# Mattdl/CLsurvey

Measured on AMD Instinct MI355X. Metric: images/sec (train+importance pass), EWC small_VGG9 Tiny-ImageNet task batch, higher is better.
Workload: dtype f32 (bf16x6 split operands on the conv fwd/bwd-data matrix products, fp32 accumulate); 1 GPU; EWC small_VGG9_cl_128_128, Tiny-ImageNet shapes (3x64x64, 20 classes), batch 200: train step + Fisher step (BASELINE configs[1]); batch=200, parallelism=1 GPU

## Files before the change

clsurvey_amd/_lib.py:

```python
import ctypes as C
import os

_HERE = os.path.dirname(os.path.abspath(__file__))
LIB_PATH = os.path.join(_HERE, "libclhip.so")

_p = C.c_void_p
_i = C.c_int
_f = C.c_float
_z = C.c_size_t
_l = C.c_long


class HatParam(C.Structure):
    _fields_ = [("theta", _p), ("grad", _p), ("buf", _p), ("mask_back", _p), ("n", _z), ("is_emb", _i), ("reserved", _i)]


class HatGateJob(C.Structure):
    _fields_ = [("emb_row", _p), ("gate", _p), ("mask_pre", _p), ("n", _i), ("reserved", _i)]


class HatLayer(C.Structure):
    _fields_ = [("w", _p), ("gate_in", _p), ("out", _p), ("K", _z), ("C", _z), ("R", _z)]


class HatWgradJob(C.Structure):
    _fields_ = [("g", _p), ("w", _p), ("gate_in", _p), ("dgate_in", _p), ("K", _i), ("C", _i), ("R", _i), ("reserved", _i)]


class HatEmbJob(C.Structure):
    _fields_ = [("dgate", _p), ("gate", _p), ("mask_pre", _p), ("demb", _p), ("n", _i), ("rows", _i), ("t", _i), ("reserved", _i)]


class IcarlClass(C.Structure):
    _fields_ = [("row_begin", _i), ("row_end", _i), ("k", _i), ("out_off", _i)]


class LayerDesc(C.Structure):
    _fields_ = [("type", _i), ("cin", _i), ("cout", _i), ("relu", _i), ("pool", _i),
                ("w_off", _l), ("b_off", _l), ("ksize", _i), ("stride", _i), ("pad", _i), ("pool_k", _i), ("pool_s", _i),
                ("bn", _i), ("bn_w_off", _l), ("bn_b_off", _l), ("has_drop", _i)]


SIGNATURES = {
    "clhip_version": (_i, []),
    "clhip_arch": (C.c_char_p, []),
    "clhip_conv3x3_fwd": (_i, [_p, _p, _p, _p, _i, _i, _i, _i, _i, _i, _p]),
    "clhip_conv3x3_relu_pool_fwd": (_i, [_p, _p, _p, _p, _p, _i, _i, _i, _i, _i, _p]),
    "clhip_conv3x3_bwd_weight_unpool": (_i, [_p, _p, _p, _p, _p, _i, _i, _i, _i, _i, _p, _z, _p]),
    "clhip_conv3x3_bwd_data": (_i, [_p, _p, _p, _p, _i, _i, _i, _i, _i, _p]),
    "clhip_conv3x3_bwd_data_unpool": (_i, [_p, _p, _p, _p, _p, _i, _i, _i, _i, _i, _p]),
    "clhip_conv3x3_bwd_weight_ws": (_z, [_i, _i, _i, _i, _i]),
    "clhip_conv3x3_bwd_weight": (_i, [_p, _p, _p, _p, _i, _i, _i, _i, _i, _p, _z, _p]),
    "clhip_conv3x3_bwd_weight_slabs": (_i, [_p, _p, _p, _i, _i, _i, _i, _i, _p, _z, C.POINTER(_i), _p]),
    "clhip_conv3x3_bwd_weight_reduce": (_i, [_p, _p, _p, _i, _i, _i, _p]),
    "clhip_conv3x3_wino_ws": (_z, [_i, _i]),
    "clhip_conv3x3_wino_fwd": (_i, [_p, _p, _p, _p, _p, _i, _i, _i, _i, _i, _i, _p, _z, _p]),
    "clhip_conv3x3_wino_bwd_data": (_i, [_p, _p, _p, _p, _p, _i, _i, _i, _i, _i, _p, _z, _p]),
    "clhip_conv5x5_bs_ws": (_z, [_i, _i]),
    "clhip_conv5x5_bs_fwd": (_i, [_p, _p, _p, _p, _i, _i, _i, _i, _i, _i, _p, _z, _p]),
    "clhip_conv5x5_bs_bwd_data": (_i, [_p, _p, _p, _p, _i, _i, _i, _i, _i, _p, _z, _p]),
    "clhip_conv3x3_bs_ws": (_z, [_i, _i]),
    "clhip_conv3x3_bs_fwd": (_i, [_p, _p, _p, _p, _p, _i, _i, _i, _i, _i, _i, _p, _z, _p]),
    "clhip_conv3x3_bs_bwd_data": (_i, [_p, _p, _p, _p, _p, _i, _i, _i, _i, _i, _p, _z, _p]),
    "clhip_conv3x3_wino_bwd_weight_ws": (_z, [_i, _i, _i, _i, _i]),
    "clhip_conv3x3_wino_bwd_weight": (_i, [_p, _p, _p, _p, _p, _i, _i, _i, _i, _i, _p, _z, _p]),
    "clhip_conv3x3_wino_bwd_ws": (_z, [_i, _i, _i, _i, _i]),
    "clhip_conv3x3_wino_bwd": (_i, [_p, _p, _p, _p, _p, _p, _p, _p, _i, _i, _i, _i, _i, _p, _z, _p]),
    "clhip_maxpool2_fwd": (_i, [_p, _p, _p, _i, _i, _i, _p]),
    "clhip_maxpool2_bwd": (_i, [_p, _p, _p, _i, _i, _i, _p]),
    "clhip_fc_ws": (_z, [_i, _i, _i]),
    "clhip_fc_fwd": (_i, [_p, _p, _p, _p, _i, _i, _i, _i, _p, _z, _p]),
    "clhip_fc_bwd_data": (_i, [_p, _p, _p, _p, _i, _i, _i, _p, _z, _p]),
    "clhip_fc_bwd_weight": (_i, [_p, _p, _p, _p, _i, _i, _i, _p, _z, _p]),
    "clhip_relu_bwd": (_i, [_p, _p, _p, _z, _p]),
    "clhip_softmax_ce": (_i, [_p, _p, _i, _i, _i, _p, _p, _p, _p]),
    "clhip_mse_zero_sum": (_i, [_p, _z, _p, _p, _p]),
    "clhip_reg_sgd_step": (_i, [_p, _p, _p, _p, _p, _z, _f, _f, _f, _f, _i, _p]),
    "clhip_fisher_accum": (_i, [_p, _p, _z, _f, _p]),
    "clhip_mas_accum": (_i, [_p, _p, _z, _f, _f, _p]),
    "clhip_si_step": (_i, [_p, _p, _p, _p, _p, _p, _z, _f, _f, _f, _f, _i, _p]),
    "clhip_si_consolidate": (_i, [_p, _p, _p, _p, _z, _f, _p]),
    "clhip_maxpool_fwd": (_i, [_p, _p, _p, _i, _i, _i, _i, _i, _p]),
    "clhip_maxpool_bwd": (_i, [_p, _p, _p, _i, _i, _i, _i, _i, _p]),
    "clhip_conv2d_bwd_weight_ws": (_z, [_i] * 9),
    "clhip_conv2d_fwd": (_i, [_p, _p, _p, _p] + [_i] * 10 + [_p]),
    "clhip_conv2d_bwd_data": (_i, [_p, _p, _p, _p] + [_i] * 9 + [_p]),
    "clhip_conv2d_bwd_weight": (_i, [_p, _p, _p, _p] + [_i] * 9 + [_p, _z, _p]),
    "clhip_conv3x3_bs_bwd_weight_ws": (_z, [_i] * 5),
    "clhip_conv3x3_bs_bwd_weight": (_i, [_p] * 5 + [_i] * 5 + [_p, _z, _p]),
    "clhip_conv5x5_bs_bwd_weight_ws": (_z, [_i] * 5),
    "clhip_conv5x5_bs_bwd_weight": (_i, [_p] * 4 + [_i] * 5 + [_p, _z, _p]),
    "clhip_conv2d_s2d_ws": (_z, [_i] * 8),
    "clhip_conv2d_s2d_fwd": (_i, [_p, _p, _p, _p] + [_i] * 9 + [_p, _z, _p]),
    "clhip_conv2d_s2d_bwd_weight": (_i, [_p, _p, _p, _p] + [_i] * 8 + [_p, _z, _p]),
    "clhip_imm_merge": (_i, [_p, _p, _p, _i, _z, _p, _p]),
    "clhip_lwf_loss": (_i, [_p, _p, _p, _p, _i, _i, _i, _i, _f, _f, _i, _p, _p, _p, _p]),
    "clhip_packnet_finetune_mask": (_i, [_p, _z, _i, _p]),
    "clhip_packnet_kth_ws": (_z, []),
    "clhip_packnet_kth_abs": (_i, [_p, _p, _z, _i, _z, _p, _p, _z, _p]),
    "clhip_packnet_prune": (_i, [_p, _p, _z, _i, _p, _p]),
    "clhip_mask_grad_zero": (_i, [_p, _p, _z, _i, _p]),
    "clhip_mask_weight_zero": (_i, [_p, _p, _z, _i, _i, _p]),
    "clhip_packnet_sgd_step": (_i, [_p, _p, _p, _p, _z, _i, _f, _f, _f, _i, _p]),
    "clhip_hat_gate": (_i, [_p, _i, _f, _p, _p]),
    "clhip_hat_scale_weight": (_i, [_p, _p, _p, _z, _z, _z, _p]),
    "clhip_hat_weight_grad": (_i, [_p, _p, _p, _p, _p, _i, _i, _i, _p]),
    "clhip_hat_emb_grad": (_i, [_p, _p, _p, _i, _f, _f, _p, _p]),
    "clhip_hat_reg_sums": (_i, [_p, _p, _i, _p, _p]),
    "clhip_hat_backmask": (_i, [_p, _p, _p, _z, _z, _z, _p]),
    "clhip_hat_sgd_ws": (_z, []),
    "clhip_hat_sgd_step": (_i, [_p, _p, _p, _p, _z, _f, _f, _f, _i, _i, _f, _f, _f, _f, _i, _p, _z, _p]),
    "clhip_clamp": (_i, [_p, _z, _f, _f, _p]),
    "clhip_hat_sgd_multi_ws": (_z, [_i]),
    "clhip_hat_sgd_step_multi": (_i, [_p, _i, _f, _f, _f, _i, _f, _f, _f, _f, _f, _i, _p, _z, _p]),
    "clhip_hat_gates_multi": (_i, [_p, _i, _f, _p, _p]),
    "clhip_hat_scale_weights_multi": (_i, [_p, _i, _p]),
    "clhip_hat_weight_grads_multi": (_i, [_p, _i, _p]),
    "clhip_hat_emb_grads_multi": (_i, [_p, _i, _f, _f, _f, _p, _p]),
    "clhip_softmax_ce_slice": (_i, [_p, _p, _i, _i, _i, _i, _i, _p, _p, _p, _p]),
    "clhip_net_loss_step_slice": (_i, [_p, _p, _p, _p, _p, _i, _i, _i, _i, _p, _p, _p, _p, _p]),
    "clhip_axpy": (_i, [_p, _p, _z, _f, _i, _p]),
    "clhip_gem_gram_ws": (_z, [_i]),
    "clhip_gem_gram": (_i, [_p, _z, C.POINTER(_i), _i, _z, _p, _p, _z, _p]),
    "clhip_gem_project": (_i, [_p, _z, C.POINTER(_i), C.POINTER(_f), _i, _p, _p, _z, _p]),
    "clhip_gem_qp": (_i, [_p, _i, C.c_double, C.c_double, _p, _p, _p]),
    "clhip_gem_project_dev": (_i, [_p, _z, C.POINTER(_i), _p, _p, _i, _p, _p, _z, _p]),
    "clhip_net_create": (_i, [C.POINTER(LayerDesc), _i, _i, _i, _i, _i, C.POINTER(_p)]),
    "clhip_net_set_dropout": (_i, [_p, _i, _p, _l]),
    "clhip_net_set_bn": (_i, [_p, _i, _p, _p, _f, _f]),
    "clhip_net_set_training": (_i, [_p, _i]),
    "clhip_net_probe": (_i, [_p, _i]),
    "clhip_net_probe_read": (_i, [_p, C.POINTER(_f), C.POINTER(_i)]),
    "clhip_net_layer_input": (_i, [_p, _i, _p, _p]),
    "clhip_net_layer_pool_idx": (_i, [_p, _i, _p, _p]),
    "clhip_net_layer_paths": (_i, [_p, _i]),
    "clhip_net_probe_kind": (_i, [_p, _i, _i]),
    "clhip_net_set_input_grad": (_i, [_p, _i, _p]),
    "clhip_sigmoid_fwd": (_i, [_p, _p, _z, _p]),
    "clhip_sigmoid_bwd": (_i, [_p, _p, _p, _z, _p]),
    "clhip_mse_mean": (_i, [_p, _p, _z, _f, _p, _p, _p]),
    "clhip_adadelta_step": (_i, [_p, _p, _p, _p, _z, _f, _f, _f, _f, _p]),
    "clhip_bn_ws": (_z, [_i]),
    "clhip_bn_fwd": (_i, [_p, _p, _p, _p, _p, _p, _p, _p, _i, _i, _i, _i, _f, _f, _i, _p, _z, _p]),
    "clhip_bn_bwd": (_i, [_p, _p, _p, _p, _p, _p, _p, _p, _p, _i, _i, _i, _i, _i, _p, _z, _p]),
    "clhip_net_destroy": (None, [_p]),
    "clhip_net_workspace_bytes": (_z, [_p]),
    "clhip_net_num_classes": (_i, [_p]),
    "clhip_net_forward": (_i, [_p, _p, _p, _i, _p, _p, _p]),
    "clhip_net_backward": (_i, [_p, _p, _p, _p, _i, _p, _p, _p]),
    "clhip_net_loss_step": (_i, [_p, _p, _p, _p, _p, _i, _i, _p, _p, _p, _p, _p]),
    "clhip_rehearsal_assemble": (_i, [_p, _p, _i, _z, _p, _p, _l, _l, _i, _p, _i, _p, _p, _p]),
    "clhip_rehearsal_assemble_crop_flip": (_i, [_p, _p, _i, _i, _i, _i, _i, _i, _p, _l, _p, _p, _p, _l, _l, _i, _p, _p, _i, _p, _p, _p]),
    "clhip_loss_segments": (_i, [_p, _p, _p, _i, _i, _i, _p, _i, _f, _p, _p, _p, _p]),
    "clhip_net_loss_step_loss_segments": (_i, [_p, _p, _p, _p, _p, _p, _i, _i, _p, _i, _f, _p, _p, _p, _p, _p]),
    "clhip_gather_tasks": (_i, [_p, _i, _z, _p, _i, _p, _p, _p]),
    "clhip_slice_argmax_count": (_i, [_p, _i, _i, _p, _i, _p, _p, _p, _p, _p]),
    "clhip_gather_tasks_crop_flip": (_i, [_p, _i, _i, _i, _i, _i, _i, _p, _p, _i, _p, _p, _p]),
    "clhip_icarl_herd": (_i, [_p, _l, _i, _p, C.POINTER(IcarlClass), _i, _p, _l, _p]),
    "clhip_icarl_nme": (_i, [_p, _p, _i, _i, _i, _i, _i, _p, _p]),
}

_lib = None


def lib():
    global _lib
    if _lib is None:
        path = os.environ.get("CLHIP_LIB", LIB_PATH)
        if not os.path.exists(path):
            raise RuntimeError(
                "clsurvey_amd: %s not found. Build it with `python clsurvey_amd/build.py` "
                "(hipcc --offload-arch=gfx950). There is no CPU fallback." % path)
        import torch
        bundled = os.path.join(os.path.dirname(torch.__file__), "lib", "libamdhip64.so")
        if os.path.exists(bundled):
            C.CDLL(bundled, mode=C.RTLD_GLOBAL)
        h = C.CDLL(path)
        for name, (res, args) in SIGNATURES.items():
            fn = getattr(h, name)
            fn.restype = res
            fn.argtypes = args
        _lib = h
    return _lib


class ClhipError(RuntimeError):
    pass


def check(rc, what):
    if rc != 0:
        if rc > 0:
            raise ClhipError("%s: HIP error %d" % (what, rc))
        names = {-1: "CLHIP_EINVAL", -2: "CLHIP_ENOSPC", -3: "CLHIP_ENOTSUP"}
        raise ClhipError("%s: %s" % (what, names.get(rc, rc)))
```

clsurvey_amd/csrc/common.hpp:

```cpp
#pragma once
#include <hip/hip_runtime.h>
#include <stdint.h>
#include <stddef.h>
#include "../../include/clhip.h"

#define CLHIP_LAUNCH_CHECK()                          \
    do {                                              \
        hipError_t e__ = hipGetLastError();           \
        if (e__ != hipSuccess) return (int)e__;       \
    } while (0)

static inline hipStream_t as_stream(void* s) { return reinterpret_cast<hipStream_t>(s); }

static inline bool aligned16(const void* p) { return (reinterpret_cast<uintptr_t>(p) & 15u) == 0; }

static inline int ew_grid(size_t work_items, int block) {
    size_t g = (work_items + block - 1) / block;
    if (g < 1) g = 1;
    if (g > 2048) g = 2048;
    return (int)g;
}

static __device__ __attribute__((aligned(16))) float clhip_zero16[4] = {0.f, 0.f, 0.f, 0.f};

constexpr int CLHIP_OOB = (int)0x80000000;

constexpr int CLHIP_POOL_DEAD = 4;
typedef unsigned int clhip_u32x4 __attribute__((ext_vector_type(4)));
__device__ __forceinline__ __amdgpu_buffer_rsrc_t clhip_rsrc(const void* p, size_t bytes) {
    return __builtin_amdgcn_make_buffer_rsrc(const_cast<void*>(p), 0, bytes > 0x7fffffffull ? 0x7fffffff : (int)bytes, 0x00020000);
}
__device__ __forceinline__ float clhip_buf_load(__amdgpu_buffer_rsrc_t r, int voff, int soff) {
    return __uint_as_float(__builtin_amdgcn_raw_buffer_load_b32(r, voff, soff, 0));
}
__device__ __forceinline__ float4 clhip_buf_load4(__amdgpu_buffer_rsrc_t r, int voff, int soff) {
    const clhip_u32x4 v = __builtin_amdgcn_raw_buffer_load_b128(r, voff, soff, 0);
    return make_float4(__uint_as_float(v.x), __uint_as_float(v.y), __uint_as_float(v.z), __uint_as_float(v.w));
}
__device__ __forceinline__ float2 clhip_buf_load2(__amdgpu_buffer_rsrc_t r, int voff, int soff) {
    typedef unsigned int u32x2 __attribute__((ext_vector_type(2)));
    const u32x2 v = __builtin_amdgcn_raw_buffer_load_b64(r, voff, soff, 0);
    return make_float2(__uint_as_float(v.x), __uint_as_float(v.y));
}
__device__ __forceinline__ unsigned clhip_buf_load_u16(__amdgpu_buffer_rsrc_t r, int voff, int soff) {
    return (unsigned)__builtin_amdgcn_raw_buffer_load_b16(r, voff, soff, 0);
}
__device__ __forceinline__ unsigned clhip_buf_load_u8(__amdgpu_buffer_rsrc_t r, int voff, int soff) {
    return (unsigned)__builtin_amdgcn_raw_buffer_load_b8(r, voff, soff, 0);
}
#ifndef CLHIP_ST_AUX
#define CLHIP_ST_AUX 16
#endif
__device__ __forceinline__ void clhip_buf_store(float v, __amdgpu_buffer_rsrc_t r, int voff, int soff) {
    __builtin_amdgcn_raw_buffer_store_b32(__float_as_uint(v), r, voff, soff, CLHIP_ST_AUX);
}
__device__ __forceinline__ void clhip_buf_store_u8(uint8_t v, __amdgpu_buffer_rsrc_t r, int voff, int soff) {
    __builtin_amdgcn_raw_buffer_store_b8(v, r, voff, soff, 0);
}
__device__ __forceinline__ void clhip_buf_store4(float4 v, __amdgpu_buffer_rsrc_t r, int voff, int soff) {
    const clhip_u32x4 q = {__float_as_uint(v.x), __float_as_uint(v.y), __float_as_uint(v.z), __float_as_uint(v.w)};
    __builtin_amdgcn_raw_buffer_store_b128(q, r, voff, soff, CLHIP_ST_AUX);
}
__device__ __forceinline__ void clhip_buf_store2(float2 v, __amdgpu_buffer_rsrc_t r, int voff, int soff) {
    typedef unsigned int u32x2 __attribute__((ext_vector_type(2)));
    const u32x2 q = {__float_as_uint(v.x), __float_as_uint(v.y)};
    __builtin_amdgcn_raw_buffer_store_b64(q, r, voff, soff, CLHIP_ST_AUX);
}
__device__ __forceinline__ __amdgpu_buffer_rsrc_t clhip_out_rsrc(void* base) {
    return __builtin_amdgcn_make_buffer_rsrc(base, 0, 0x7fffffff, 0x00020000);
}
__device__ __forceinline__ size_t out_img_of(int C, int hw) { return (size_t)C * hw; }

__device__ __forceinline__ float wave_max(float v) {
#pragma unroll
    for (int o = 32; o > 0; o >>= 1) v = fmaxf(v, __shfl_xor(v, o, 64));
    return v;
}
__device__ __forceinline__ float wave_sum(float v) {
#pragma unroll
    for (int o = 32; o > 0; o >>= 1) v += __shfl_xor(v, o, 64);
    return v;
}
__device__ __forceinline__ double wave_sum(double v) {
#pragma unroll
    for (int o = 32; o > 0; o >>= 1) v += __shfl_xor(v, o, 64);
    return v;
}
__device__ __forceinline__ int wave_min(int v) {
#pragma unroll
    for (int o = 32; o > 0; o >>= 1) v = min(v, __shfl_xor(v, o, 64));
    return v;
}

typedef float floatx16 __attribute__((ext_vector_type(16)));
typedef float floatx4 __attribute__((ext_vector_type(4)));

__device__ __forceinline__ int mfma32_row(int r, int lane) { return (r & 3) + 8 * (r >> 2) + 4 * (lane >> 5); }


#define CLHIP_FC_MAX 4
struct clhip_fc_chain {
    int n;
    long w_off[CLHIP_FC_MAX], b_off[CLHIP_FC_MAX];
    int din[CLHIP_FC_MAX], dout[CLHIP_FC_MAX], relu[CLHIP_FC_MAX];
    size_t act_off[CLHIP_FC_MAX], dz_off[CLHIP_FC_MAX];
};
int clhip_internal_fc_chain_ok(const clhip_fc_chain* d);
int clhip_internal_fc_chain_wgrad(const clhip_fc_chain* d, float* grads, const float* x, int N, const float* acts,
                                  const float* dlogits, const float* dz, hipStream_t s);
struct clhip_gemm_args {
    const float* a; const float* b; float* out;
    int M, N, K; long sam, sak, sbk, sbn; int n_tiles, splits, k_per_split;
    const float* bias; const float* mask_src; int relu;
};
int clhip_internal_fc_bwd_data_args(const float* dy, const float* w, const float* relu_src, float* dx, int M, int I, int O,
                                    clhip_gemm_args* args_out);
int clhip_internal_fc_bwd_combo(const clhip_gemm_args* g, int gemm_blocks, const clhip_fc_chain* d, float* grads, const float* x,
                                int N, const float* acts, const float* dlogits, const float* dz, hipStream_t s);

int clhip_internal_fc_tail_ok(const clhip_fc_chain* d);
int clhip_internal_fc_tail(const clhip_fc_chain* d, const float* params, float* acts, int N, const int64_t* labels,
                           int reduction, int col_off, int ncols, float* dlogits, float* fcdz, float* loss_out, double* stats,
                           void* row_scratch, unsigned* counter, int do_loss, int do_bwd, const float* h1_slabs, int live,
                           hipStream_t s);
int clhip_internal_fc_fwd_partial(const float* x, const float* w, int M, int I, int O, void* ws, size_t ws_bytes, int* live,
                                  hipStream_t s);

#define CLHIP_WGRAD_JOBS_MAX 32
struct clhip_wgrad_job { const float* part; float* dw; float* db; int K, C, splits; int taps; };
int clhip_internal_conv3x3_wgrad_partial(const float* x, const float* dy, const uint8_t* unpool_idx, float* dw, float* db, int N,
                                         int C, int K, int H, int W, void* ws, size_t ws_bytes, void* stream, clhip_wgrad_job* job);
int clhip_internal_wgrad_reduce_multi(const clhip_wgrad_job* jobs, int n, hipStream_t s);

bool clhip_internal_convkk_ok(int N, int Cin, int Cout, int H, int W, int R, int S, int stride, int pad);
int clhip_internal_convkk(int mode, const float* in, const float* w, const float* bias, const float* mask_src, float* out, int N,
                          int Cin, int Cout, int H, int W, int relu, hipStream_t s);

struct clhip_wino_wt { const float* w; float* U; int Ko, Ci, mode, pad; };
int clhip_internal_wino_weights(const clhip_wino_wt* jobs, int n, hipStream_t s);
int clhip_internal_weight_images(const clhip_wino_wt* wino_jobs, int n_wino, const clhip_wino_wt* bs_jobs, int n_bs, hipStream_t s);
int clhip_internal_wino_conv_u(int mode, const float* in, const float* U, const float* bias, const float* mask_src, float* out,
                               uint8_t* pool_idx, int unpool, int N, int Cin, int Cout, int H, int W, int relu, hipStream_t s);
bool clhip_internal_wino_ok(int Cin, int Cout, int H, int W);
size_t clhip_internal_wino_ws(int Cin, int Cout);
bool clhip_internal_bs_ok(int Cin, int Cout, int H, int W);
bool clhip_internal_bs_preferred(int Cin, int Cout, int H, int W);
bool clhip_internal_bs5_preferred(int Cin, int Cout, int H, int W);
size_t clhip_internal_bs5_ws(int Cin, int Cout);
int clhip_internal_bs5_conv_u(int mode, const float* in, const void* wimg, const float* bias, const float* mask_src, float* out, int N,
                              int Cin, int Cout, int H, int W, int relu, hipStream_t s);
size_t clhip_internal_bs_ws(int Cin, int Cout);
int clhip_internal_bs_weights(const clhip_wino_wt* jobs, int n, hipStream_t s);
int clhip_internal_bs_conv_u(int mode, const float* in, const void* wimg, const float* bias, const float* mask_src, float* out,
                             uint8_t* pool_idx, int unpool, int N, int Cin, int Cout, int H, int W, int relu, hipStream_t s);
bool clhip_internal_bs5_wgrad_ok(int N, int C, int K, int H, int W);
size_t clhip_internal_bs5_wgrad_ws(int N, int C, int K, int H, int W);
int clhip_internal_bs5_wgrad(const float* x, const float* dy, float* dw, float* db, int N, int C, int K, int H, int W, void* ws,
                             size_t ws_bytes, hipStream_t s);
size_t clhip_internal_bs3k_wgrad_ws(int N, int C, int K, int H, int W);
int clhip_internal_bs3k_wgrad(const float* x, const float* dy, float* dw, float* db, int N, int C, int K, int H, int W, void* ws,
                              size_t ws_bytes, hipStream_t s);
bool clhip_internal_bs_wgrad_ok(int C, int K, int H, int W);
bool clhip_internal_bs_wgrad_preferred(int C, int K, int H, int W, int pooled);
size_t clhip_internal_bs_wgrad_ws(int N, int C, int K, int H, int W);
int clhip_internal_bs_wgrad_partial(const float* x, const float* dy, const uint8_t* unpool_idx, float* dw, float* db, int N, int C, int K,
                                    int H, int W, void* ws, size_t ws_bytes, hipStream_t s, clhip_wgrad_job* job);
bool clhip_internal_wino_wgrad_ok(int C, int K, int H, int W);
size_t clhip_internal_wino_wgrad_ws(int N, int C, int K, int H, int W);
int clhip_internal_wino_wgrad_partial(const float* x, const float* dy, const uint8_t* unpool_idx, float* dw, float* db, int N, int C,
                                      int K, int H, int W, void* ws, size_t ws_bytes, hipStream_t s, clhip_wgrad_job* job);
int clhip_internal_wino_pair(const float* dy, const uint8_t* unpool_idx, const float* U, const float* mask_src, float* dx,
                             const float* x, float* dw, float* db, int N, int C, int K, int H, int W, void* ws, size_t ws_bytes,
                             hipStream_t s, clhip_wgrad_job* job);
bool clhip_internal_wino_pair_shape(int N, int C, int K, int H, int W, int pooled);
int clhip_internal_wino_conv(int mode, const float* in, const float* w, const float* bias, const float* mask_src, float* out,
                             uint8_t* pool_idx, int unpool, int N, int Cin, int Cout, int H, int W, int relu, void* ws,
                             size_t ws_bytes, hipStream_t s);
```

clsurvey_amd/csrc/conv3x3.hip:

```cpp
#include "common.hpp"

namespace {

#ifdef CLHIP_TRACE
__device__ unsigned long long* g_trace = nullptr;
#define TR_NOW() __builtin_amdgcn_s_memtime()
#endif

constexpr int KT = 64;
constexpr int LDW = 65;

template <int TW, int TH, int NB>
struct Geo {
    static constexpr int BP = TW * TH * NB;
    static constexpr int TWP = TW + 2;
    static constexpr int PLANE = NB * (TH + 2) * TWP;
    static constexpr int NT = (BP + 63) / 64;
    static constexpr bool DENSE = (32 % TW != 0 && TW != 32);
    static_assert(DENSE || BP == 64 || BP == 128, "block tile must hold 64 or 128 pixels");
    static_assert(!DENSE || (NB == 1 && BP <= 192), "dense tiles: one plane of at most 192 pixels");
};

template <int TW, int TH>
__device__ __forceinline__ void tile_pixel(int s, int li, bool pool, int& nb, int& th, int& tw) {
    if (pool && TW == 32) {
        nb = 0; th = 2 * (s >> 1) + (li >> 4); tw = 16 * (s & 1) + (li & 15);
    } else {
        const int q = 32 * s + li;
        tw = q % TW; th = (q / TW) % TH; nb = q / (TW * TH);
        if ((32 % TW != 0 && TW != 32) && q >= TW * TH) { nb = 0; th = TH; tw = 0; }
    }
}

#ifndef CLHIP_CONV_MIN_WAVES
#define CLHIP_CONV_MIN_WAVES 1
#endif
template <int TW, int TH, int NB, int CK>
struct ConvLds {
    static constexpr int BUF_FLOATS = CK * 9 * LDW + CK * Geo<TW, TH, NB>::PLANE;
    static constexpr int FLOATS = 2 * BUF_FLOATS;
};

template <int TW, int TH, int NB, int CK, int MODE, bool VEC, bool UNPOOL = false>
__device__ __forceinline__ void conv3x3_mfma_body(
    const float* __restrict__ in, const float* __restrict__ wt, const float* __restrict__ bias,
    const float* __restrict__ mask_src, float* __restrict__ out,
    int N, int Cin, int Cout, int H, int W, int Kw, int Cw, int relu,
    int tiles_w, int tiles_h, int n_pix_tiles, uint8_t* __restrict__ pool_idx,
    const int bid, const int img0, float* __restrict__ lds, float* __restrict__ bias_s) {
    using G = Geo<TW, TH, NB>;
    static_assert(!UNPOOL || (MODE == 1 && VEC), "the fused un-pool lives in the 16-byte staging of backward-data");
    const bool pool = !UNPOOL && pool_idx != nullptr;
    constexpr int WS_FLOATS = CK * 9 * LDW;
    constexpr int XS_FLOATS = CK * G::PLANE;
    constexpr int BUF_FLOATS = WS_FLOATS + XS_FLOATS;
    static_assert(BUF_FLOATS == ConvLds<TW, TH, NB, CK>::BUF_FLOATS, "shared-array size of the launching kernel");

    const int tid = threadIdx.x;
    const int lane = tid & 63;
    const int wave = tid >> 6;
#ifdef CLHIP_TRACE
    const unsigned long long tr_start = TR_NOW();
#endif
    const int wk = wave & 1;
    const int wp = wave >> 1;
    const int li = lane & 31;
    const int kk = lane >> 5;

    const int kt = bid / n_pix_tiles;
    const int pt = bid - kt * n_pix_tiles;
    const int tw_i = pt % tiles_w;
    const int th_i = (pt / tiles_w) % tiles_h;
    const int ng = pt / (tiles_w * tiles_h);
    const int n0 = img0 + ng * NB, h0 = th_i * TH, w0 = tw_i * TW;
    const int ko0 = kt * KT;
    if (MODE == 0 && threadIdx.x < KT) bias_s[threadIdx.x] = (bias && ko0 + (int)threadIdx.x < Cout) ? bias[ko0 + threadIdx.x] : 0.f;

    constexpr int W_ELEMS = KT * CK * 9;
    const size_t plane_hw = (size_t)H * W;
    const int n_chunks = (Cin + CK - 1) / CK;
    const int Wp = W >> 1;
    const size_t plane_in = UNPOOL ? (size_t)(H >> 1) * Wp : plane_hw;
    const float* in_blk = in + (size_t)n0 * Cin * plane_in;

    constexpr int W_IT = VEC ? (W_ELEMS / 4 + 255) / 256 : (W_ELEMS + 255) / 256;
    constexpr int XROWS = CK * NB * (TH + 2);
    constexpr int XV_ELEMS = XROWS * (TW / 4);
    constexpr int X_IT = VEC ? (XV_ELEMS + 255) / 256 : (XS_FLOATS + 255) / 256;
    constexpr int H_IT = VEC ? (XROWS * 2 + 255) / 256 : 0;
    constexpr int NUNITS = W_IT + X_IT + H_IT;
    float4 wv[VEC ? W_IT : 1];
    float4 xv[VEC ? X_IT : 1];
    float hv[VEC ? (H_IT > 0 ? H_IT : 1) : 1];
    float wreg[VEC ? 1 : W_IT];
    float xreg[VEC ? 1 : X_IT];
    int woff[W_IT], wdst[VEC ? W_IT * (MODE == 0 ? 1 : 4) : W_IT];
    int xoff[X_IT], xdst[VEC ? X_IT : 1];
    int hoff[H_IT > 0 ? H_IT : 1], hdst[H_IT > 0 ? H_IT : 1];
    int wch[VEC ? 1 : W_IT], xch[VEC ? 1 : X_IT];
    float2 xp[UNPOOL ? X_IT : 1];
    unsigned xi[UNPOOL ? X_IT : 1], hi[UNPOOL && H_IT > 0 ? H_IT : 1];
    int xioff[UNPOOL ? X_IT : 1], xcode[UNPOOL ? X_IT : 1], hioff[UNPOOL && H_IT > 0 ? H_IT : 1], hcode[UNPOOL && H_IT > 0 ? H_IT : 1];

    if constexpr (VEC) {
#pragma unroll
        for (int j = 0; j < W_IT; ++j) {
            const int e = tid + 256 * j;
            woff[j] = CLHIP_OOB;
            if (MODE == 0) {
                const int kl = e / (CK * 9 / 4), f = e - kl * (CK * 9 / 4);
                if (e < W_ELEMS / 4 && ko0 + kl < Kw) woff[j] = ((ko0 + kl) * Cw * 9 + 4 * f) * 4;
            } else {
                const int kl = e / (KT * 9 / 4), f = e - kl * (KT * 9 / 4);
                if (e < W_ELEMS / 4 && 4 * f < (Cw - ko0) * 9) woff[j] = ((kl * Cw + ko0) * 9 + 4 * f) * 4;
            }
        }
#pragma unroll
        for (int j = 0; j < X_IT; ++j) {
            const int e = tid + 256 * j;
            const int rowid = e / (TW / 4), f = e - rowid * (TW / 4);
            const int cl = rowid / (NB * (TH + 2)), rr = rowid - cl * (NB * (TH + 2));
            const int nb = rr / (TH + 2), row = rr - nb * (TH + 2);
            const int n = n0 + nb, h = h0 - 1 + row;
            xoff[j] = CLHIP_OOB;
            if constexpr (UNPOOL) {
                xioff[j] = CLHIP_OOB;
                xcode[j] = (h & 1) << 1;
                if (e < XV_ELEMS && n < N && h >= 0 && h < H) {
                    xioff[j] = (int)(((size_t)nb * Cin + cl) * plane_in) + (h >> 1) * Wp + ((w0 + 4 * f) >> 1);
                    xoff[j] = xioff[j] * 4;
                }
            } else if (e < XV_ELEMS && n < N && h >= 0 && h < H) {
                xoff[j] = ((int)(((size_t)nb * Cin + cl) * plane_hw) + h * W + w0 + 4 * f) * 4;
            }
        }
#pragma unroll
        for (int j = 0; j < H_IT; ++j) {
            const int e = tid + 256 * j;
            const int rowid = e >> 1, side = e & 1;
            const int cl = rowid / (NB * (TH + 2)), rr = rowid - cl * (NB * (TH + 2));
            const int nb = rr / (TH + 2), row = rr - nb * (TH + 2);
            const int n = n0 + nb, h = h0 - 1 + row, w = side ? w0 + TW : w0 - 1;
            hoff[j] = CLHIP_OOB;
            if constexpr (UNPOOL) {
                hioff[j] = CLHIP_OOB;
                hcode[j] = ((h & 1) << 1) | (w & 1);
                if (e < XROWS * 2 && n < N && h >= 0 && h < H && w >= 0 && w < W) {
                    hioff[j] = (int)(((size_t)nb * Cin + cl) * plane_in) + (h >> 1) * Wp + (w >> 1);
                    hoff[j] = hioff[j] * 4;
                }
            } else if (e < XROWS * 2 && n < N && h >= 0 && h < H && w >= 0 && w < W) {
                hoff[j] = ((int)(((size_t)nb * Cin + cl) * plane_hw) + h * W + w) * 4;
            }
// ... 510 lines not shown
        const bool real = tap(j, c, r, s2);
#pragma unroll
        for (int half = 0; half < 2; ++half) {
            const int ch = ko0 + 32 * half + li;
            a[half][j] = (real && ch < Cout) ? wt[(size_t)ch * 27 + c * 9 + r * 3 + s2] : 0.f;
        }
    }
    const int b_row = li + kk * C3_TWP, b_col = li + kk, b_pln = li + kk * C3_PLANE;
    auto b_addr = [&](int j) -> int {
        if (j < 9) return b_row + (j / 3) * C3_PLANE + (j % 3);
        if (j < 12) return b_col + (j - 9) * C3_PLANE + 2 * C3_TWP;
        if (j == 12) return b_pln + 2 * C3_TWP + 2;
        return li + 2 * C3_PLANE + 2 * C3_TWP + 2;
    };

    float sv[7];
    const size_t plane_hw = (size_t)H * W;
    const int st_src = kk * W + li;
    const int st_dst = kk * C3_TWP + li + 1;
    const int e_line = lane >> 1, e_side = lane & 1;
    const int e_c = e_line >> 2, e_rr = e_line & 3;
    const int st_esrc = e_c * (int)plane_hw + (e_rr - 1) * W + (e_side ? C3_TW : -1);
    const int st_edst = e_c * C3_PLANE + e_rr * C3_TWP + (e_side ? C3_TW + 1 : 0);
    auto tile_coords = [&](int t, int& n, int& h, int& w0) {
        const int tw = t % tiles_w, q = t / tiles_w;
        const int th = q % tiles_h;
        n = q / tiles_h; h = th * C3_TH + 2 * wave; w0 = tw * C3_TW;
    };
    auto load_tile = [&](int t) {
        int n, h, w0;
        tile_coords(t, n, h, w0);
        const float* xb = x + (size_t)n * 3 * plane_hw + (size_t)h * W + w0;
        bool rok[2];
        rok[0] = (unsigned)(h - 1 + kk) < (unsigned)H;
        rok[1] = (unsigned)(h + 1 + kk) < (unsigned)H;
#pragma unroll
        for (int i = 0; i < 6; ++i) {
            const float* p = xb + (i >> 1) * (ptrdiff_t)plane_hw + (2 * (i & 1) - 1) * W + st_src;
            sv[i] = *(rok[i & 1] ? p : clhip_zero16);
        }
        const bool eok = lane < 24 && (unsigned)(h - 1 + e_rr) < (unsigned)H &&
                         (unsigned)(w0 + (e_side ? C3_TW : -1)) < (unsigned)W;
        const float* pe = xb + st_esrc;
        sv[6] = *(eok ? pe : clhip_zero16);
    };
    float* hw_s = halo_s + wave * (2 * C3_HALO);
    auto store_tile = [&](int buf) {
        float* d = hw_s + buf * C3_HALO;
#pragma unroll
        for (int i = 0; i < 6; ++i) d[(i >> 1) * C3_PLANE + 2 * (i & 1) * C3_TWP + st_dst] = sv[i];
        if (lane < 24) d[st_edst] = sv[6];
    };

    const int OH = H >> 1, OW = W >> 1;
    int tile = blockIdx.x, buf = 0;
    if (tile < ntiles) { load_tile(tile); store_tile(0); }
    __builtin_amdgcn_s_waitcnt(0x0F70);
    __syncthreads();
    float* pw = pool_s + wave * (KT * C3_PLD);
    uint8_t* iw = idx_s + wave * (KT * 16);
    float* pw_l = pw + 4 * kk * C3_PLD + (li >> 1);
    uint8_t* iw_l = iw + 4 * kk * 16 + (li >> 1);
    const float* bias_k = bias_s + 4 * kk;
    for (; tile < ntiles; tile += gridDim.x, buf ^= 1) {
        const int next = tile + gridDim.x;
        if (next < ntiles) load_tile(next);

        floatx16 acc[2][2];
#pragma unroll
        for (int half = 0; half < 2; ++half)
#pragma unroll
            for (int row = 0; row < 2; ++row)
#pragma unroll
                for (int r = 0; r < 16; ++r) acc[half][row][r] = 0.f;
        const float* xs = hw_s + buf * C3_HALO;
        float b0[14], b1[14];
#pragma unroll
        for (int j = 0; j < 14; ++j) { b0[j] = xs[b_addr(j)]; b1[j] = xs[b_addr(j) + C3_TWP]; }
        __builtin_amdgcn_sched_barrier(0);
#pragma unroll
        for (int j = 0; j < 14; ++j) {
            acc[0][0] = __builtin_amdgcn_mfma_f32_32x32x2f32(a[0][j], b0[j], acc[0][0], 0, 0, 0);
            acc[1][0] = __builtin_amdgcn_mfma_f32_32x32x2f32(a[1][j], b0[j], acc[1][0], 0, 0, 0);
            acc[0][1] = __builtin_amdgcn_mfma_f32_32x32x2f32(a[0][j], b1[j], acc[0][1], 0, 0, 0);
            acc[1][1] = __builtin_amdgcn_mfma_f32_32x32x2f32(a[1][j], b1[j], acc[1][1], 0, 0, 0);
        }

        if (next < ntiles) store_tile(buf ^ 1);

        int n, h, w0;
        tile_coords(tile, n, h, w0);
        asm volatile("" ::: "memory");
#pragma unroll
        for (int half = 0; half < 2; ++half)
#pragma unroll
            for (int r = 0; r < 16; ++r) {
                const float bv = bias_k[32 * half + (r & 3) + 8 * (r >> 2)];
                const float tl = fmaxf(acc[half][0][r] + bv, 0.f), bl = fmaxf(acc[half][1][r] + bv, 0.f);
                const float tr = dpp_xor1(tl), br = dpp_xor1(bl);
                float m = tl; int am = 0;
                if (tr > m) { m = tr; am = 1; }
                if (bl > m) { m = bl; am = 2; }
                if (br > m) { m = br; am = 3; }
                if (!(m > 0.f)) am = CLHIP_POOL_DEAD;
                acc[half][0][r] = m;
                acc[half][1][r] = __int_as_float(am);
            }
        if (!(li & 1)) {
#pragma unroll
            for (int half = 0; half < 2; ++half)
#pragma unroll
                for (int r = 0; r < 16; ++r) {
                    const int c0 = 32 * half + (r & 3) + 8 * (r >> 2);
                    pw_l[c0 * C3_PLD] = acc[half][0][r];
                    iw_l[c0 * 16] = (uint8_t)__float_as_int(acc[half][1][r]);
                }
        }
        __builtin_amdgcn_wave_barrier();
        if (h < H) {
            const size_t chw = (size_t)OH * OW;
            const size_t obase = (size_t)n * Cout * chw + (size_t)(h >> 1) * OW + (w0 >> 1);
#pragma unroll
            for (int i = 0; i < 4; ++i) {
                const int q = lane + 64 * i, cl = q >> 2, part = q & 3;
                const float4 v = *reinterpret_cast<const float4*>(pw + cl * C3_PLD + 4 * part);
                if (ko0 + cl < Cout) *reinterpret_cast<float4*>(out + obase + (size_t)(ko0 + cl) * chw + 4 * part) = v;
            }
            const uint4 iv = *reinterpret_cast<const uint4*>(iw + lane * 16);
            if (ko0 + lane < Cout) *reinterpret_cast<uint4*>(pool_idx + obase + (size_t)(ko0 + lane) * chw) = iv;
        }
        __builtin_amdgcn_wave_barrier();
    }
}

#ifndef CLHIP_C3W64
#define CLHIP_C3W64 1
#endif
constexpr int W6_TWP = 67;
constexpr int W6_PLANE = 4 * W6_TWP;
constexpr int W6_HALO = 3 * W6_PLANE;

#ifndef C3W64_ABL
#define C3W64_ABL 0
#endif
#ifndef CLHIP_C3W64_BIAS_IN_K
#define CLHIP_C3W64_BIAS_IN_K 0
#endif
#if C3W64_ABL & 8
__device__ __forceinline__ floatx16 c3w64_fake_mfma(float a, float b, floatx16 c) { c[0] += a * b; return c; }
#define C3W64_MFMA(a, b, c, x, y, z) c3w64_fake_mfma(a, b, c)
#else
#define C3W64_MFMA(a, b, c, x, y, z) __builtin_amdgcn_mfma_f32_32x32x2f32(a, b, c, x, y, z)
#endif
template <bool FULL>
__global__ __launch_bounds__(512) void conv3x3_c3w64_relu_pool_kernel(
    const float* __restrict__ x, const float* __restrict__ wt, const float* __restrict__ bias,
    float* __restrict__ out, uint8_t* __restrict__ pool_idx, int N, int Cout, int H, int W,
    int tiles_w, int row_pairs, int ntiles) {
    __shared__ __attribute__((aligned(16))) float halo_s[8 * 2 * W6_HALO];
#if CLHIP_C3W64_BIAS_IN_K
    __shared__ float ones_s[W6_TWP + 5];
#else
    __shared__ float bias_s[KT];
#endif
    const int tid = threadIdx.x, lane = tid & 63, wave = tid >> 6, li = lane & 31, kk = lane >> 5;
    const int ko0 = blockIdx.y * KT;
#if CLHIP_C3W64_BIAS_IN_K
    if (tid < W6_TWP + 5) ones_s[tid] = 1.f;
#else
    if (tid < KT) bias_s[tid] = (bias && ko0 + tid < Cout) ? bias[ko0 + tid] : 0.f;
#endif

    float a[2][14];
    auto tap = [&](int j, int& c, int& r, int& s) -> bool {
        if (j < 9) { c = j / 3; s = j - 3 * c; r = kk; return true; }
        if (j < 12) { c = j - 9; r = 2; s = kk; return true; }
        if (j == 12) { c = kk; r = 2; s = 2; return true; }
        c = 2; r = 2; s = 2; return kk == 0;
    };
#pragma unroll
    for (int j = 0; j < 14; ++j) {
        int c, r, s2;
        const bool real = tap(j, c, r, s2);
#pragma unroll
        for (int half = 0; half < 2; ++half) {
            const int ch = ko0 + 32 * half + li;
            a[half][j] = (real && ch < Cout) ? wt[(size_t)ch * 27 + c * 9 + r * 3 + s2] : 0.f;
#if CLHIP_C3W64_BIAS_IN_K
            if (j == 13 && kk == 1) a[half][j] = (bias && ch < Cout) ? bias[ch] : 0.f;
#endif
        }
    }
    const int b_row = 2 * li + kk * W6_TWP, b_col = 2 * li + kk, b_pln = 2 * li + kk * W6_PLANE;
    auto b_addr = [&](int j) -> int {
        if (j < 9) return b_row + (j / 3) * W6_PLANE + (j % 3);
        if (j < 12) return b_col + (j - 9) * W6_PLANE + 2 * W6_TWP;
        if (j == 12) return b_pln + 2 * W6_TWP + 2;
        return 2 * li + 2 * W6_PLANE + 2 * W6_TWP + 2;
    };

    const int simd = blockIdx.x * 4 + (wave & 3), nsimd = gridDim.x * 4;
    const int units = 2 * ntiles;
    const int per = units / nsimd, rem = units - per * nsimd;
    const int s_start = simd * per + min(simd, rem), s_cnt = per + (simd < rem ? 1 : 0);
    const int first = (s_cnt + 1) >> 1;
    const int u0 = __builtin_amdgcn_readfirstlane((wave >> 2) ? s_start + first : s_start);
    const int u1 = __builtin_amdgcn_readfirstlane((wave >> 2) ? s_start + s_cnt : s_start + first);

    const size_t plane_hw = (size_t)H * W;
    const __amdgpu_buffer_rsrc_t r_x = clhip_rsrc(x, (size_t)N * 3 * plane_hw * 4);
    float sv[13];
    const int e_line = lane >> 1, e_side = lane & 1, e_c = e_line >> 2, e_rr = e_line & 3;
    auto tile_coords = [&](int t, int& n, int& h, int& w0) {
        const int tw = t % tiles_w, q = t / tiles_w;
        const int rp = q % row_pairs;
        n = q / row_pairs; h = 2 * rp; w0 = tw * 64;
    };
    auto load_tile = [&](int t) {
        int n, h, w0;
        tile_coords(t, n, h, w0);
        const int base = (n * 3 * H + h - 1) * W + w0;
#pragma unroll
        for (int i = 0; i < 12; ++i) {
            const int c = i >> 2, rr = i & 3;
            const bool ok = (unsigned)(h - 1 + rr) < (unsigned)H;
            sv[i] = clhip_buf_load(r_x, ok ? (base + (c * H + rr) * W + lane) * 4 : CLHIP_OOB, 0);
        }
        const int ecol = w0 + (e_side ? 64 : -1);
        const bool eok = (lane < 24) & ((unsigned)(h - 1 + e_rr) < (unsigned)H) & ((unsigned)ecol < (unsigned)W);
        sv[12] = clhip_buf_load(r_x, eok ? ((n * 3 * H + h - 1) * W + (e_c * H + e_rr) * W + ecol) * 4 : CLHIP_OOB, 0);
    };
    float* hw_s = halo_s + wave * (2 * W6_HALO);
    auto store_tile = [&](int buf) {
        float* d = hw_s + buf * W6_HALO;
#pragma unroll
        for (int i = 0; i < 12; ++i) d[(i >> 2) * W6_PLANE + (i & 3) * W6_TWP + 1 + lane] = sv[i];
        if (lane < 24) d[e_c * W6_PLANE + e_rr * W6_TWP + (e_side ? 65 : 0)] = sv[12];
    };

    const int OH = H >> 1, OW = W >> 1;
    const int chw = OH * OW;
    const __amdgpu_buffer_rsrc_t r_o = clhip_rsrc(out, (size_t)N * Cout * chw * 4);
    const __amdgpu_buffer_rsrc_t r_i = clhip_rsrc(pool_idx, (size_t)N * Cout * chw);
    __syncthreads();
    if (u0 >= u1) return;
    int t_cur = u0 >> 1;
    const int t_last = (u1 - 1) >> 1;
    int buf = 0;
    load_tile(t_cur);
    store_tile(0);
    if (t_cur < t_last) load_tile(t_cur + 1);
    for (int u = u0; u < u1; ++u) {
        const int t = u >> 1, half = u & 1;
        float ac[14];
#pragma unroll
        for (int j = 0; j < 14; ++j) ac[j] = half ? a[1][j] : a[0][j];
        floatx16 acc[2][2];
        const float* xs = hw_s + buf * W6_HALO;
        float b[2][2][14];
#pragma unroll
        for (int j = 0; j < 14; ++j)
#pragma unroll
            for (int row = 0; row < 2; ++row)
#pragma unroll
                for (int par = 0; par < 2; ++par)
#if C3W64_ABL & 4
                    b[row][par][j] = __int_as_float(0x3f800000 + j + row + par + lane);
#else
#if CLHIP_C3W64_BIAS_IN_K
                    b[row][par][j] = (j == 13 && kk == 1) ? ones_s[row * W6_TWP + par] : xs[b_addr(j) + row * W6_TWP + par];
#else
                    b[row][par][j] = xs[b_addr(j) + row * W6_TWP + par];
#endif
#endif
        __builtin_amdgcn_sched_barrier(0);
        {
            const floatx16 zero = {0.f, 0.f, 0.f, 0.f, 0.f, 0.f, 0.f, 0.f, 0.f, 0.f, 0.f, 0.f, 0.f, 0.f, 0.f, 0.f};
            acc[0][0] = C3W64_MFMA(ac[0], b[0][0][0], zero, 0, 0, 0);
            acc[0][1] = C3W64_MFMA(ac[0], b[0][1][0], zero, 0, 0, 0);
            acc[1][0] = C3W64_MFMA(ac[0], b[1][0][0], zero, 0, 0, 0);
            acc[1][1] = C3W64_MFMA(ac[0], b[1][1][0], zero, 0, 0, 0);
        }
#pragma unroll
        for (int j = 1; j < 14; ++j) {
            acc[0][0] = C3W64_MFMA(ac[j], b[0][0][j], acc[0][0], 0, 0, 0);
            acc[0][1] = C3W64_MFMA(ac[j], b[0][1][j], acc[0][1], 0, 0, 0);
            acc[1][0] = C3W64_MFMA(ac[j], b[1][0][j], acc[1][0], 0, 0, 0);
            acc[1][1] = C3W64_MFMA(ac[j], b[1][1][j], acc[1][1], 0, 0, 0);
        }
        const bool last_of_tile = u + 1 < u1 && ((u + 1) >> 1) != t;
        if (last_of_tile) {
            store_tile(buf ^ 1);
            t_cur = t + 1;
            if (t_cur < t_last) load_tile(t_cur + 1);
        }
        int n, h, w0;
        tile_coords(t, n, h, w0);
        const int cbase = ko0 + 32 * half;
        const int obase = ((n * Cout + cbase) * OH + (h >> 1)) * OW + (w0 >> 1);
        const int ovoff = (4 * kk * chw + li);
#pragma unroll
        for (int r = 0; r < 16; ++r) {
            const int c0 = (r & 3) + 8 * (r >> 2);
#if CLHIP_C3W64_BIAS_IN_K
            const float bv = 0.f;
#else
            const float bv = bias_s[32 * half + 4 * kk + c0];
#endif
#if C3W64_ABL & 2
            const float m2 = acc[0][0][r] + acc[0][1][r] + acc[1][0][r] + acc[1][1][r];
            const bool cok2 = FULL || cbase + c0 + 4 * kk < Cout;
            clhip_buf_store(m2, r_o, cok2 ? ovoff * 4 : CLHIP_OOB, (obase + c0 * chw) * 4);
            clhip_buf_store_u8((uint8_t)r, r_i, cok2 ? ovoff : CLHIP_OOB, obase + c0 * chw);
            continue;
#endif
            const float tl = acc[0][0][r] + bv, tr = acc[0][1][r] + bv, bl = acc[1][0][r] + bv, br = acc[1][1][r] + bv;
            float mx, m;
            asm("v_max3_f32 %0, %1, %2, %3" : "=v"(mx) : "v"(tl), "v"(tr), "v"(bl));
            asm("v_max_f32 %0, %1, %2" : "=v"(mx) : "v"(mx), "v"(br));
            int am = 3;
            am = bl == mx ? 2 : am;
            am = tr == mx ? 1 : am;
            am = tl == mx ? 0 : am;
            if (!(mx > 0.f)) am = CLHIP_POOL_DEAD;
            asm("v_max_f32 %0, 0, %1" : "=v"(m) : "v"(mx));
            const bool cok = FULL || cbase + c0 + 4 * kk < Cout;
#if C3W64_ABL & 1
            if (m == 12345.678f) {
#endif
            clhip_buf_store(m, r_o, cok ? ovoff * 4 : CLHIP_OOB, (obase + c0 * chw) * 4);
            clhip_buf_store_u8((uint8_t)am, r_i, cok ? ovoff : CLHIP_OOB, obase + c0 * chw);
#if C3W64_ABL & 1
            }
#endif
        }
        if (last_of_tile) buf ^= 1;
    }
}

int launch_c3w64_pool(const float* x, const float* wt, const float* bias, float* out, uint8_t* idx,
                      int N, int Cout, int H, int W, hipStream_t s) {
    const int tiles_w = W / 64, row_pairs = H / 2;
    const long long ntiles = (long long)tiles_w * row_pairs * N;
    const int kts = (Cout + KT - 1) / KT;
    long long gx = 256;
    if (gx * 8 > 2 * ntiles) gx = (2 * ntiles + 7) / 8;
    if (Cout % KT == 0)
        hipLaunchKernelGGL(conv3x3_c3w64_relu_pool_kernel<true>, dim3((unsigned)gx, (unsigned)kts), dim3(512), 0, s,
                           x, wt, bias, out, idx, N, Cout, H, W, tiles_w, row_pairs, (int)ntiles);
    else
        hipLaunchKernelGGL(conv3x3_c3w64_relu_pool_kernel<false>, dim3((unsigned)gx, (unsigned)kts), dim3(512), 0, s,
                           x, wt, bias, out, idx, N, Cout, H, W, tiles_w, row_pairs, (int)ntiles);
    CLHIP_LAUNCH_CHECK();
    return 0;
}

int launch_c3_pool(const float* x, const float* wt, const float* bias, float* out, uint8_t* idx,
                   int N, int Cout, int H, int W, hipStream_t s) {
    const int tiles_w = W / C3_TW, tiles_h = (H + C3_TH - 1) / C3_TH;
    const long long ntiles = (long long)tiles_w * tiles_h * N;
    const int kts = (Cout + KT - 1) / KT;
    if (ntiles <= 0 || ntiles > 0x7fffffffLL) return CLHIP_EINVAL;
    long long gx = 512 / kts;
    if (gx < 1) gx = 1;
    if (gx > ntiles) gx = ntiles;
    hipLaunchKernelGGL(conv3x3_c3_relu_pool_kernel, dim3((unsigned)gx, (unsigned)kts), dim3(256), 0, s,
                       x, wt, bias, out, idx, N, Cout, H, W, tiles_w, tiles_h, (int)ntiles);
    CLHIP_LAUNCH_CHECK();
    return 0;
}

bool vec_ok(const float* in, const float* wt, int Cin, int H, int W, int Cw) {
    const int TW = W > 16 ? 32 : (W > 8 ? 16 : 8);
    return (Cin % 8 == 0) && (Cw % 4 == 0) && (W % 4 == 0) && (W % TW == 0) && aligned16(in) && aligned16(wt);
}

}

extern "C" {

#ifdef CLHIP_TRACE
int clhip_debug_set_conv_trace(void* p) {
    unsigned long long* q = static_cast<unsigned long long*>(p);
    return (int)hipMemcpyToSymbol(HIP_SYMBOL(g_trace), &q, sizeof(q));
}
#endif

int clhip_conv3x3_fwd(const float* x, const float* w, const float* b, float* y,
                      int N, int C, int K, int H, int W, int relu, void* stream) {
    if (!x || !w || !y || N <= 0 || C <= 0 || K <= 0 || H <= 0 || W <= 0) return CLHIP_EINVAL;
    hipStream_t s = as_stream(stream);
    if (C <= 4) return launch_conv<4, 0, false>(x, w, b, nullptr, y, N, C, K, H, W, K, C, relu, s);
    if (vec_ok(x, w, C, H, W, C)) return launch_conv<8, 0, true>(x, w, b, nullptr, y, N, C, K, H, W, K, C, relu, s);
    return launch_conv<8, 0, false>(x, w, b, nullptr, y, N, C, K, H, W, K, C, relu, s);
}

int clhip_conv3x3_relu_pool_fwd(const float* x, const float* w, const float* b, float* y_pool, uint8_t* idx_u8,
                                int N, int C, int K, int H, int W, void* stream) {
    if (!x || !w || !y_pool || !idx_u8 || N <= 0 || C <= 0 || K <= 0 || H <= 0 || W <= 0 || (H & 1) || (W & 1))
        return CLHIP_EINVAL;
    hipStream_t s = as_stream(stream);
    if (CLHIP_C3W64 && C == 3 && W % 64 == 0 && H % 2 == 0 && (size_t)N * 3 * H * W < ((size_t)1 << 29) &&
        (size_t)N * K * (H / 2) * (W / 2) < ((size_t)1 << 29))
        return launch_c3w64_pool(x, w, b, y_pool, idx_u8, N, K, H, W, s);
    if (C == 3 && W % C3_TW == 0) return launch_c3_pool(x, w, b, y_pool, idx_u8, N, K, H, W, s);

    if (C <= 4) return launch_conv<4, 0, false>(x, w, b, nullptr, y_pool, N, C, K, H, W, K, C, 1, s, idx_u8);
    if (vec_ok(x, w, C, H, W, C)) return launch_conv<8, 0, true>(x, w, b, nullptr, y_pool, N, C, K, H, W, K, C, 1, s, idx_u8);
    return launch_conv<8, 0, false>(x, w, b, nullptr, y_pool, N, C, K, H, W, K, C, 1, s, idx_u8);
}

int clhip_conv3x3_bwd_data(const float* dy, const float* w, const float* relu_src, float* dx,
                           int N, int C, int K, int H, int W, void* stream) {
    if (!dy || !w || !dx || N <= 0 || C <= 0 || K <= 0 || H <= 0 || W <= 0) return CLHIP_EINVAL;
    if (vec_ok(dy, w, K, H, W, C))
        return launch_conv<8, 1, true>(dy, w, nullptr, relu_src, dx, N, K, C, H, W, K, C, 0, as_stream(stream));
    return launch_conv<8, 1, false>(dy, w, nullptr, relu_src, dx, N, K, C, H, W, K, C, 0, as_stream(stream));
}

int clhip_conv3x3_bwd_data_unpool(const float* dy_pool, const uint8_t* idx_u8, const float* w, const float* relu_src, float* dx,
                                  int N, int C, int K, int H, int W, void* stream) {
    if (!dy_pool || !idx_u8 || !w || !dx || N <= 0 || C <= 0 || K <= 0 || H <= 0 || W <= 0) return CLHIP_EINVAL;
    if ((H & 1) || (W & 1) || !vec_ok(dy_pool, w, K, H, W, C) || (reinterpret_cast<uintptr_t>(idx_u8) & 1u)) return CLHIP_ENOTSUP;
    return launch_conv<8, 1, true, true>(dy_pool, w, nullptr, relu_src, dx, N, K, C, H, W, K, C, 0, as_stream(stream),
                                         const_cast<uint8_t*>(idx_u8));
}

}
```

clsurvey_amd/csrc/engine.hip:

```cpp
#include <vector>
#include <cstdlib>
#include <new>
#include "common.hpp"

namespace {

struct LayerPlan {
    int type;
    int cin, cout, relu, pool;
    long w_off, b_off;
    int h, w;
    int ks, st, pd;
    int oh, ow;
    int pk, ps;
    int ph, pw;
    size_t in_elems, out_elems, pool_elems;
    size_t act_off;
    size_t pool_off;
    size_t idx_off;
    int bn;
    long bn_w_off, bn_b_off;
    size_t z_off;
    size_t stat_off;
    float* rmean; float* rvar; float bn_momentum, bn_eps;
    size_t wino_uf, wino_ud;
    int wino_f, wino_d, wino_w;
    int bs5_f, bs5_d;
    int bs5_w;
    int bs_f, bs_d;
    int bs_w;
    int s2d;
    size_t s2d_off, s2d_bytes;
    int wg3;
    size_t wg_off, wg_bytes;
    const float* extra_grad;
    const float* drop;
    long drop_stride;
    int has_drop_buf;
    size_t drop_off;
};

constexpr long long WINO_MIN_UNITS = 640;
constexpr long long WINO16_MIN_UNITS = 384;
static bool wino_small_wgrad() { return true; }

static bool wino_enabled() {
    const char* e = std::getenv("CLHIP_WINO");
    return !(e && e[0] == '0');
}

constexpr unsigned PROBE_RING = 64;
#ifndef CLHIP_OVERLAP_DEFAULT
#define CLHIP_OVERLAP_DEFAULT 0
#endif

struct NetPlan {
    std::vector<LayerPlan> layers;
    int max_batch, in_c, in_h, in_w, n_classes;
    size_t in_elems;
    size_t acts_floats;
    size_t idx_bytes;
    size_t grad_floats;
    size_t scratch_bytes;
    size_t wino_bytes;
    size_t off_wino;
    size_t off_s2d;
    int s2d_fresh_n;
    size_t total_bytes;
    size_t off_acts, off_idx, off_g0, off_g1, off_scratch, off_dlogits, off_loss, off_fcdz, off_wg;
    int training;
    int n_wg;
    int fc_first;
    bool fc_fused;
    clhip_fc_chain chain;
    int probe_layer;
    int probe_kind;
    unsigned probe_count;
    std::vector<hipEvent_t> probe_ev;
    bool fc_tail, no_combo;
    unsigned* tail_counter;
    size_t off_rows;
    bool overlap;
    int overlap_mode;
    hipStream_t side;
    std::vector<hipEvent_t> ev_dy, ev_wg;
    ~NetPlan() {
        for (hipEvent_t e : ev_dy) (void)hipEventDestroy(e);
        for (hipEvent_t e : ev_wg) (void)hipEventDestroy(e);
        if (side) (void)hipStreamDestroy(side);
        if (tail_counter) (void)hipFree(tail_counter);
        for (hipEvent_t e : probe_ev) (void)hipEventDestroy(e);
    }
};

inline size_t align_up(size_t v, size_t a) { return (v + a - 1) / a * a; }

__global__ void drop_scale_kernel(float* __restrict__ h, const float* __restrict__ mask, long stride, int feat, size_t total) {
    for (size_t i = blockIdx.x * (size_t)blockDim.x + threadIdx.x; i < total; i += (size_t)gridDim.x * blockDim.x) {
        const size_t n = i / feat, f = i - n * feat;
        h[i] *= mask[n * stride + f];
    }
}

__global__ void add_inplace_kernel(float* __restrict__ a, const float* __restrict__ b, size_t n) {
    for (size_t i = blockIdx.x * (size_t)blockDim.x + threadIdx.x; i < n; i += (size_t)gridDim.x * blockDim.x) a[i] += b[i];
}

int add_inplace(float* a, const float* b, size_t n, hipStream_t s) {
    hipLaunchKernelGGL(add_inplace_kernel, dim3(ew_grid(n, 256)), dim3(256), 0, s, a, b, n);
    CLHIP_LAUNCH_CHECK();
    return 0;
}

__global__ void drop_copy_kernel(const float* __restrict__ h, float* __restrict__ out, const float* __restrict__ mask, long stride,
                                 int feat, size_t total) {
    for (size_t i = blockIdx.x * (size_t)blockDim.x + threadIdx.x; i < total; i += (size_t)gridDim.x * blockDim.x) {
        const size_t n = i / feat, f = i - n * feat;
        out[i] = h[i] * mask[n * stride + f];
    }
}

int drop_copy(const float* h, float* out, const float* mask, long stride, size_t feat, int N, hipStream_t s) {
    const size_t total = feat * N;
    hipLaunchKernelGGL(drop_copy_kernel, dim3(ew_grid(total, 256)), dim3(256), 0, s, h, out, mask, stride, (int)feat, total);
    CLHIP_LAUNCH_CHECK();
    return 0;
}

int drop_scale(float* h, const float* mask, long stride, size_t feat, int N, hipStream_t s) {
    const size_t total = feat * N;
    hipLaunchKernelGGL(drop_scale_kernel, dim3(ew_grid(total, 256)), dim3(256), 0, s, h, mask, stride, (int)feat, total);
    CLHIP_LAUNCH_CHECK();
    return 0;
}

}

extern "C" {

int clhip_net_create(const clhip_layer_desc* descs, int n_layers, int max_batch, int in_c, int in_h, int in_w,
                     void** out_handle) {
    if (!descs || n_layers <= 0 || max_batch <= 0 || !out_handle) return CLHIP_EINVAL;
    NetPlan* p = new (std::nothrow) NetPlan();
    if (!p) return CLHIP_ENOSPC;
    p->max_batch = max_batch; p->in_c = in_c; p->in_h = in_h; p->in_w = in_w;
    p->in_elems = (size_t)in_c * in_h * in_w;
    int c = in_c, h = in_h, w = in_w;
    size_t feat = p->in_elems;
    size_t acts = 0, idxb = 0, gmax = 0, scratch = 0, wg_total = 0, wino_ws = 0, s2d_total = 0;
    int n_wg = 0;
    bool seen_fc = false;
    for (int i = 0; i < n_layers; ++i) {
        LayerPlan L{};
        L.type = descs[i].type; L.cin = descs[i].cin; L.cout = descs[i].cout;
        L.relu = descs[i].relu; L.pool = descs[i].pool; L.w_off = descs[i].w_off; L.b_off = descs[i].b_off;
        if (L.type == 0) {
            if (seen_fc || L.cin != c) { delete p; return CLHIP_EINVAL; }
            L.h = h; L.w = w;
            L.ks = descs[i].ksize > 0 ? descs[i].ksize : 3;
            L.st = descs[i].ksize > 0 ? descs[i].stride : 1;
            L.pd = descs[i].ksize > 0 ? descs[i].pad : 1;
            if (L.st < 1 || L.pd < 0) { delete p; return CLHIP_EINVAL; }
            L.oh = (h + 2 * L.pd - L.ks) / L.st + 1; L.ow = (w + 2 * L.pd - L.ks) / L.st + 1;
            if (L.oh <= 0 || L.ow <= 0) { delete p; return CLHIP_EINVAL; }
            const bool vgg = L.ks == 3 && L.st == 1 && L.pd == 1;
            L.in_elems = (size_t)c * h * w;
            L.out_elems = (size_t)L.cout * L.oh * L.ow;
            L.bn = descs[i].bn ? 1 : 0; L.bn_w_off = descs[i].bn_w_off; L.bn_b_off = descs[i].bn_b_off;
            L.bn_momentum = 0.1f; L.bn_eps = 1e-5f;
            if (L.bn) {
                L.z_off = acts; acts += L.out_elems * max_batch;
                L.stat_off = acts; acts += align_up(2 * (size_t)L.cout, 4);
                const size_t bs = clhip_bn_ws(L.cout);
                if (bs > scratch) scratch = bs;
            }
            L.act_off = acts; acts += L.out_elems * max_batch;
            int oh = L.oh, ow = L.ow;
            if (L.pool) {
                L.pk = descs[i].pool_k > 0 ? descs[i].pool_k : 2;
                L.ps = descs[i].pool_k > 0 ? descs[i].pool_s : 2;
                if (L.ps < 1 || oh < L.pk || ow < L.pk) { delete p; return CLHIP_EINVAL; }
                if (L.pk == 2 && L.ps == 2 && ((oh & 1) || (ow & 1))) { delete p; return CLHIP_EINVAL; }
                L.ph = (oh - L.pk) / L.ps + 1; L.pw = (ow - L.pk) / L.ps + 1;
                L.pool_elems = (size_t)L.cout * L.ph * L.pw;
                L.pool_off = acts; acts += L.pool_elems * max_batch;
                L.idx_off = idxb; idxb += align_up(L.pool_elems * max_batch, 256);
                oh = L.ph; ow = L.pw;
            }
            L.wg3 = (vgg && (L.w % 4 == 0 || L.cin * 9 <= 32)) ? 1 : 0;
            size_t s = L.wg3 ? clhip_conv3x3_bwd_weight_ws(max_batch, L.cin, L.cout, L.h, L.w)
                             : clhip_conv2d_bwd_weight_ws(max_batch, L.cin, L.h, L.w, L.cout, L.ks, L.ks, L.st, L.pd);
            if (s > scratch) scratch = s;
            if (L.wg3) { L.wg_off = wg_total; L.wg_bytes = align_up(s, 256); wg_total += L.wg_bytes; ++n_wg; }
            if (vgg && !L.bn) {
                const long long tiles = (long long)max_batch * ((L.h + 1) / 2) * ((L.w + 1) / 2);
                auto units = [&](int kout) { return ((tiles + 31) / 32) * ((kout + 31) / 32); };
                auto enough = [&](int kout) {
                    if (units(kout) >= WINO_MIN_UNITS) return true;
                    return L.h == 8 && L.w == 8 && (long long)max_batch * ((kout + 31) / 32) >= WINO16_MIN_UNITS;
                };
                const bool wino = wino_enabled();
                L.wino_f = wino && clhip_internal_wino_ok(L.cin, L.cout, L.h, L.w) && enough(L.cout);
                L.wino_d = wino && i > 0 && clhip_internal_wino_ok(L.cout, L.cin, L.h, L.w) && enough(L.cin);
                const bool even = ((L.h | L.w) & 1) == 0;
                L.bs_f = clhip_internal_bs_preferred(L.cin, L.cout, L.h, L.w) && (even || !L.pool);
                L.bs_d = i > 0 && clhip_internal_bs_preferred(L.cout, L.cin, L.h, L.w) && (even || !L.pool);
                if (L.bs_f) L.wino_f = 1;
                if (L.bs_d) L.wino_d = 1;
                if (wino && clhip_internal_wino_wgrad_ok(L.cin, L.cout, L.h, L.w)) {
                    const int kc = (L.cin / 64) * (L.cout / 64), splits = (256 + kc - 1) / kc;
                    const long long stages = (long long)max_batch * (((L.w + 1) / 2 + (L.w >= 16 ? 7 : 3)) / (L.w >= 16 ? 8 : 4)) *
                                             (((L.h + 1) / 2 + (L.w >= 16 ? 1 : 3)) / (L.w >= 16 ? 2 : 4));
                    L.wino_w = stages >= 8LL * splits || wino_small_wgrad();
                    if (L.wino_w) {
                        const size_t ww = clhip_internal_wino_wgrad_ws(max_batch, L.cin, L.cout, L.h, L.w);
                        if (L.wg3) {
                            if (ww > L.wg_bytes) { wg_total += align_up(ww, 256) - L.wg_bytes; L.wg_bytes = align_up(ww, 256); }
                        } else {
                            L.wg_off = wg_total; L.wg_bytes = align_up(ww, 256); wg_total += L.wg_bytes; ++n_wg;
                        }
                    }
                }
                {
                    const bool pooled22 = L.pool && L.pk == 2 && L.ps == 2;
                    const bool merged = i > 0 && L.wino_w && L.wino_d && !L.bs_d && L.wg_bytes &&
                                        clhip_internal_wino_pair_shape(max_batch, L.cin, L.cout, L.h, L.w, pooled22 ? 1 : 0);
                    if (!merged && clhip_internal_bs_wgrad_preferred(L.cin, L.cout, L.h, L.w, pooled22 ? 1 : 0)) {
                        const size_t bw = clhip_internal_bs_wgrad_ws(max_batch, L.cin, L.cout, L.h, L.w);
                        if (bw && L.wg3) {
                            L.bs_w = 1;
                            if (bw > L.wg_bytes) { wg_total += align_up(bw, 256) - L.wg_bytes; L.wg_bytes = align_up(bw, 256); }
                        }
                    }
                }
                if (L.wino_f) { L.wino_uf = wino_ws; wino_ws += align_up(L.bs_f ? clhip_internal_bs_ws(L.cin, L.cout) : clhip_internal_wino_ws(L.cin, L.cout), 256); }
                if (L.wino_d) { L.wino_ud = wino_ws; wino_ws += align_up(L.bs_d ? clhip_internal_bs_ws(L.cout, L.cin) : clhip_internal_wino_ws(L.cout, L.cin), 256); }
            }
            if (!vgg && !L.bn && L.ks == 5 && L.st == 1 && L.pd == 2) {
                L.bs5_f = clhip_internal_bs5_preferred(L.cin, L.cout, L.h, L.w);
                L.bs5_d = i > 0 && clhip_internal_bs5_preferred(L.cout, L.cin, L.h, L.w);
                {
                    const char* e = std::getenv("CLHIP_BS_WGRAD");
                    const size_t w5 = (e && e[0] == '0') ? 0 : clhip_internal_bs5_wgrad_ws(max_batch, L.cin, L.cout, L.h, L.w);
                    if (w5) { L.bs5_w = 1; if (w5 > scratch) scratch = w5; }
                }
                if (L.bs5_f) { L.wino_uf = wino_ws; wino_ws += align_up(clhip_internal_bs5_ws(L.cin, L.cout), 256); }
                if (L.bs5_d) { L.wino_ud = wino_ws; wino_ws += align_up(clhip_internal_bs5_ws(L.cout, L.cin), 256); }
            }
            if (!vgg && !L.bn && i == 0 && !descs[i].has_drop) {
                const char* e = std::getenv("CLHIP_S2D");
                const size_t sb = !(e && e[0] == '1') ? 0 : clhip_conv2d_s2d_ws(max_batch, L.cin, L.h, L.w, L.cout, L.ks, L.st, L.pd);
                if (sb) { L.s2d = 1; L.s2d_off = s2d_total; L.s2d_bytes = align_up(sb, 256); s2d_total += L.s2d_bytes; }
            }
            if (L.out_elems > gmax) gmax = L.out_elems;
            if (L.in_elems > gmax) gmax = L.in_elems;
            h = oh; w = ow;
            c = L.cout;
            feat = (size_t)c * h * w;
        } else if (L.type == 1) {
            seen_fc = true;
            if ((size_t)L.cin != feat) { delete p; return CLHIP_EINVAL; }
            L.in_elems = feat; L.out_elems = (size_t)L.cout;
            L.act_off = acts; acts += L.out_elems * max_batch;
            size_t s = clhip_fc_ws(max_batch, L.cin, L.cout);
            if (s > scratch) scratch = s;
            if (L.in_elems > gmax) gmax = L.in_elems;
            if (L.out_elems > gmax) gmax = L.out_elems;
            feat = L.out_elems;
        } else { delete p; return CLHIP_EINVAL; }
        L.has_drop_buf = (descs[i].has_drop && i > 0) ? 1 : 0;
        if (L.has_drop_buf) { L.drop_off = acts; acts += L.in_elems * max_batch; }
        p->layers.push_back(L);
    }
    p->n_classes = (int)feat;
    p->acts_floats = acts; p->idx_bytes = idxb; p->grad_floats = gmax * max_batch; p->scratch_bytes = scratch;
    size_t off = 0;
    p->off_acts = off; off += align_up(acts * 4, 256);
    p->off_idx = off; off += align_up(idxb, 256);
    p->off_g0 = off; off += align_up(p->grad_floats * 4, 256);
    p->off_g1 = off; off += align_up(p->grad_floats * 4, 256);
    p->off_scratch = off; off += align_up(scratch, 256);
    p->wino_bytes = wino_ws;
    p->off_wino = off; off += align_up(wino_ws, 256);
    p->off_dlogits = off; off += align_up((size_t)max_batch * p->n_classes * 4, 256);
    p->off_loss = off; off += 256;
    p->fc_first = n_layers;
    for (int i = 0; i < n_layers; ++i) if (p->layers[i].type == 1) { p->fc_first = i; break; }
    p->fc_fused = false;
    p->off_fcdz = off;
    const int nfc = n_layers - p->fc_first;
    if (nfc >= 1 && nfc <= CLHIP_FC_MAX) {
        clhip_fc_chain& ch = p->chain;
        ch.n = nfc;
        size_t dzf = 0;
        for (int l = 0; l < nfc; ++l) {
            const LayerPlan& L = p->layers[p->fc_first + l];
            ch.w_off[l] = L.w_off; ch.b_off[l] = L.b_off; ch.din[l] = L.cin; ch.dout[l] = L.cout; ch.relu[l] = L.relu;
            ch.act_off[l] = L.act_off;
            ch.dz_off[l] = dzf;
            if (l < nfc - 1) dzf += (size_t)L.cout * max_batch;
        }
        if (clhip_internal_fc_chain_ok(&ch)) {
            p->fc_fused = true;
            off += align_up(dzf * 4 + 256, 256);
            p->off_rows = off;
            off += align_up((size_t)max_batch * 8, 256);
        }
    }
    p->off_wg = off;
    p->n_wg = (n_wg >= 2 && n_wg <= CLHIP_WGRAD_JOBS_MAX) ? n_wg : 0;
    if (p->n_wg) off += align_up(wg_total, 256);
    p->off_s2d = off; off += s2d_total;
    p->s2d_fresh_n = 0;
    p->total_bytes = off;
    p->training = 1;
    p->overlap = false;
    p->side = nullptr;
    const char* ov = getenv("CLHIP_WGRAD_OVERLAP");
    bool any_bn = false;
    for (const LayerPlan& L : p->layers) any_bn = any_bn || L.bn;
    p->overlap_mode = (ov && ov[0] == '1') ? 1 : (ov && ov[0] == '2') ? 2 : CLHIP_OVERLAP_DEFAULT;
    if (p->overlap_mode && !any_bn) {
        if (hipStreamCreateWithFlags(&p->side, hipStreamNonBlocking) == hipSuccess) {
            p->overlap = true;
            p->ev_dy.resize(n_layers); p->ev_wg.resize(n_layers);
            for (int i = 0; i < n_layers && p->overlap; ++i)
                if (hipEventCreateWithFlags(&p->ev_dy[i], hipEventDisableTiming) != hipSuccess ||
                    hipEventCreateWithFlags(&p->ev_wg[i], hipEventDisableTiming) != hipSuccess) p->overlap = false;
        } else {
            (void)hipGetLastError();
            p->side = nullptr;
        }
    }
    p->probe_layer = -1;
    p->probe_kind = 0;
    p->probe_count = 0;
    p->fc_tail = false;
    p->no_combo = false;
    p->tail_counter = nullptr;
    const char* tl = getenv("CLHIP_FC_TAIL");
    if (tl && tl[0] == '0') p->no_combo = true;
    if (p->fc_fused && !(tl && tl[0] == '0') && clhip_internal_fc_tail_ok(&p->chain) &&
        max_batch <= 1024) {
        if (hipMalloc(reinterpret_cast<void**>(&p->tail_counter), 256) == hipSuccess &&
            hipMemset(p->tail_counter, 0, 256) == hipSuccess) {
            p->fc_tail = true;
        } else {
            (void)hipGetLastError();
            if (p->tail_counter) { (void)hipFree(p->tail_counter); p->tail_counter = nullptr; }
        }
    }
    *out_handle = p;
    return 0;
}

int clhip_net_set_dropout(void* handle, int layer, const float* mask, long row_stride) {
    NetPlan* p = static_cast<NetPlan*>(handle);
    if (!p || layer <= 0 || layer >= (int)p->layers.size() || row_stride < 0) return CLHIP_EINVAL;
    p->layers[layer].drop = mask;
    p->layers[layer].drop_stride = row_stride;
    return 0;
}

int clhip_net_set_bn(void* handle, int layer, float* running_mean, float* running_var, float momentum, float eps) {
    NetPlan* p = static_cast<NetPlan*>(handle);
    if (!p || layer < 0 || layer >= (int)p->layers.size() || !p->layers[layer].bn || !(eps > 0.f)) return CLHIP_EINVAL;
    LayerPlan& L = p->layers[layer];
    L.rmean = running_mean; L.rvar = running_var; L.bn_momentum = momentum; L.bn_eps = eps;
    return 0;
}

int clhip_net_layer_input(void* handle, int layer, size_t* ws_float_off, size_t* in_elems) {
    NetPlan* p = static_cast<NetPlan*>(handle);
    if (!p || layer <= 0 || layer >= (int)p->layers.size() || !ws_float_off || !in_elems) return CLHIP_EINVAL;
    const LayerPlan& P = p->layers[layer - 1];
    *ws_float_off = p->off_acts / sizeof(float) + ((P.type == 0 && P.pool) ? P.pool_off : P.act_off);
    *in_elems = p->layers[layer].in_elems;
    return 0;
}

int clhip_net_layer_pool_idx(void* handle, int layer, size_t* ws_byte_off, size_t* elems) {
    NetPlan* p = static_cast<NetPlan*>(handle);
    if (!p || layer < 0 || layer >= (int)p->layers.size() || !ws_byte_off || !elems) return CLHIP_EINVAL;
    const LayerPlan& L = p->layers[layer];
    if (L.type != 0 || !L.pool) return CLHIP_EINVAL;
    *ws_byte_off = p->off_idx + L.idx_off;
    *elems = L.pool_elems;
    return 0;
}

int clhip_net_layer_paths(void* handle, int layer) {
    NetPlan* p = static_cast<NetPlan*>(handle);
    if (!p || layer < 0 || layer >= (int)p->layers.size()) return CLHIP_EINVAL;
    const LayerPlan& L = p->layers[layer];
    const bool defer_capable = p->n_wg > 0 && !(p->overlap && p->overlap_mode == 1);
    return (L.wino_f ? 1 : 0) | (L.wino_d ? 2 : 0) | ((L.wino_w && defer_capable) ? 4 : 0) | ((L.bs_f || L.bs5_f) ? 8 : 0) |
           ((L.bs_d || L.bs5_d) ? 16 : 0) | ((L.bs_w && defer_capable) ? 32 : 0);
}

int clhip_net_set_input_grad(void* handle, int layer, const float* extra) {
    NetPlan* p = static_cast<NetPlan*>(handle);
    if (!p || layer <= 0 || layer >= (int)p->layers.size()) return CLHIP_EINVAL;
    p->layers[layer].extra_grad = extra;
    return 0;
}

int clhip_net_probe(void* handle, int layer) {
    NetPlan* p = static_cast<NetPlan*>(handle);
    if (!p || layer >= (int)p->layers.size()) return CLHIP_EINVAL;
    if (layer >= 0 && p->probe_ev.empty()) {
        std::vector<hipEvent_t> made;
        made.reserve(2 * PROBE_RING);
        for (unsigned i = 0; i < 2 * PROBE_RING; ++i) {
            hipEvent_t e;
            if (hipEventCreate(&e) != hipSuccess) {
                for (hipEvent_t m : made) (void)hipEventDestroy(m);
                return CLHIP_ENOTSUP;
            }
            made.push_back(e);
        }
        p->probe_ev.swap(made);
    }
    p->probe_layer = layer;
    p->probe_kind = 0;
    p->probe_count = 0;
    return 0;
}

int clhip_net_probe_kind(void* handle, int layer, int kind) {
    if (kind < 0 || kind > 2) return CLHIP_EINVAL;
    const int rc = clhip_net_probe(handle, layer);
    if (rc == 0) static_cast<NetPlan*>(handle)->probe_kind = kind;
    return rc;
}

int clhip_net_probe_read(void* handle, float* avg_us, int* count) {
    NetPlan* p = static_cast<NetPlan*>(handle);
    if (!p || !avg_us || !count) return CLHIP_EINVAL;
    const unsigned n = p->probe_count < PROBE_RING ? p->probe_count : PROBE_RING;
    double sum = 0.0;
    for (unsigned i = 0; i < n; ++i) {
        const unsigned slot = (p->probe_count - 1 - i) % PROBE_RING;
        float ms = 0.f;
        hipError_t e = hipEventSynchronize(p->probe_ev[2 * slot + 1]);
        if (e == hipSuccess) e = hipEventElapsedTime(&ms, p->probe_ev[2 * slot], p->probe_ev[2 * slot + 1]);
        if (e != hipSuccess) return (int)e;
        sum += ms;
    }
    *avg_us = n ? (float)(sum / n * 1e3) : 0.f;
    *count = (int)n;
    p->probe_count = 0;
    return 0;
}

int clhip_net_set_training(void* handle, int training) {
    NetPlan* p = static_cast<NetPlan*>(handle);
    if (!p) return CLHIP_EINVAL;
    p->training = training ? 1 : 0;
    return 0;
}

void clhip_net_destroy(void* handle) { delete static_cast<NetPlan*>(handle); }

size_t clhip_net_workspace_bytes(void* handle) { return handle ? static_cast<NetPlan*>(handle)->total_bytes : 0; }
int clhip_net_num_classes(void* handle) { return handle ? static_cast<NetPlan*>(handle)->n_classes : 0; }

static bool tail_usable(const NetPlan* p, const float* params, const void* ws, int N) {
    if (!p->fc_tail) return false;
    for (size_t i = p->fc_first + 1; i < p->layers.size(); ++i)
        if (p->layers[i].drop || p->layers[i].extra_grad) return false;
    const float* acts = reinterpret_cast<const float*>(static_cast<const char*>(ws) + p->off_acts);
    return aligned16(params + p->chain.w_off[1]) && aligned16(params + p->chain.w_off[2]) && aligned16(acts + p->chain.act_off[0]) &&
           aligned16(params + p->chain.b_off[0]) &&
           (size_t)N * (p->n_classes | 1) <= 12288;
}

static int plan_conv_u(int bs, int mode, const float* in, const float* U, const float* bias, const float* mask_src, float* out,
                       uint8_t* pool_idx, int unpool, int N, int Cin, int Cout, int H, int W, int relu, hipStream_t s) {
    return bs ? clhip_internal_bs_conv_u(mode, in, U, bias, mask_src, out, pool_idx, unpool, N, Cin, Cout, H, W, relu, s)
              : clhip_internal_wino_conv_u(mode, in, U, bias, mask_src, out, pool_idx, unpool, N, Cin, Cout, H, W, relu, s);
}

static int wino_prepare(NetPlan* p, const float* params, char* base, bool fwd, bool bwd, hipStream_t s) {
    std::vector<clhip_wino_wt> jobs, bsjobs;
    jobs.reserve(2 * p->layers.size());
    bsjobs.reserve(2 * p->layers.size());
    for (const LayerPlan& L : p->layers) {
        if (L.type != 0) continue;
        if (fwd && L.wino_f)
            (L.bs_f ? bsjobs : jobs).push_back(clhip_wino_wt{params + L.w_off, reinterpret_cast<float*>(base + p->off_wino + L.wino_uf), L.cout, L.cin, 0, 0});
        if (bwd && L.wino_d)
            (L.bs_d ? bsjobs : jobs).push_back(clhip_wino_wt{params + L.w_off, reinterpret_cast<float*>(base + p->off_wino + L.wino_ud), L.cin, L.cout, 1, 0});
        if (fwd && L.bs5_f)
            bsjobs.push_back(clhip_wino_wt{params + L.w_off, reinterpret_cast<float*>(base + p->off_wino + L.wino_uf), L.cout, L.cin, 0, 5});
        if (bwd && L.bs5_d)
            bsjobs.push_back(clhip_wino_wt{params + L.w_off, reinterpret_cast<float*>(base + p->off_wino + L.wino_ud), L.cin, L.cout, 1, 5});
    }
    return clhip_internal_weight_images(jobs.data(), (int)jobs.size(), bsjobs.data(), (int)bsjobs.size(), s);
}

static int net_forward_impl(void* handle, const float* params, const float* x, int N, void* ws, float* logits_out,
                            void* stream, int tail, int* slabs_live = nullptr, bool prep_bwd = false) {
    NetPlan* p = static_cast<NetPlan*>(handle);
    if (!p || !params || !x || !ws || N <= 0 || N > p->max_batch) return CLHIP_EINVAL;
    char* base = static_cast<char*>(ws);
    float* acts = reinterpret_cast<float*>(base + p->off_acts);
    uint8_t* idx = reinterpret_cast<uint8_t*>(base + p->off_idx);
    void* scratch = base + p->off_scratch;
    if (p->wino_bytes) {
        int rcw = wino_prepare(p, params, base, true, prep_bwd, as_stream(stream));
        if (rcw) return rcw;
    }
    const float* cur = x;
    int rc;
    const size_t n_run = tail ? (size_t)p->fc_first + 1 : p->layers.size();
    int live = 0;
    for (size_t li = 0; li < n_run; ++li) {
        const LayerPlan& L = p->layers[li];
        float* y = acts + L.act_off;
        const bool probed = (int)li == p->probe_layer && p->probe_kind == 0 && !p->probe_ev.empty();
        if (probed) (void)hipEventRecord(p->probe_ev[2 * (p->probe_count % PROBE_RING)], as_stream(stream));
        struct ProbeEnd {
            NetPlan* p; bool on; hipStream_t s;
            ~ProbeEnd() { if (on) { (void)hipEventRecord(p->probe_ev[2 * (p->probe_count % PROBE_RING) + 1], s); ++p->probe_count; } }
        } probe_end{p, probed, as_stream(stream)};
        if (L.drop && L.has_drop_buf) {
            float* dropped = acts + L.drop_off;
            rc = drop_copy(cur, dropped, L.drop, L.drop_stride, L.in_elems, N, as_stream(stream));
            if (rc) return rc;
            cur = dropped;
        } else if (L.drop) {
            rc = drop_scale(const_cast<float*>(cur), L.drop, L.drop_stride, L.in_elems, N, as_stream(stream));
            if (rc) return rc;
        }
        const bool vgg = L.type == 0 && L.ks == 3 && L.st == 1 && L.pd == 1;
        const bool pool22 = L.pool && L.pk == 2 && L.ps == 2;
        if (L.type == 0 && (L.bn || !(vgg && (!L.pool || pool22)))) {
            float* zc = L.bn ? acts + L.z_off : y;
            const int crelu = L.bn ? 0 : L.relu;
            rc = (vgg && L.wino_f)
                     ? plan_conv_u(L.bs_f, 0, cur, reinterpret_cast<const float*>(base + p->off_wino + L.wino_uf), params + L.b_off,
                                                  nullptr, zc, nullptr, 0, N, L.cin, L.cout, L.h, L.w, crelu, as_stream(stream))
                 : vgg ? clhip_conv3x3_fwd(cur, params + L.w_off, params + L.b_off, zc, N, L.cin, L.cout, L.h, L.w, crelu, stream)
                 : L.bs5_f ? clhip_internal_bs5_conv_u(0, cur, base + p->off_wino + L.wino_uf, params + L.b_off, nullptr, zc, N, L.cin, L.cout,
                                                       L.h, L.w, crelu, as_stream(stream))
                 : L.s2d ? clhip_conv2d_s2d_fwd(cur, params + L.w_off, params + L.b_off, zc, N, L.cin, L.h, L.w, L.cout, L.ks, L.st, L.pd,
                                                crelu, base + p->off_s2d + L.s2d_off, L.s2d_bytes, stream)
                     : clhip_conv2d_fwd(cur, params + L.w_off, params + L.b_off, zc, N, L.cin, L.h, L.w, L.cout, L.ks, L.ks, L.st,
                                        L.pd, crelu, stream);
            if (rc) return rc;
            if (L.s2d) p->s2d_fresh_n = N;
            if (L.bn) {
                float* st = acts + L.stat_off;
                rc = clhip_bn_fwd(zc, params + L.bn_w_off, params + L.bn_b_off, L.rmean, L.rvar, y, st, st + L.cout, N, L.cout,
                                  L.oh * L.ow, p->training, L.bn_momentum, L.bn_eps, L.relu, scratch, p->scratch_bytes, stream);
                if (rc) return rc;
            }
            cur = y;
            if (L.pool) {
                float* pl = acts + L.pool_off;
                rc = pool22 ? clhip_maxpool2_fwd(y, pl, idx + L.idx_off, N * L.cout, L.oh, L.ow, stream)
                            : clhip_maxpool_fwd(y, pl, idx + L.idx_off, N * L.cout, L.oh, L.ow, L.pk, L.ps, stream);
                if (rc) return rc;
                cur = pl;
            }
        } else if (L.type == 0) {
            if (L.pool && L.relu) {
                float* pl = acts + L.pool_off;
                rc = L.wino_f ? plan_conv_u(L.bs_f, 0, cur, reinterpret_cast<const float*>(base + p->off_wino + L.wino_uf),
                                                           params + L.b_off, nullptr, pl, idx + L.idx_off, 0, N, L.cin, L.cout, L.h, L.w, 1,
                                                           as_stream(stream))
                              : clhip_conv3x3_relu_pool_fwd(cur, params + L.w_off, params + L.b_off, pl, idx + L.idx_off, N, L.cin,
                                                            L.cout, L.h, L.w, stream);
                if (rc) return rc;
                cur = pl;
            } else {
                rc = L.wino_f ? plan_conv_u(L.bs_f, 0, cur, reinterpret_cast<const float*>(base + p->off_wino + L.wino_uf),
                                                           params + L.b_off, nullptr, y, nullptr, 0, N, L.cin, L.cout, L.h, L.w, L.relu,
                                                           as_stream(stream))
                              : clhip_conv3x3_fwd(cur, params + L.w_off, params + L.b_off, y, N, L.cin, L.cout, L.h, L.w, L.relu, stream);
                if (rc) return rc;
                cur = y;
                if (L.pool) {
                    float* pl = acts + L.pool_off;
                    rc = clhip_maxpool2_fwd(y, pl, idx + L.idx_off, N * L.cout, L.h, L.w, stream);
                    if (rc) return rc;
                    cur = pl;
                }
            }
        } else {
            if (tail && (int)li == p->fc_first) {
                rc = clhip_internal_fc_fwd_partial(cur, params + L.w_off, N, L.cin, L.cout, scratch, p->scratch_bytes, &live,
                                                   as_stream(stream));
                if (rc) return rc;
            }
            if (!live) {
                rc = clhip_fc_fwd(cur, params + L.w_off, params + L.b_off, y, N, L.cin, L.cout, L.relu, scratch,
                                  p->scratch_bytes, stream);
                if (rc) return rc;
            }
            cur = y;
        }
    }
    if (slabs_live) *slabs_live = live;
    if (tail == 1) return 0;
    if (tail == 2) {
        rc = clhip_internal_fc_tail(&p->chain, params, acts, N, nullptr, 0, 0, 0, nullptr, nullptr, nullptr, nullptr,
                                    base + p->off_rows, p->tail_counter, 0, 0, static_cast<const float*>(scratch), live,
                                    as_stream(stream));
        if (rc) return rc;
        cur = acts + p->layers.back().act_off;
    }
    if (logits_out) {
        hipError_t e = hipMemcpyAsync(logits_out, cur, (size_t)N * p->n_classes * sizeof(float),
                                      hipMemcpyDeviceToDevice, as_stream(stream));
        if (e != hipSuccess) return (int)e;
    }
    return 0;
}

int clhip_net_forward(void* handle, const float* params, const float* x, int N, void* ws, float* logits_out,
                      void* stream) {
    NetPlan* p = static_cast<NetPlan*>(handle);
    if (!p || !params || !x || !ws || N <= 0 || N > p->max_batch) return CLHIP_EINVAL;
    return net_forward_impl(handle, params, x, N, ws, logits_out, stream, tail_usable(p, params, ws, N) ? 2 : 0);
}

static int net_backward_impl(void* handle, const float* params, float* grads, const float* x, int N, void* ws,
                             const float* dlogits, void* stream, bool tail_done, bool wino_ready = false) {
    NetPlan* p = static_cast<NetPlan*>(handle);
    if (!p || !params || !grads || !x || !ws || !dlogits || N <= 0 || N > p->max_batch) return CLHIP_EINVAL;
    char* base = static_cast<char*>(ws);
    float* acts = reinterpret_cast<float*>(base + p->off_acts);
    uint8_t* idx = reinterpret_cast<uint8_t*>(base + p->off_idx);
    float* g[2] = {reinterpret_cast<float*>(base + p->off_g0), reinterpret_cast<float*>(base + p->off_g1)};
    void* scratch = base + p->off_scratch;
    const float* gin = dlogits;
    int gin_buf = -1;
    int flip = 0;
    int rc;
    const int top = (int)p->layers.size() - 1;
    float* fcdz = reinterpret_cast<float*>(base + p->off_fcdz);
    hipStream_t main_s = as_stream(stream);
    if (p->wino_bytes && !wino_ready) {
        rc = wino_prepare(p, params, base, false, true, main_s);
        if (rc) return rc;
    }
    const bool ov = p->overlap && p->overlap_mode == 1;
    const bool ov_small = p->overlap && p->overlap_mode == 2;
    auto side_ok = [&](int layer) {
        if (ov) return true;
        const LayerPlan& Ls = p->layers[layer];
        return ov_small && Ls.type == 0 && Ls.wg3 && Ls.h * Ls.w <= 256;
    };
    hipEvent_t pending[2] = {nullptr, nullptr};
    hipEvent_t last_side = nullptr;
    int taken = -1;
    const bool defer = p->n_wg > 0 && !ov;
    auto pair_ok = [&](const LayerPlan& Lp, int layer) {
        return defer && layer > 0 && Lp.type == 0 && Lp.ks == 3 && Lp.st == 1 && Lp.pd == 1 && !Lp.bn && Lp.wino_w && Lp.wino_d &&
               !Lp.bs_d && !Lp.bs_w && Lp.wg_bytes && !Lp.drop && !Lp.extra_grad && !side_ok(layer);
    };
    clhip_wgrad_job jobs[CLHIP_WGRAD_JOBS_MAX];
    int n_jobs = 0;
    auto take = [&]() -> float* {
        const int bi = flip;
        flip ^= 1;
        if (pending[bi]) { (void)hipStreamWaitEvent(main_s, pending[bi], 0); pending[bi] = nullptr; }
        taken = bi;
        return g[bi];
    };
    auto on_side = [&](int layer, int dy_buf, auto&& launch) -> int {
        if (!side_ok(layer)) return launch(stream);
        hipError_t e = hipEventRecord(p->ev_dy[layer], main_s);
        if (e == hipSuccess) e = hipStreamWaitEvent(p->side, p->ev_dy[layer], 0);
        if (e != hipSuccess) return (int)e;
        const int r = launch((void*)p->side);
        if (r) return r;
        e = hipEventRecord(p->ev_wg[layer], p->side);
        if (e != hipSuccess) return (int)e;
        last_side = p->ev_wg[layer];
        if (dy_buf >= 0) pending[dy_buf] = p->ev_wg[layer];
        return 0;
    };
    for (int i = top; i >= 0; --i) {
        const LayerPlan& L = p->layers[i];
        const float* xin = x;
        if (i > 0) {
            const LayerPlan& P = p->layers[i - 1];
            xin = acts + ((P.type == 0 && P.pool) ? P.pool_off : P.act_off);
            if (L.drop && L.has_drop_buf) xin = acts + L.drop_off;
        }
        const float* xmask = xin;
        if (i > 0 && L.type == 0 && !L.drop) {
            const LayerPlan& P = p->layers[i - 1];
            if (P.type == 0 && !P.bn && P.ks == 3 && P.st == 1 && P.pd == 1 && P.pool && P.pk == 2 && P.ps == 2 && P.relu) xmask = nullptr;
        }
        if (L.type == 1 && tail_done && i > p->fc_first) {
            gin = fcdz + p->chain.dz_off[i - p->fc_first - 1];
            gin_buf = -1;
            continue;
        }
        if (L.type == 1) {
            if (!p->fc_fused) {
                rc = clhip_fc_bwd_weight(xin, gin, grads + L.w_off, grads + L.b_off, N, L.cin, L.cout, scratch, p->scratch_bytes, stream);
                if (rc) return rc;
            }
            bool combo = false;
            clhip_fc_chain ch;
            if (p->fc_fused && i == p->fc_first) {
                ch = p->chain;
                for (int l = 1; l < ch.n; ++l) {
                    const LayerPlan& Ll = p->layers[p->fc_first + l];
                    if (Ll.drop && Ll.has_drop_buf) ch.act_off[l - 1] = Ll.drop_off;
                }
            }
            if (i > 0) {
                float* gout;
                if (p->fc_fused && i > p->fc_first) { gout = fcdz + p->chain.dz_off[i - p->fc_first - 1]; gin_buf = -1; }
                else { gout = take(); gin_buf = taken; }
                clhip_gemm_args ga;
// ... 265 lines not shown
```

clsurvey_amd/csrc/wino.hip:

```cpp
#include "common.hpp"
#include "bs_weight.hpp"
#include <cstdlib>

namespace {

#ifndef CLHIP_W16G_ABL
#define CLHIP_W16G_ABL 0
#endif
#ifndef CLHIP_W16G_PRIO
#define CLHIP_W16G_PRIO 2
#endif
#ifndef CLHIP_W16_ADIRECT
#define CLHIP_W16_ADIRECT 1
#endif
#ifndef CLHIP_W16G_PRIO_UNPOOL
#define CLHIP_W16G_PRIO_UNPOOL 0
#endif
#ifndef CLHIP_WGPS_FENCE
#ifndef CLHIP_WGPS_PITCH
#define CLHIP_WGPS_PITCH 0
#endif
#define CLHIP_WGPS_FENCE 1
#endif
#ifndef CLHIP_W16G_BURST
#define CLHIP_W16G_BURST 0
#endif
#ifndef CLHIP_W16G_PF
#define CLHIP_W16G_PF 2
#endif
#ifndef CLHIP_W16G_ADIRECT
#define CLHIP_W16G_ADIRECT 1
#endif

constexpr int WKT = 64;
constexpr int WCK = 8;
constexpr int WFP = 20;
constexpr int W_FLOATS = WCK * WKT * WFP;
constexpr int WD_FLOATS = 4 * WKT * 16;
#if CLHIP_W16G_ADIRECT
constexpr int WU_FLOATS = W_FLOATS + 2 * WD_FLOATS;
#else
constexpr int WU_FLOATS = W_FLOATS;
#endif

__device__ __forceinline__ void wino_u_store(float* __restrict__ U, int kts, int n_chunks, int kt, int chunk, int c_l, int k_l,
                                             const float4 (&u)[4]) {
    float4* dst = reinterpret_cast<float4*>(U + (((size_t)(kt * n_chunks + chunk) * WCK + c_l) * WKT + k_l) * WFP);
#pragma unroll
    for (int a = 0; a < 4; ++a) dst[a] = u[a];
    dst[4] = make_float4(0.f, 0.f, 0.f, 0.f);
#if CLHIP_W16G_ADIRECT
    float* Ud = U + (size_t)kts * n_chunks * W_FLOATS;
    const int chunk4 = 2 * chunk + (c_l >> 2), q = c_l & 3, wk = k_l >> 5, r = (k_l >> 4) & 1, ti = k_l & 15;
    float4* dd = reinterpret_cast<float4*>(Ud + ((((size_t)(kt * 2 * n_chunks + chunk4) * 2 + wk) * 2 + r) * 4) * 256 + (q * 16 + ti) * 4);
#pragma unroll
    for (int a = 0; a < 4; ++a) dd[a * 64] = u[a];
#else
    (void)kts;
#endif
}

template <int TCB, int TRB, int NIMG>
struct WGeoW {
    static_assert(TCB * TRB * NIMG == 64, "64 tiles per block");
    static constexpr int PW = 2 * TCB + 2;
    static constexpr int PR = 2 * TRB + 2;
    static constexpr int PLANE = NIMG * PR * PW;
    static constexpr int X_FLOATS = WCK * PLANE;
    static constexpr int BUF = W_FLOATS + X_FLOATS;
};

__global__ __launch_bounds__(256) void wino_weight_kernel(const float* __restrict__ w, float* __restrict__ U, int Ko, int Ci,
                                                          int mode, int n_chunks) {
    const int total = ((Ko + WKT - 1) / WKT) * n_chunks * WCK * WKT;
    for (int i = blockIdx.x * 256 + threadIdx.x; i < total; i += gridDim.x * 256) {
        const int k_l = i % WKT, c_l = (i / WKT) % WCK, chunk = (i / (WKT * WCK)) % n_chunks, kt = i / (WKT * WCK * n_chunks);
        const int k = kt * WKT + k_l, c = chunk * WCK + c_l;
        float g[3][3];
#pragma unroll
        for (int r = 0; r < 3; ++r)
#pragma unroll
            for (int s = 0; s < 3; ++s) {
                float v = 0.f;
                if (k < Ko && c < Ci)
                    v = mode == 0 ? w[((size_t)k * Ci + c) * 9 + r * 3 + s]
                                  : w[((size_t)c * Ko + k) * 9 + (2 - r) * 3 + (2 - s)];
                g[r][s] = v;
            }
        float t[4][3];
#pragma unroll
        for (int s = 0; s < 3; ++s) {
            t[0][s] = g[0][s];
            t[1][s] = 0.5f * (g[0][s] + g[1][s] + g[2][s]);
            t[2][s] = 0.5f * (g[0][s] - g[1][s] + g[2][s]);
            t[3][s] = g[2][s];
        }
        float4 u[4];
#pragma unroll
        for (int a = 0; a < 4; ++a)
            u[a] = make_float4(t[a][0], 0.5f * (t[a][0] + t[a][1] + t[a][2]), 0.5f * (t[a][0] - t[a][1] + t[a][2]), t[a][2]);
        wino_u_store(U, (Ko + WKT - 1) / WKT, n_chunks, kt, chunk, c_l, k_l, u);
    }
}

constexpr int WT_JOBS = 24;
struct WtJobs { int n; int pad; clhip_wino_wt j[WT_JOBS]; int first[WT_JOBS + 1]; };

__device__ __forceinline__ void wino_weight_one(const float* __restrict__ w, float* __restrict__ U, int Ko, int Ci, int mode,
                                                int n_chunks, int i) {
    const int k_l = i % WKT, c_l = (i / WKT) % WCK, chunk = (i / (WKT * WCK)) % n_chunks, kt = i / (WKT * WCK * n_chunks);
    const int k = kt * WKT + k_l, c = chunk * WCK + c_l;
    float g[3][3];
#pragma unroll
    for (int r = 0; r < 3; ++r)
#pragma unroll
        for (int s = 0; s < 3; ++s) {
            float v = 0.f;
            if (k < Ko && c < Ci)
                v = mode == 0 ? w[((size_t)k * Ci + c) * 9 + r * 3 + s] : w[((size_t)c * Ko + k) * 9 + (2 - r) * 3 + (2 - s)];
            g[r][s] = v;
        }
    float t[4][3];
#pragma unroll
    for (int s = 0; s < 3; ++s) {
        t[0][s] = g[0][s];
        t[1][s] = 0.5f * (g[0][s] + g[1][s] + g[2][s]);
        t[2][s] = 0.5f * (g[0][s] - g[1][s] + g[2][s]);
        t[3][s] = g[2][s];
    }
    float4 u[4];
#pragma unroll
    for (int a = 0; a < 4; ++a)
        u[a] = make_float4(t[a][0], 0.5f * (t[a][0] + t[a][1] + t[a][2]), 0.5f * (t[a][0] - t[a][1] + t[a][2]), t[a][2]);
    wino_u_store(U, (Ko + WKT - 1) / WKT, n_chunks, kt, chunk, c_l, k_l, u);
}

__global__ __launch_bounds__(256) void wino_weight_multi_kernel(WtJobs J) {
    int jb = 0;
    for (int i = 1; i < J.n; ++i) jb = ((int)blockIdx.x >= J.first[i]) ? i : jb;
    const clhip_wino_wt& q = J.j[jb];
    if ((J.pad >> jb) & 1) {
        bs_weight_block(q, (int)blockIdx.x - J.first[jb], (int)threadIdx.x);
        return;
    }
    const int n_chunks = (q.Ci + WCK - 1) / WCK;
    const int total = ((q.Ko + WKT - 1) / WKT) * n_chunks * WCK * WKT;
    const int i = ((int)blockIdx.x - J.first[jb]) * 256 + threadIdx.x;
    if (i < total) wino_weight_one(q.w, q.U, q.Ko, q.Ci, q.mode, n_chunks, i);
}

template <int TCB, int TRB, int NIMG, int MODE, bool UNPOOL, bool ROWPACK = false>
__global__ __launch_bounds__(256, 1) void wino_conv_kernel(
    const float* __restrict__ in, const float* __restrict__ U, const float* __restrict__ bias,
    const float* __restrict__ mask_src, float* __restrict__ out, uint8_t* __restrict__ pool_idx,
    int N, int Cin, int Cout, int H, int W, int relu, int tiles_w, int tiles_h, int n_pix_blocks) {
    using G = WGeoW<TCB, TRB, NIMG>;
    static_assert(!ROWPACK || (TRB == 1 && !UNPOOL), "row packing: one tile row per entity, no fused un-pooling");
    __shared__ __attribute__((aligned(16))) float lds[2 * G::BUF];
    __shared__ float bias_s[WKT];
    const int tid = threadIdx.x, lane = tid & 63, wave = tid >> 6;
    const int wk = wave & 1, wp = wave >> 1;
    const int li = lane & 31, kk = lane >> 5;

    const int kt = blockIdx.x / n_pix_blocks, pb = blockIdx.x - kt * n_pix_blocks;
    const int bw = pb % tiles_w, bh = (pb / tiles_w) % tiles_h, ng = pb / (tiles_w * tiles_h);
    const int v0 = ROWPACK ? pb * NIMG : 0;
    const int n0 = ROWPACK ? v0 / tiles_h : ng * NIMG, h0 = ROWPACK ? 0 : bh * 2 * TRB, w0 = ROWPACK ? 0 : bw * 2 * TCB;
    const int ko0 = kt * WKT;
    const int n_chunks = (Cin + WCK - 1) / WCK;
    if (MODE == 0 && tid < WKT) bias_s[tid] = (bias && ko0 + tid < Cout) ? bias[ko0 + tid] : 0.f;

    const int Hi = UNPOOL ? H >> 1 : H, Wi = UNPOOL ? W >> 1 : W;
    const size_t plane_in = (size_t)Hi * Wi;
    const float* in_blk = in + (size_t)n0 * Cin * plane_in;
    const __amdgpu_buffer_rsrc_t rs_x = clhip_rsrc(in_blk, (size_t)(N - n0) * Cin * plane_in * sizeof(float));
    const __amdgpu_buffer_rsrc_t rs_i = clhip_rsrc(UNPOOL ? pool_idx + (size_t)n0 * Cin * plane_in : pool_idx,
                                                   UNPOOL ? (size_t)(N - n0) * Cin * plane_in : 0);
    const __amdgpu_buffer_rsrc_t rs_u = clhip_rsrc(U + (size_t)kt * n_chunks * W_FLOATS, (size_t)n_chunks * W_FLOATS * sizeof(float));

    constexpr int W_IT = W_FLOATS / 4 / 256;
    constexpr int X_IT = (G::X_FLOATS + 255) / 256;
    constexpr int NU = W_IT + X_IT;
    float4 wv[W_IT];
    float xr[X_IT];
    unsigned xi[UNPOOL ? X_IT : 1];
    int xoff[X_IT], xcode[UNPOOL ? X_IT : 1];
#pragma unroll
    for (int j = 0; j < X_IT; ++j) {
        const int e = tid + 256 * j;
        xoff[j] = CLHIP_OOB;
        if (e < G::X_FLOATS) {
            const int cl = e / G::PLANE, rem = e - cl * G::PLANE;
            const int col = rem % G::PW, rr = rem / G::PW;
            const int row = rr % G::PR, nb = rr / G::PR;
            int n = n0 + nb, h = h0 - 1 + row;
            const int w = w0 - 1 + col;
            if constexpr (ROWPACK) { const int v = v0 + nb; n = v / tiles_h; h = 2 * (v - n * tiles_h) - 1 + row; }
            const int nr = n - n0;
            if (n < N && h >= 0 && h < H && w >= 0 && w < W) {
                if constexpr (UNPOOL) {
                    xoff[j] = (int)(((size_t)nr * Cin + cl) * plane_in) + (h >> 1) * Wi + (w >> 1);
                    xcode[j] = ((h & 1) << 1) | (w & 1);
                } else {
                    xoff[j] = ((int)(((size_t)nr * Cin + cl) * plane_in) + h * W + w) * 4;
                }
            }
        }
    }
    auto load_unit = [&](int u, int chunk) {
        const int cw = chunk < n_chunks ? chunk : n_chunks - 1;
        if (u < W_IT) {
            wv[u] = clhip_buf_load4(rs_u, (tid + 256 * u) * 16, cw * W_FLOATS * 4);
        } else {
            const int j = u - W_IT;
            const int xb = cw * WCK * (int)plane_in;
            if constexpr (UNPOOL) {
                xr[j] = clhip_buf_load(rs_x, xoff[j] != CLHIP_OOB ? xoff[j] * 4 : CLHIP_OOB, xb * 4);
                xi[j] = clhip_buf_load_u8(rs_i, xoff[j], xb);
            } else {
                xr[j] = clhip_buf_load(rs_x, xoff[j], xb * 4);
            }
        }
    };
    auto store_unit = [&](int u, int bo) {
        if (u < W_IT) {
            float* wd = lds + bo + 4 * (tid + 256 * u);
            *reinterpret_cast<floatx4*>(wd) = floatx4{wv[u].x, wv[u].y, wv[u].z, wv[u].w};
        } else {
            const int j = u - W_IT;
            float* xs = lds + bo + W_FLOATS;
            if (256 * (j + 1) <= G::X_FLOATS || tid + 256 * j < G::X_FLOATS) {
                if constexpr (UNPOOL) xs[tid + 256 * j] = ((int)xi[j] == xcode[j]) ? xr[j] : 0.f;
                else xs[tid + 256 * j] = xr[j];
            }
        }
    };

    const int t_idx = 32 * wp + li;
    const int t_img = t_idx / (TRB * TCB), t_row = (t_idx / TCB) % TRB, t_col = t_idx % TCB;
    const int d_off = W_FLOATS + kk * G::PLANE + (t_img * G::PR + 2 * t_row) * G::PW + 2 * t_col;
    const int a_off = (kk * WKT + wk * 32 + li) * WFP;

    floatx16 acc[16];
#pragma unroll
    for (int f = 0; f < 16; ++f)
#pragma unroll
        for (int r = 0; r < 16; ++r) acc[f][r] = 0.f;

    typedef float f2 __attribute__((ext_vector_type(2)));
    constexpr int NP = WCK / 2;
    floatx4 av[2][4];
    float vv[2][16];
    f2 dlo[4], dhi[4], tlo[4], thi[4];
    auto rd_a = [&](const float* abase, int pair, int q, int slot) {
        av[slot][q] = *reinterpret_cast<const floatx4*>(abase + 2 * pair * WKT * WFP + 4 * q);
    };
    auto rd_d = [&](const float* dbase, int pair, int r) {
        dlo[r] = *reinterpret_cast<const f2*>(dbase + 2 * pair * G::PLANE + r * G::PW);
        dhi[r] = *reinterpret_cast<const f2*>(dbase + 2 * pair * G::PLANE + r * G::PW + 2);
    };
    auto row_tf = [&](int i) {
        if (i == 0) { tlo[0] = dlo[0] - dlo[2]; thi[0] = dhi[0] - dhi[2]; }
        if (i == 1) { tlo[1] = dlo[1] + dlo[2]; thi[1] = dhi[1] + dhi[2]; }
        if (i == 2) { tlo[2] = dlo[2] - dlo[1]; thi[2] = dhi[2] - dhi[1]; }
        if (i == 3) { tlo[3] = dlo[1] - dlo[3]; thi[3] = dhi[1] - dhi[3]; }
    };
    auto col_tf = [&](int i, int slot) {
        const f2 o = tlo[i] - thi[i];
        vv[slot][4 * i + 0] = o.x;
        vv[slot][4 * i + 3] = o.y;
        vv[slot][4 * i + 1] = tlo[i].y + thi[i].x;
        vv[slot][4 * i + 2] = thi[i].x - tlo[i].y;
    };

#pragma unroll
    for (int u = 0; u < NU; ++u) load_unit(u, 0);
#pragma unroll
    for (int u = 0; u < NU; ++u) store_unit(u, 0);
#pragma unroll
    for (int u = 0; u < NU; ++u) load_unit(u, 1);
    __syncthreads();
#pragma unroll
    for (int q = 0; q < 4; ++q) rd_a(lds + a_off, 0, q, 0);
#pragma unroll
    for (int r = 0; r < 4; ++r) rd_d(lds + d_off, 0, r);
#pragma unroll
    for (int i = 0; i < 4; ++i) row_tf(i);
#pragma unroll
    for (int i = 0; i < 4; ++i) col_tf(i, 0);

    static_assert(NU <= 32, "two store units per slot of pair 0, one load unit per slot of pairs 1-2");
    for (int chunk = 0; chunk < n_chunks; ++chunk) {
        const int bo = (chunk & 1) * G::BUF, bn = G::BUF - bo;
        const float* a_cur = lds + bo + a_off;
        const float* d_cur = lds + bo + d_off;
        const float* a_nxt = lds + bn + a_off;
        const float* d_nxt = lds + bn + d_off;
#pragma unroll
        for (int p = 0; p < NP; ++p) {
            const float* ab = (p + 1 < NP) ? a_cur : a_nxt;
            const float* db = (p + 1 < NP) ? d_cur : d_nxt;
// ... 1310 lines not shown
            t[0][j] = m[0][j] + s12;
            t[1][j] = 0.5f * (m[1][j] - m[2][j]);
            t[2][j] = s12 + m[3][j];
        }
        const int k = k0 + wp * 16 + 4 * q + r;
        if (k < K && cidx < C) {
#pragma unroll
            for (int a = 0; a < 3; ++a) {
                const float s12 = 0.5f * (t[a][1] + t[a][2]);
                clhip_buf_store(t[a][0] + s12, rs_slab, (int)(((3 * a + 0) * K + k) * C + cidx) * 4, 0);
                clhip_buf_store(0.5f * (t[a][1] - t[a][2]), rs_slab, (int)(((3 * a + 1) * K + k) * C + cidx) * 4, 0);
                clhip_buf_store(s12 + t[a][3], rs_slab, (int)(((3 * a + 2) * K + k) * C + cidx) * 4, 0);
            }
        }
    }
    if (ct == 0 && wc == 0) {
        bfin += __shfl_xor(bfin, 16, 64);
        bfin += __shfl_xor(bfin, 32, 64);
        const int k = k0 + wp * 16 + li;
        if (q == 0 && k < K) clhip_buf_store(bfin, rs_slab, (int)(9 * K * C + k) * 4, 0);
    }
}

template <int TCS, int TRS, bool UNPOOL, bool VEC>
__global__ __launch_bounds__(256, 2) void wino_wgrad_ps_kernel(
    const float* __restrict__ x, const float* __restrict__ dy, float* __restrict__ part, const uint8_t* __restrict__ unpool_idx,
    int N, int C, int K, int H, int W, int tiles_w, int tiles_h, int total_stages, int splits, int c_tiles, size_t slab_stride) {
    __shared__ __attribute__((aligned(16))) float lds[WGeoP<TCS, TRS>::LDS_FLOATS];
    wino_wgrad_ps_body<TCS, TRS, UNPOOL, VEC>(lds, (int)blockIdx.x, x, dy, part, unpool_idx, N, C, K, H, W, tiles_w, tiles_h,
                                              total_stages, splits, c_tiles, slab_stride);
}

static bool wgrad_ps_on() { return true; }

template <int DK, int TC, int TR, int EROWS, bool UNPOOL, int TCS, int TRS>
__global__ __launch_bounds__(256, 2) void wino_pair_kernel(
    const float* __restrict__ d_in, const float* __restrict__ d_U, const float* __restrict__ d_mask, float* __restrict__ d_out,
    uint8_t* __restrict__ d_idx, int N, int d_Cin, int d_Cout, int H, int W, int d_tiles_w, int d_tiles_h, int d_npb,
    const float* __restrict__ w_x, float* __restrict__ w_part, int w_tiles_w, int w_tiles_h, int w_total, int w_splits, int w_ctiles,
    size_t w_slab, int nb_w) {
    constexpr int LD = DK ? wino16_lds_floats<UNPOOL, 1>() : wino16g_lds_floats<TC, TR, EROWS>(), LW = WGeoP<TCS, TRS>::LDS_FLOATS;
    __shared__ __attribute__((aligned(16))) float lds[LD > LW ? LD : LW];
    const int b = (int)blockIdx.x;
    const int kind = b < nb_w ? 1 : 0, idx = kind ? b : b - nb_w;
    if (kind == 0) {
        if constexpr (DK)
            wino_conv16_body<1, UNPOOL, 1>(lds, idx, d_in, d_U, nullptr, d_mask, d_out, d_idx, N, d_Cin, d_Cout, 0);
        else
            wino_conv16g_body<TC, TR, EROWS, 1, UNPOOL>(lds, idx, d_in, d_U, nullptr, d_mask, d_out, d_idx, N, d_Cin, d_Cout, H, W, 0,
                                                        d_tiles_w, d_tiles_h, d_npb);
    } else
        wino_wgrad_ps_body<TCS, TRS, UNPOOL, true>(lds, idx, w_x, d_in, w_part, d_idx, N, d_Cout, d_Cin, H, W, w_tiles_w, w_tiles_h,
                                                   w_total, w_splits, w_ctiles, w_slab);
}

template <int MODE, bool UNPOOL>
int launch_wino(const float* in, const float* U, const float* bias, const float* mask_src, float* out, uint8_t* pool_idx,
                int N, int Cin, int Cout, int H, int W, int relu, hipStream_t s) {
    const int kts = (Cout + WKT - 1) / WKT;
    if (H == 8 && W == 8 && ((long long)N * 16 + 31) / 32 * ((Cout + 31) / 32) < WINO16_BELOW_UNITS) {
        const bool narrow = (long long)N * ((Cout + 31) / 32) <= 512;
        const long long blocks = (long long)(narrow ? N : (N + 1) / 2) * kts;
        if (blocks <= 0 || blocks > 0x7fffffffLL) return CLHIP_EINVAL;
        if (narrow)
            hipLaunchKernelGGL((wino_conv16_kernel<MODE, UNPOOL, 1>), dim3((unsigned)blocks), dim3(256), 0, s, in, U, bias, mask_src, out,
                               pool_idx, N, Cin, Cout, relu);
        else
            hipLaunchKernelGGL((wino_conv16_kernel<MODE, UNPOOL, 2>), dim3((unsigned)blocks), dim3(256), 0, s, in, U, bias, mask_src, out,
                               pool_idx, N, Cin, Cout, relu);
        CLHIP_LAUNCH_CHECK();
        return 0;
    }
    if (wino16g_on()) {
#define WINO_16G(TC_, TR_, ER_, UNP_)                                                                                          \
        do {                                                                                                                   \
            const int tiles_w = ((W + 1) / 2 + TC_ - 1) / TC_, groups = ((H + 1) / 2 + ER_ - 1) / ER_;                          \
            constexpr int NE_ = 2 * TR_ / ER_;                                                                                  \
            const long long npb = (((long long)N * groups + NE_ - 1) / NE_) * tiles_w, blocks = npb * kts;                      \
            if (blocks <= 0 || blocks > 0x7fffffffLL) return CLHIP_EINVAL;                                                      \
            hipLaunchKernelGGL((wino_conv16g_kernel<TC_, TR_, ER_, MODE, UNP_>), dim3((unsigned)blocks), dim3(256), 0, s, in, U, \
                               bias, mask_src, out, pool_idx, N, Cin, Cout, H, W, relu, tiles_w, groups, (int)npb);             \
            CLHIP_LAUNCH_CHECK();                                                                                               \
            return 0;                                                                                                           \
        } while (0)
        if ((H | W) & 1) { if (W <= 16) WINO_16G(8, 2, 1, false); }
        else if (W >= 16) WINO_16G(8, 2, 4, UNPOOL);
        else if (H == 8 && W == 8) WINO_16G(4, 4, 4, UNPOOL);
#undef WINO_16G
    }
#define WINO_GEO(TCB_, TRB_, NIMG_)                                                                                          \
    do {                                                                                                                      \
        const int tiles_w = ((W + 1) / 2 + TCB_ - 1) / TCB_, tiles_h = ((H + 1) / 2 + TRB_ - 1) / TRB_, ngrp = (N + NIMG_ - 1) / NIMG_; \
        const long long npb = (long long)tiles_w * tiles_h * ngrp, blocks = npb * kts;                                        \
        if (blocks <= 0 || blocks > 0x7fffffffLL) return CLHIP_EINVAL;                                                        \
        hipLaunchKernelGGL((wino_conv_kernel<TCB_, TRB_, NIMG_, MODE, UNPOOL>), dim3((unsigned)blocks), dim3(256), 0, s, in, U, \
                           bias, mask_src, out, pool_idx, N, Cin, Cout, H, W, relu, tiles_w, tiles_h, (int)npb);              \
    } while (0)
    WINO_GEO(4, 4, 4);
#undef WINO_GEO
    CLHIP_LAUNCH_CHECK();
    return 0;
}

}

bool clhip_internal_wino_ok(int Cin, int Cout, int H, int W) {
    if (Cin % WCK || Cin < 16 || Cout % 32 || H < 4 || W < 8) return false;
    if (((H | W) & 1) == 0) return true;
    return W > 8 && W <= 16;
}

size_t clhip_internal_wino_ws(int Cin, int Cout) {
    return (size_t)((Cout + WKT - 1) / WKT) * ((Cin + WCK - 1) / WCK) * WU_FLOATS * sizeof(float);
}

int clhip_internal_wino_conv_u(int mode, const float* in, const float* U, const float* bias, const float* mask_src, float* out,
                               uint8_t* pool_idx, int unpool, int N, int Cin, int Cout, int H, int W, int relu, hipStream_t s) {
    if (!in || !U || !out || !clhip_internal_wino_ok(Cin, Cout, H, W)) return CLHIP_EINVAL;
    if (((H | W) & 1) && (pool_idx || unpool)) return CLHIP_ENOTSUP;
    if (mode == 0) return launch_wino<0, false>(in, U, bias, nullptr, out, pool_idx, N, Cin, Cout, H, W, relu, s);
    if (unpool) return launch_wino<1, true>(in, U, nullptr, mask_src, out, pool_idx, N, Cin, Cout, H, W, 0, s);
    return launch_wino<1, false>(in, U, nullptr, mask_src, out, nullptr, N, Cin, Cout, H, W, 0, s);
}

int clhip_internal_wino_weights(const clhip_wino_wt* jobs, int n, hipStream_t s) {
    if (n <= 0) return 0;
    if (!jobs) return CLHIP_EINVAL;
    for (int base = 0; base < n; base += WT_JOBS) {
        WtJobs J;
        J.n = n - base < WT_JOBS ? n - base : WT_JOBS;
        J.pad = 0;
        int blocks = 0;
        for (int i = 0; i < J.n; ++i) {
            const clhip_wino_wt& q = jobs[base + i];
            if (!q.w || !q.U || q.Ko <= 0 || q.Ci <= 0) return CLHIP_EINVAL;
            J.j[i] = q;
            J.first[i] = blocks;
            const int total = ((q.Ko + WKT - 1) / WKT) * ((q.Ci + WCK - 1) / WCK) * WCK * WKT;
            blocks += (total + 255) / 256;
        }
        J.first[J.n] = blocks;
        hipLaunchKernelGGL(wino_weight_multi_kernel, dim3(blocks), dim3(256), 0, s, J);
        CLHIP_LAUNCH_CHECK();
    }
    return 0;
}

int clhip_internal_weight_images(const clhip_wino_wt* wj, int nw, const clhip_wino_wt* bj, int nb, hipStream_t s) {
    if (nw <= 0 || nb <= 0 || nw + nb > WT_JOBS) {
        const int rc = clhip_internal_wino_weights(wj, nw, s);
        if (rc) return rc;
        return clhip_internal_bs_weights(bj, nb, s);
    }
    if (!wj || !bj) return CLHIP_EINVAL;
    WtJobs J;
    J.n = nw + nb;
    J.pad = 0;
    int blocks = 0;
    for (int i = 0; i < J.n; ++i) {
        const bool is_bs = i >= nw;
        const clhip_wino_wt& q = is_bs ? bj[i - nw] : wj[i];
        if (!q.w || !q.U || q.Ko <= 0 || q.Ci <= 0) return CLHIP_EINVAL;
        J.j[i] = q;
        J.first[i] = blocks;
        if (is_bs) {
            J.pad |= 1 << i;
            blocks += bs_weight_blocks(q);
        } else {
            const int total = ((q.Ko + WKT - 1) / WKT) * ((q.Ci + WCK - 1) / WCK) * WCK * WKT;
            blocks += (total + 255) / 256;
        }
    }
    J.first[J.n] = blocks;
    hipLaunchKernelGGL(wino_weight_multi_kernel, dim3(blocks), dim3(256), 0, s, J);
    CLHIP_LAUNCH_CHECK();
    return 0;
}

int clhip_internal_wino_conv(int mode, const float* in, const float* w, const float* bias, const float* mask_src, float* out,
                             uint8_t* pool_idx, int unpool, int N, int Cin, int Cout, int H, int W, int relu, void* ws,
                             size_t ws_bytes, hipStream_t s) {
    if (!in || !w || !out || !ws || !clhip_internal_wino_ok(Cin, Cout, H, W) || ws_bytes < clhip_internal_wino_ws(Cin, Cout))
        return CLHIP_EINVAL;
    float* U = static_cast<float*>(ws);
    const int n_chunks = (Cin + WCK - 1) / WCK;
    const int total = ((Cout + WKT - 1) / WKT) * n_chunks * WCK * WKT;
    hipLaunchKernelGGL(wino_weight_kernel, dim3((total + 255) / 256), dim3(256), 0, s, w, U, Cout, Cin, mode, n_chunks);
    CLHIP_LAUNCH_CHECK();
    return clhip_internal_wino_conv_u(mode, in, U, bias, mask_src, out, pool_idx, unpool, N, Cin, Cout, H, W, relu, s);
}

bool clhip_internal_wino_wgrad_ok(int C, int K, int H, int W) {
    return C % WKT == 0 && K % WKT == 0 && H >= 4 && W >= 8;
}

size_t clhip_internal_wino_wgrad_ws(int N, int C, int K, int H, int W) {
    if (N <= 0 || !clhip_internal_wino_wgrad_ok(C, K, H, W)) return 0;
    const int kc_tiles = (K / WKT) * (C / WKT);
    return ((size_t)9 * K * C + K) * (size_t)((256 + kc_tiles - 1) / kc_tiles) * sizeof(float);
}

struct WgradGeo {
    bool wide, ps, vec;
    int tiles_w, tiles_h, kc_tiles, kc32;
    long long total, splits;
    size_t slab;
};

static int wino_wgrad_geo(const float* x, const float* dy, const uint8_t* unpool_idx, int N, int C, int K, int H, int W,
                          size_t ws_bytes, WgradGeo* g) {
    if (!clhip_internal_wino_wgrad_ok(C, K, H, W)) return CLHIP_ENOTSUP;
    if ((size_t)N * K * H * W >= ((size_t)1 << 29) || (size_t)N * C * H * W >= ((size_t)1 << 29)) return CLHIP_ENOTSUP;
    g->wide = W >= 16;
    const int TCS = g->wide ? 8 : 4, TRS = g->wide ? 2 : 4;
    if (((H | W) & 1) && unpool_idx) return CLHIP_ENOTSUP;
    g->tiles_w = ((W + 1) / 2 + TCS - 1) / TCS;
    g->tiles_h = ((H + 1) / 2 + TRS - 1) / TRS;
    g->total = (long long)g->tiles_w * g->tiles_h * N;
    if (g->total > 0x7fffffffLL) return CLHIP_ENOTSUP;
    g->kc_tiles = (K / WKT) * (C / WKT);
    g->slab = (size_t)9 * K * C + K;
    long long splits = g->kc_tiles >= 256 ? 1 : 256 / g->kc_tiles;
    if (splits > g->total) splits = g->total;
    const long long cap = (long long)(ws_bytes / (g->slab * sizeof(float)));
    if (cap < 1) return CLHIP_ENOSPC;
    if (splits > cap) splits = cap;
    g->splits = splits;
    g->vec = W % (2 * TCS) == 0 && ((reinterpret_cast<uintptr_t>(x) | reinterpret_cast<uintptr_t>(dy)) & 15) == 0;
    g->kc32 = (K / 32) * (C / 32);
    g->ps = wgrad_ps_on() && g->total < 16 * splits;
    if (g->ps) {
        const int target = ((long long)H * W <= 64 && g->kc32 <= 16) ? 256 : 512;
        long long sp = g->kc32 >= target ? 1 : target / g->kc32;
        if (sp > g->total) sp = g->total;
        if (sp > cap) sp = cap;
        g->splits = sp;
    }
    return 0;
}

int clhip_internal_wino_wgrad_partial(const float* x, const float* dy, const uint8_t* unpool_idx, float* dw, float* db, int N, int C,
                                      int K, int H, int W, void* ws, size_t ws_bytes, hipStream_t s, clhip_wgrad_job* job) {
    if (!x || !dy || !dw || !ws || !job || N <= 0) return CLHIP_EINVAL;
    WgradGeo g;
    const int rc = wino_wgrad_geo(x, dy, unpool_idx, N, C, K, H, W, ws_bytes, &g);
    if (rc) return rc;
    const bool wide = g.wide;
    const int tiles_w = g.tiles_w, tiles_h = g.tiles_h, kc_tiles = g.kc_tiles;
    const long long total = g.total, splits = g.splits;
    const size_t slab = g.slab;
    float* part = static_cast<float*>(ws);
    if (g.ps) {
        const long long sp = g.splits;
        const unsigned gridp = (unsigned)(g.kc32 * sp);
        const bool vec = g.vec;
#define WGP(TCS_, TRS_, UNP_)                                                                                                       \
        do {                                                                                                                       \
            if (vec) hipLaunchKernelGGL((wino_wgrad_ps_kernel<TCS_, TRS_, UNP_, true>), dim3(gridp), dim3(256), 0, s, x, dy, part,  \
                                        unpool_idx, N, C, K, H, W, tiles_w, tiles_h, (int)total, (int)sp, C / 32, slab);            \
            else hipLaunchKernelGGL((wino_wgrad_ps_kernel<TCS_, TRS_, UNP_, false>), dim3(gridp), dim3(256), 0, s, x, dy, part,     \
                                    unpool_idx, N, C, K, H, W, tiles_w, tiles_h, (int)total, (int)sp, C / 32, slab);                \
        } while (0)
        if (wide) { if (unpool_idx) WGP(8, 2, true); else WGP(8, 2, false); }
        else { if (unpool_idx) WGP(4, 4, true); else WGP(4, 4, false); }
#undef WGP
        CLHIP_LAUNCH_CHECK();
        *job = clhip_wgrad_job{part, dw, db, K, C, (int)sp};
        return 0;
    }
    const unsigned grid = (unsigned)(kc_tiles * splits);
    const bool vecg = g.vec;
#define WG(TCS_, TRS_, UNP_)                                                                                                         \
    do {                                                                                                                            \
        if (vecg) hipLaunchKernelGGL((wino_wgrad_kernel<TCS_, TRS_, 1, UNP_, true>), dim3(grid), dim3(256), 0, s, x, dy, part,       \
                                     unpool_idx, N, C, K, H, W, tiles_w, tiles_h, (int)total, (int)splits, C / WKT, slab);           \
        else hipLaunchKernelGGL((wino_wgrad_kernel<TCS_, TRS_, 1, UNP_, false>), dim3(grid), dim3(256), 0, s, x, dy, part,           \
                                unpool_idx, N, C, K, H, W, tiles_w, tiles_h, (int)total, (int)splits, C / WKT, slab);                \
    } while (0)
    if (wide) { if (unpool_idx) WG(8, 2, true); else WG(8, 2, false); }
    else { if (unpool_idx) WG(4, 4, true); else WG(4, 4, false); }
#undef WG
    CLHIP_LAUNCH_CHECK();
    *job = clhip_wgrad_job{part, dw, db, K, C, (int)splits};
    return 0;
}

#ifndef CLHIP_PAIR_MAX_PIXELS
#define CLHIP_PAIR_MAX_PIXELS 256
#endif
int clhip_internal_wino_pair(const float* dy, const uint8_t* unpool_idx, const float* U, const float* mask_src, float* dx,
                             const float* x, float* dw, float* db, int N, int C, int K, int H, int W, void* ws, size_t ws_bytes,
                             hipStream_t s, clhip_wgrad_job* job) {
    if (!dy || !U || !dx || !x || !dw || !ws || !job || N <= 0) return CLHIP_EINVAL;
    if (((H | W) & 1) || (long long)H * W > CLHIP_PAIR_MAX_PIXELS || !clhip_internal_wino_ok(K, C, H, W)) return CLHIP_ENOTSUP;
    const bool wide = W >= 16, m88 = H == 8 && W == 8;
    if (!wide && !m88) return CLHIP_ENOTSUP;
    WgradGeo g;
    const int rc = wino_wgrad_geo(x, dy, unpool_idx, N, C, K, H, W, ws_bytes, &g);
    if (rc) return rc == CLHIP_ENOSPC ? CLHIP_ENOTSUP : rc;
    if (!g.ps || !g.vec || g.wide != wide) return CLHIP_ENOTSUP;
    const int TC = wide ? 8 : 4, TR = wide ? 2 : 4, ER = 4, NE = 2 * TR / ER;
    const int d_tiles_w = (W / 2 + TC - 1) / TC, d_groups = (H / 2 + ER - 1) / ER;
    const bool narrow = m88 && ((long long)N * 16 + 31) / 32 * ((C + 31) / 32) < WINO16_BELOW_UNITS && (long long)N * ((C + 31) / 32) <= 512;
    const long long npb = narrow ? N : (((long long)N * d_groups + NE - 1) / NE) * d_tiles_w, nb_d = npb * ((C + WKT - 1) / WKT);
    const long long nb_w = (long long)g.kc32 * g.splits;
    if (nb_d <= 0 || nb_w <= 0 || nb_d + nb_w > 0x7fffffffLL) return CLHIP_ENOTSUP;
    float* part = static_cast<float*>(ws);
    uint8_t* idx = const_cast<uint8_t*>(unpool_idx);
#define PAIR(DK_, TC_, TR_, UNP_)                                                                                                   \
    hipLaunchKernelGGL((wino_pair_kernel<DK_, TC_, TR_, 4, UNP_, TC_, TR_>), dim3((unsigned)(nb_d + nb_w)), dim3(256), 0, s, dy, U,  \
                       mask_src, dx, idx, N, K, C, H, W, d_tiles_w, d_groups, (int)npb, x, part, g.tiles_w, g.tiles_h, (int)g.total, \
                       (int)g.splits, C / 32, g.slab, (int)nb_w)
    if (wide) { if (unpool_idx) PAIR(0, 8, 2, true); else PAIR(0, 8, 2, false); }
    else if (narrow) { if (unpool_idx) PAIR(1, 4, 4, true); else PAIR(1, 4, 4, false); }
    else { if (unpool_idx) PAIR(0, 4, 4, true); else PAIR(0, 4, 4, false); }
#undef PAIR
    CLHIP_LAUNCH_CHECK();
    *job = clhip_wgrad_job{part, dw, db, K, C, (int)g.splits};
    return 0;
}

bool clhip_internal_wino_pair_shape(int N, int C, int K, int H, int W, int pooled) {
    if (N <= 0 || ((H | W) & 1) || (long long)H * W > CLHIP_PAIR_MAX_PIXELS || !clhip_internal_wino_ok(K, C, H, W)) return false;
    const bool wide = W >= 16, m88 = H == 8 && W == 8;
    if (!wide && !m88) return false;
    WgradGeo g;
// ... 71 lines not shown
```

clsurvey_amd/net.py:

```python
import ctypes as C
import weakref

import torch
import torch.nn as nn

from . import _lib
from ._lib import check, LayerDesc


def _pad4(n):
    return (n + 3) // 4 * 4


class ParamArena:
    _registry = weakref.WeakValueDictionary()

    @classmethod
    def find(cls, params):
        params = list(params)
        if not params:
            return None
        a = cls._registry.get(id(params[0]))
        if a is None or len(a.params) != len(params) or any(x is not y for x, y in zip(a.params, params)):
            return None
# ... 70 lines not shown
            if ks[0] != ks[1] or st[0] != st[1] or pd[0] != pd[1] or m.groups != 1 or _pair(m.dilation) != (1, 1):
                raise NotImplementedError("NetEngine: square kernels, symmetric stride / padding, no groups / dilation")
            j = i + 1
            if j < len(feats) and isinstance(feats[j], nn.BatchNorm2d):
                bn = feats[j]
                if not with_bn:
                    raise NotImplementedError("this caller does not handle BatchNorm2d layers")
                if not bn.affine or not bn.track_running_stats or bn.momentum is None or bn.num_features != m.out_channels:
                    raise NotImplementedError("NetEngine: BatchNorm2d must be affine with running statistics and a momentum")
                bns[len(layers)] = bn
                j += 1
            relu = j < len(feats) and isinstance(feats[j], nn.ReLU)
            j += 1 if relu else 0
            pool = False
            if j < len(feats) and isinstance(feats[j], nn.MaxPool2d):
                mp = feats[j]
                pk, ps = _pair(mp.kernel_size), _pair(mp.stride if mp.stride is not None else mp.kernel_size)
                if pk[0] != pk[1] or ps[0] != ps[1] or _pair(mp.padding) != (0, 0) or mp.ceil_mode or _pair(mp.dilation) != (1, 1):
                    raise NotImplementedError("NetEngine: square un-padded floor-mode max-pool only")
                pool = True if (pk[0], ps[0]) == (2, 2) else (pk[0], ps[0])
                j += 1
            if pending is not None:
                drops[len(layers)] = pending
                pending = None
            layers.append(("conv", m, relu, pool))
            i = j
        else:
            raise NotImplementedError("NetEngine: unsupported feature module %r" % (m,))
    cls = list(model.classifier.children())
    i = 0
    while i < len(cls):
        m = cls[i]
        if isinstance(m, nn.Dropout):
            pending = m
            i += 1
        elif isinstance(m, nn.Linear):
            relu = i + 1 < len(cls) and isinstance(cls[i + 1], nn.ReLU)
            if pending is not None:
                drops[len(layers)] = pending
                pending = None
            layers.append(("fc", m, relu, False))
            i += 2 if relu else 1
        else:
            raise NotImplementedError("NetEngine: unsupported classifier module %r" % (m,))
    if pending is not None or 0 in drops:
        raise NotImplementedError("NetEngine: Dropout must sit in front of a layer other than the first")
    return (layers, drops, bns) if with_bn else (layers, drops)


def parse_vgg(model):
    return parse_net(model)[0]


def conv_geometry(m):
    return _pair(m.kernel_size)[0], _pair(m.stride)[0], _pair(m.padding)[0]


class NetEngine:
    LOSS = {"ce_mean": 0, "ce_sum": 1, "mse_sum_zero": 2}

    def __init__(self, model, max_batch, in_shape, device="cuda", layers=None, params=None, drops=None):
        self.model = model
        self.device = torch.device(device)
        self.drops, self.bns = {}, {}
        if layers is None:
            self.layers, self.drops, self.bns = parse_net(model, with_bn=True)
            specs = [(kind, m.weight, m.bias, m.in_channels if kind == "conv" else m.in_features,
                      m.out_channels if kind == "conv" else m.out_features, relu, pool) +
                     ((conv_geometry(m),) if kind == "conv" else ()) for kind, m, relu, pool in self.layers]
        else:
            specs = list(layers)
            self.layers = specs
            self.drops = dict(drops or {})
        if any(sp[2] is None for sp in specs):
            raise NotImplementedError("NetEngine: layers without bias")
        self.arena = ParamArena(list(model.parameters()) if params is None else list(params), self.device)
        descs = (LayerDesc * len(specs))()
        for d, sp in zip(descs, specs):
            kind, w, b, cin, cout, relu, pool = sp[:7]
            d.type = 0 if kind == "conv" else 1
            d.cin, d.cout = int(cin), int(cout)
            d.relu, d.pool = int(relu), int(bool(pool))
            if isinstance(pool, tuple):
                d.pool_k, d.pool_s = int(pool[0]), int(pool[1])
            if kind == "conv":
                d.ksize, d.stride, d.pad = (int(v) for v in (sp[7] if len(sp) > 7 else (w.shape[2], 1, w.shape[2] // 2)))
            d.w_off = self.arena.slot(w)[0]
            d.b_off = self.arena.slot(b)[0]
        for li in self.drops:
            descs[li].has_drop = 1
        for li, bn in self.bns.items():
            descs[li].bn = 1
            descs[li].bn_w_off = self.arena.slot(bn.weight)[0]
            descs[li].bn_b_off = self.arena.slot(bn.bias)[0]
        self.max_batch = int(max_batch)
        self.in_shape = tuple(in_shape)
        h = C.c_void_p()
        L = _lib.lib()
        check(L.clhip_net_create(descs, len(specs), self.max_batch, *self.in_shape, C.byref(h)),
              "clhip_net_create")
        self._h = h
        self.n_classes = L.clhip_net_num_classes(h)
        self.ws = torch.empty(L.clhip_net_workspace_bytes(h), dtype=torch.uint8, device=self.device)
        self.loss = torch.zeros(1, dtype=torch.float32, device=self.device)
        for li, bn in self.bns.items():
            for name in ("running_mean", "running_var", "num_batches_tracked"):
                buf = getattr(bn, name)
                buf.data = buf.data.to(self.device).contiguous()
            check(L.clhip_net_set_bn(h, li, bn.running_mean.data_ptr(), bn.running_var.data_ptr(), float(bn.momentum), float(bn.eps)),
                  "clhip_net_set_bn")
        self._training = None
        self.in_elems = {}
        shp = self.in_shape
        if self.drops:
            with torch.no_grad():
                c, h, w = shp
                for li, sp in enumerate(specs):
                    self.in_elems[li] = c * h * w
                    if sp[0] == "conv":
                        ks, st, pd = sp[7] if len(sp) > 7 else (3, 1, 1)
                        c, h, w = sp[4], (h + 2 * pd - ks) // st + 1, (w + 2 * pd - ks) // st + 1
                        if sp[6]:
                            pk, ps = sp[6] if isinstance(sp[6], tuple) else (2, 2)
                            h, w = (h - pk) // ps + 1, (w - pk) // ps + 1
                    else:
                        c, h, w = sp[4], 1, 1
        self.auto_dropout = True
        self._masks = {}

    def set_dropout(self, layer, mask):
        if mask is None:
            self._masks.pop(layer, None)
            ptr, stride = None, 0
        else:
            if not mask.is_cuda or mask.dtype != torch.float32 or not mask.is_contiguous():
                raise RuntimeError("dropout masks are contiguous fp32 HIP tensors")
            if mask.shape[-1] != self.in_elems[layer] or (mask.dim() == 2 and mask.shape[0] < 1):
                raise RuntimeError("dropout mask shape %s does not fit layer %d" % (tuple(mask.shape), layer))
            self._masks[layer] = mask
            ptr, stride = mask.data_ptr(), (mask.shape[-1] if mask.dim() == 2 else 0)
        check(_lib.lib().clhip_net_set_dropout(self._h, int(layer), ptr, int(stride)), "clhip_net_set_dropout")

    def layer_input(self, layer, n):
        off, elems = C.c_size_t(), C.c_size_t()
        check(_lib.lib().clhip_net_layer_input(self._h, int(layer), C.byref(off), C.byref(elems)), "clhip_net_layer_input")
        lo = off.value * 4
        return self.ws[lo:lo + n * elems.value * 4].view(torch.float32).view(n, elems.value)

    def pool_idx(self, layer, n):
        off, elems = C.c_size_t(), C.c_size_t()
        check(_lib.lib().clhip_net_layer_pool_idx(self._h, int(layer), C.byref(off), C.byref(elems)), "clhip_net_layer_pool_idx")
        return self.ws[off.value:off.value + n * elems.value].view(n, elems.value)

    def layer_paths(self, layer):
        bits = _lib.lib().clhip_net_layer_paths(self._h, int(layer))
        if bits < 0:
            raise RuntimeError("clhip_net_layer_paths(%d)" % layer)
        return {"fwd": bool(bits & 1), "bwd_data": bool(bits & 2), "bwd_weight": bool(bits & 4),
                "bs_fwd": bool(bits & 8), "bs_bwd_data": bool(bits & 16), "bs_bwd_weight": bool(bits & 32)}

    def set_input_grad(self, layer, extra):
        if extra is not None and (not extra.is_cuda or extra.dtype != torch.float32 or not extra.is_contiguous()):
            raise RuntimeError("set_input_grad needs a contiguous fp32 HIP tensor")
        self._extra = extra
        check(_lib.lib().clhip_net_set_input_grad(self._h, int(layer), extra.data_ptr() if extra is not None else None),
              "clhip_net_set_input_grad")

    def _mode(self):
        if not self.bns:
            return
        training = bool(self.model.training)
        if training != self._training:
            check(_lib.lib().clhip_net_set_training(self._h, int(training)), "clhip_net_set_training")
            self._training = training
        if training:
            for bn in self.bns.values():
                bn.num_batches_tracked += 1

    def probe(self, layer, kind="fwd"):
        k = {"fwd": 0, "bwd_data": 1, "bwd_weight": 2}[kind]
        check(_lib.lib().clhip_net_probe_kind(self._h, -1 if layer is None else int(layer), k), "clhip_net_probe_kind")

    def probe_read(self):
        import ctypes as C
        us, n = C.c_float(0.0), C.c_int(0)
        check(_lib.lib().clhip_net_probe_read(self._h, C.byref(us), C.byref(n)), "clhip_net_probe_read")
        return float(us.value), int(n.value)

    def _auto_drop(self, n):
        if not self.drops or not self.auto_dropout:
            return
        for li, m in self.drops.items():
            if self.model.training and m.p > 0:
                keep = 1.0 - m.p
                mask = torch.empty((n, self.in_elems[li]), dtype=torch.float32, device=self.device).bernoulli_(keep).div_(keep)
                self.set_dropout(li, mask)
            elif li in self._masks:
                self.set_dropout(li, None)

    def __del__(self):
        try:
            if getattr(self, "_h", None):
                _lib.lib().clhip_net_destroy(self._h)
                self._h = None
        except Exception:
            pass

    def _check_x(self, x):
        if not x.is_cuda or x.dtype != torch.float32 or not x.is_contiguous():
            raise RuntimeError("NetEngine needs contiguous fp32 HIP tensors")
        if tuple(x.shape[1:]) != self.in_shape or x.shape[0] > self.max_batch:
            raise RuntimeError("NetEngine: bad input shape %s" % (tuple(x.shape),))

    def forward(self, x, params=None):
        self._check_x(x)
        self._mode()
        self._auto_drop(x.shape[0])
        logits = torch.empty((x.shape[0], self.n_classes), dtype=torch.float32, device=self.device)
        check(_lib.lib().clhip_net_forward(self._h, (params if params is not None else self.arena.theta).data_ptr(),
                                           x.data_ptr(), x.shape[0],
                                           self.ws.data_ptr(), logits.data_ptr(),
                                           torch.cuda.current_stream().cuda_stream), "clhip_net_forward")
        return logits

    def backward(self, x, dlogits):
        self._check_x(x)
        check(_lib.lib().clhip_net_backward(self._h, self.arena.theta.data_ptr(), self.arena.grad.data_ptr(), x.data_ptr(),
                                            x.shape[0], self.ws.data_ptr(), dlogits.data_ptr(),
                                            torch.cuda.current_stream().cuda_stream), "clhip_net_backward")

    def loss_step(self, x, y, kind="ce_mean", backward=True, stats=None, want_logits=False, params=None,
                  class_slice=None):
        self._check_x(x)
        self._mode()
        self._auto_drop(x.shape[0])
        logits = torch.empty((x.shape[0], self.n_classes), dtype=torch.float32, device=self.device) if want_logits else None
        o1, nc = (class_slice[0], class_slice[1] - class_slice[0]) if class_slice is not None else (0, 0)
        check(_lib.lib().clhip_net_loss_step_slice(
            self._h, (params if params is not None else self.arena.theta).data_ptr(),
            self.arena.grad.data_ptr() if backward else None, x.data_ptr(),
            y.data_ptr() if y is not None else None, x.shape[0], self.LOSS[kind], int(o1), int(nc), self.ws.data_ptr(),
            self.loss.data_ptr(), stats.data_ptr() if stats is not None else None,
            logits.data_ptr() if logits is not None else None, torch.cuda.current_stream().cuda_stream),
            "clhip_net_loss_step_slice")
        return self.loss, logits

    def loss_step_segments(self, x, y, segs, n_segs, stats=None, backward=True, want_logits=False, targets=None, T=1.0):
        self._check_x(x)
        self._mode()
        self._auto_drop(x.shape[0])
        logits = torch.empty((x.shape[0], self.n_classes), dtype=torch.float32, device=self.device) if want_logits else None
        check(_lib.lib().clhip_net_loss_step_loss_segments(
            self._h, self.arena.theta.data_ptr(), self.arena.grad.data_ptr() if backward else None, x.data_ptr(),
            y.data_ptr(), targets.data_ptr() if targets is not None else None, targets.shape[1] if targets is not None else 0,
            x.shape[0], segs.data_ptr(), int(n_segs), float(T), self.ws.data_ptr(), self.loss.data_ptr(),
            stats.data_ptr() if stats is not None else None, logits.data_ptr() if logits is not None else None,
            torch.cuda.current_stream().cuda_stream), "clhip_net_loss_step_loss_segments")
        return self.loss, logits
```

include/clhip.h:

```cpp
#ifndef CLHIP_H
#define CLHIP_H

#include <stddef.h>
#include <stdint.h>

#ifdef __cplusplus
extern "C" {
#endif

#if defined(__GNUC__) || defined(__clang__)
#pragma GCC visibility push(default)
#define CLHIP_VISIBILITY_PUSHED 1
#endif

#define CLHIP_EINVAL (-1)
#define CLHIP_ENOSPC (-2)
#define CLHIP_ENOTSUP (-3)

int clhip_sigmoid_fwd(const float* x, float* y, size_t n, void* stream);
int clhip_sigmoid_bwd(const float* dy, const float* y, float* dx, size_t n, void* stream);
int clhip_mse_mean(const float* a, const float* b, size_t n, float grad_scale, float* da, float* loss_out, void* stream);
int clhip_adadelta_step(float* theta, const float* grad, float* square_avg, float* acc_delta, size_t n, float lr, float rho,
                        float eps, float weight_decay, void* stream);

// ... 28 lines not shown
int clhip_maxpool2_bwd(const float* dy, const uint8_t* idx_u8, float* dx, int NC, int H, int W,
                       void* stream);

int clhip_maxpool_fwd(const float* x, float* y, uint8_t* idx_u8, int NC, int H, int W, int k, int stride, void* stream);
int clhip_maxpool_bwd(const float* dy, const uint8_t* idx_u8, float* dx, int NC, int H, int W, int k, int stride, void* stream);

size_t clhip_bn_ws(int C);
int clhip_bn_fwd(const float* z, const float* gamma, const float* beta, float* running_mean, float* running_var, float* y,
                 float* save_mean, float* save_invstd, int N, int C, int HW, int training, float momentum, float eps, int relu,
                 void* ws, size_t ws_bytes, void* stream);
int clhip_bn_bwd(const float* dy, const float* y, const float* z, const float* gamma, const float* save_mean,
                 const float* save_invstd, float* dz, float* dgamma, float* dbeta, int N, int C, int HW, int training, int relu,
                 void* ws, size_t ws_bytes, void* stream);

size_t clhip_conv2d_bwd_weight_ws(int N, int C, int H, int W, int K, int R, int S, int stride, int pad);
int clhip_conv2d_fwd(const float* x, const float* w, const float* b, float* y, int N, int C, int H, int W, int K, int R, int S,
                     int stride, int pad, int relu, void* stream);
int clhip_conv2d_bwd_data(const float* dy, const float* w, const float* relu_src, float* dx, int N, int C, int H, int W, int K,
                          int R, int S, int stride, int pad, void* stream);
int clhip_conv2d_bwd_weight(const float* x, const float* dy, float* dw, float* db, int N, int C, int H, int W, int K, int R,
                            int S, int stride, int pad, void* ws, size_t ws_bytes, void* stream);

size_t clhip_conv3x3_bs_bwd_weight_ws(int N, int C, int K, int H, int W);
int clhip_conv3x3_bs_bwd_weight(const float* x, const float* dy, const uint8_t* idx_u8_or_null, float* dw, float* db, int N, int C, int K,
                                int H, int W, void* ws, size_t ws_bytes, void* stream);

size_t clhip_conv5x5_bs_bwd_weight_ws(int N, int C, int K, int H, int W);
int clhip_conv5x5_bs_bwd_weight(const float* x, const float* dy, float* dw, float* db, int N, int C, int K, int H, int W, void* ws,
                                size_t ws_bytes, void* stream);

size_t clhip_conv2d_s2d_ws(int N, int C, int H, int W, int K, int R, int stride, int pad);
int clhip_conv2d_s2d_fwd(const float* x, const float* w, const float* b, float* y, int N, int C, int H, int W, int K, int R, int stride,
                         int pad, int relu, void* ws, size_t ws_bytes, void* stream);
int clhip_conv2d_s2d_bwd_weight(const float* x_or_null, const float* dy, float* dw, float* db, int N, int C, int H, int W, int K, int R,
                                int stride, int pad, void* ws, size_t ws_bytes, void* stream);

size_t clhip_fc_ws(int M, int I, int O);
int clhip_fc_fwd(const float* x, const float* w, const float* b, float* y,
                 int M, int I, int O, int relu, void* ws, size_t ws_bytes, void* stream);
int clhip_fc_bwd_data(const float* dy, const float* w, const float* relu_src, float* dx,
                      int M, int I, int O, void* ws, size_t ws_bytes, void* stream);
int clhip_fc_bwd_weight(const float* x, const float* dy, float* dw, float* db,
                        int M, int I, int O, void* ws, size_t ws_bytes, void* stream);
int clhip_relu_bwd(const float* dy, const float* y, float* dx, size_t n, void* stream);

int clhip_softmax_ce(const float* logits, const int64_t* labels_i64, int N, int C, int reduction,
                     float* dlogits, float* loss_out, double* stats, void* stream);
int clhip_softmax_ce_slice(const float* logits, const int64_t* labels_i64, int N, int ld, int col_off, int ncols,
                           int reduction, float* dlogits, float* loss_out, double* stats, void* stream);
int clhip_mse_zero_sum(const float* logits, size_t n, float* dlogits, float* loss_out, void* stream);

int clhip_lwf_loss(const float* logits, const int64_t* labels_i64, const float* teacher, const int* head_sizes, int n_heads,
                   int N, int ld, int ld_teacher, float T, float reg_lambda, int distill, float* dlogits, float* loss_out2,
                   double* stats, void* stream);

int clhip_reg_sgd_step(float* theta, const float* grad, const float* omega, const float* init_val,
                       float* buf, size_t n, float reg_lambda, float lr, float momentum, float wd,
                       int first, void* stream);
int clhip_fisher_accum(float* omega, const float* grad, size_t n, float data_len, void* stream);
int clhip_mas_accum(float* omega, const float* grad, size_t n, float prev_size, float curr_size,
                    void* stream);
int clhip_si_step(float* theta, const float* grad, const float* omega, const float* init_val,
                  float* w, float* buf, size_t n, float reg_lambda, float lr, float momentum,
                  float wd, int first, void* stream);
int clhip_si_consolidate(float* omega, float* w, const float* theta, float* init_val, size_t n,
                         float slack, void* stream);

int clhip_imm_merge(const float* const* thetas, const float* const* precisions, const float* sum_precision,
                    int n_models, size_t n, float* out, void* stream);

int clhip_packnet_finetune_mask(uint8_t* mask_u8, size_t n, int cur, void* stream);
size_t clhip_packnet_kth_ws(void);
int clhip_packnet_kth_abs(const float* w, const uint8_t* mask_u8, size_t n, int cur, size_t k,
                          float* out_cutoff, void* ws, size_t ws_bytes, void* stream);
int clhip_packnet_prune(float* w, uint8_t* mask_u8, size_t n, int cur, const float* cutoff_dev, void* stream);
int clhip_mask_grad_zero(float* grad, const uint8_t* mask_u8, size_t n, int cur, void* stream);
int clhip_mask_weight_zero(float* w, const uint8_t* mask_u8, size_t n, int mode, int idx, void* stream);
int clhip_packnet_sgd_step(float* theta, float* grad, float* buf, const uint8_t* mask_u8, size_t n, int cur,
                           float lr, float momentum, float wd, int first, void* stream);

size_t clhip_conv3x3_wino_ws(int C, int K);
int clhip_conv3x3_wino_fwd(const float* x, const float* w, const float* b, float* y, uint8_t* idx_u8_or_null, int N, int C, int K,
                           int H, int W, int relu, void* ws, size_t ws_bytes, void* stream);
int clhip_conv3x3_wino_bwd_data(const float* dy, const uint8_t* idx_u8_or_null, const float* w, const float* relu_src, float* dx,
                                int N, int C, int K, int H, int W, void* ws, size_t ws_bytes, void* stream);
size_t clhip_conv3x3_wino_bwd_weight_ws(int N, int C, int K, int H, int W);
int clhip_conv3x3_wino_bwd_weight(const float* x, const float* dy, const uint8_t* idx_u8_or_null, float* dw, float* db, int N, int C,
                                  int K, int H, int W, void* ws, size_t ws_bytes, void* stream);
size_t clhip_conv3x3_wino_bwd_ws(int N, int C, int K, int H, int W);
int clhip_conv3x3_wino_bwd(const float* x, const float* dy, const uint8_t* idx_u8_or_null, const float* w, const float* relu_src,
                           float* dx, float* dw, float* db, int N, int C, int K, int H, int W, void* ws, size_t ws_bytes, void* stream);

size_t clhip_conv3x3_bs_ws(int C, int K);
int clhip_conv3x3_bs_fwd(const float* x, const float* w, const float* b, float* y, uint8_t* idx_u8_or_null, int N, int C, int K,
                         int H, int W, int relu, void* ws, size_t ws_bytes, void* stream);
int clhip_conv3x3_bs_bwd_data(const float* dy, const uint8_t* idx_u8_or_null, const float* w, const float* relu_src, float* dx,
                              int N, int C, int K, int H, int W, void* ws, size_t ws_bytes, void* stream);
size_t clhip_conv5x5_bs_ws(int C, int K);
int clhip_conv5x5_bs_fwd(const float* x, const float* w, const float* b, float* y, int N, int C, int K, int H, int W, int relu,
                         void* ws, size_t ws_bytes, void* stream);
int clhip_conv5x5_bs_bwd_data(const float* dy, const float* w, const float* relu_src, float* dx, int N, int C, int K, int H, int W,
                              void* ws, size_t ws_bytes, void* stream);

int clhip_hat_gate(const float* emb_row, int n, float s, float* gate, void* stream);
int clhip_hat_scale_weight(const float* w, const float* gate_in, float* out, size_t K, size_t C, size_t R, void* stream);
int clhip_hat_weight_grad(const float* g_wprime, const float* w, const float* gate_in, float* dw, float* dgate_in,
                          int K, int C, int R, void* stream);
int clhip_hat_emb_grad(const float* dgate, const float* gate, const float* mask_pre, int n, float s,
                       float lamb_over_count, float* demb, void* stream);
int clhip_hat_reg_sums(const float* gate, const float* mask_pre, int n, double* sums2, void* stream);
int clhip_hat_backmask(const float* a_post, const float* a_pre, float* out, size_t K, size_t C, size_t R, void* stream);
size_t clhip_hat_sgd_ws(void);
int clhip_hat_sgd_step(float* theta, float* grad, float* buf, const float* mask_back, size_t n, float lr,
                       float momentum, float wd, int is_emb, int finetune, float s, float smax, float thres_cosh,
                       float clipgrad, int first, void* ws, size_t ws_bytes, void* stream);
int clhip_clamp(float* x, size_t n, float lo, float hi, void* stream);

typedef struct { float* theta; float* grad; float* buf; const float* mask_back; size_t n; int is_emb; int reserved; } clhip_hat_param;
typedef struct { const float* emb_row; float* gate; const float* mask_pre; int n; int reserved; } clhip_hat_gate_job;
typedef struct { const float* w; const float* gate_in; float* out; size_t K, C, R; } clhip_hat_layer;
typedef struct { float* g; const float* w; const float* gate_in; float* dgate_in; int K, C, R, reserved; } clhip_hat_wgrad_job;
typedef struct { const float* dgate; const float* gate; const float* mask_pre; float* demb; int n, rows, t, reserved; } clhip_hat_emb_job;
size_t clhip_hat_sgd_multi_ws(int n_params);
int clhip_hat_sgd_step_multi(const clhip_hat_param* params, int n_params, float lr, float momentum, float wd, int finetune,
                             float s, float smax, float thres_cosh, float clipgrad, float thres_emb, int first, void* ws,
                             size_t ws_bytes, void* stream);
int clhip_hat_gates_multi(const clhip_hat_gate_job* jobs, int n_jobs, float s, double* sums2, void* stream);
int clhip_hat_scale_weights_multi(const clhip_hat_layer* layers, int n_layers, void* stream);
int clhip_hat_weight_grads_multi(const clhip_hat_wgrad_job* jobs, int n_jobs, void* stream);
int clhip_hat_emb_grads_multi(const clhip_hat_emb_job* jobs, int n_jobs, float s, float lamb, float count, const double* sums2,
                              void* stream);

typedef struct {
    int type;
    int cin, cout;
    int relu, pool;
    long w_off, b_off;
    int ksize, stride, pad;
    int pool_k, pool_s;
    int bn;
    long bn_w_off, bn_b_off;
    int has_drop;
} clhip_layer_desc;

int clhip_net_create(const clhip_layer_desc* layers, int n_layers, int max_batch, int in_c, int in_h,
                     int in_w, void** out_handle);
int clhip_net_set_dropout(void* handle, int layer, const float* mask, long row_stride);
int clhip_net_set_bn(void* handle, int layer, float* running_mean, float* running_var, float momentum, float eps);
int clhip_net_set_training(void* handle, int training);
int clhip_net_probe(void* handle, int layer);
int clhip_net_probe_kind(void* handle, int layer, int kind);
int clhip_net_probe_read(void* handle, float* avg_us, int* count);
int clhip_net_layer_pool_idx(void* handle, int layer, size_t* ws_byte_off, size_t* elems_per_sample);
int clhip_net_layer_paths(void* handle, int layer);

int clhip_net_layer_input(void* handle, int layer, size_t* ws_float_off, size_t* in_elems);
int clhip_net_set_input_grad(void* handle, int layer, const float* extra);
void clhip_net_destroy(void* handle);
size_t clhip_net_workspace_bytes(void* handle);
int clhip_net_num_classes(void* handle);
int clhip_net_forward(void* handle, const float* params, const float* x, int N, void* ws,
                      float* logits_out, void* stream);
int clhip_net_backward(void* handle, const float* params, float* grads, const float* x, int N, void* ws,
                       const float* dlogits, void* stream);
int clhip_net_loss_step(void* handle, const float* params, float* grads, const float* x,
                        const int64_t* labels_i64, int N, int loss_kind, void* ws, float* loss_out,
                        double* stats, float* logits_out, void* stream);

int clhip_net_loss_step_slice(void* handle, const float* params, float* grads, const float* x,
                              const int64_t* labels_i64, int N, int loss_kind, int col_off, int ncols, void* ws,
                              float* loss_out, double* stats, float* logits_out, void* stream);

int clhip_axpy(float* y, const float* x, size_t n, float alpha, int assign, void* stream);
size_t clhip_gem_gram_ws(int m);
int clhip_gem_gram(const float* G, size_t ld, const int* row_idx_host, int m, size_t n, double* out_f64, void* ws,
                   size_t ws_bytes, void* stream);
int clhip_gem_project(const float* G, size_t ld, const int* row_idx_host, const float* v_host, int m, const float* g,
                      float* out, size_t n, void* stream);
int clhip_gem_qp(const double* gram_f64, int m, double margin, double eps, double* v_out_f64, int* info_i32, void* stream);
int clhip_gem_project_dev(const float* G, size_t ld, const int* row_idx_host, const double* v_dev_f64, const int* info_dev,
                          int m, const float* g, float* out, size_t n, void* stream);

#define CLHIP_LOSS_MAX_ROWS 1024
#define CLHIP_LOSS_MAX_SEGS 256
typedef struct clhip_loss_segment { int row_begin; int row_end; int col_off; int ncols; float scale; int kind; } clhip_loss_segment;
int clhip_rehearsal_assemble(const float* x, const int64_t* labels_i64, int B, size_t row_elems, float* store_x,
                             int64_t* store_labels, long store_rows, long ring_row0, int ring_rows, const int* gather_rows,
                             int E, float* x_mix, int64_t* labels_mix, void* stream);
int clhip_rehearsal_assemble_crop_flip(const float* x, const int64_t* labels_i64, int B, int C, int Hs, int Ws, int th, int tw,
                                       const float* src_frames, long src_rows, const int64_t* src_idx, float* store_frames,
                                       int64_t* store_labels, long store_rows, long ring_row0, int ring_rows,
                                       const int* gather_rows, const int* gather_params, int E, float* x_mix, int64_t* labels_mix,
                                       void* stream);
int clhip_loss_segments(const float* logits, const int64_t* labels_i64, const float* targets, int ld_t, int N, int ld,
                        const clhip_loss_segment* segs, int n_segs, float T, float* dlogits, float* loss_out, double* stats,
                        void* stream);
int clhip_net_loss_step_loss_segments(void* handle, const float* params, float* grads, const float* x,
                                      const int64_t* labels_i64, const float* targets, int ld_t, int N,
                                      const clhip_loss_segment* segs, int n_segs, float T, void* ws, float* loss_out,
                                      double* stats, float* logits_out, void* stream);

#define CLHIP_MAX_TASKS 64
typedef struct clhip_task_src { const float* x; const int64_t* labels; int64_t cum_rows; int64_t label_shift; } clhip_task_src;
int clhip_gather_tasks(const clhip_task_src* tasks_dev, int T, size_t row_elems, const int64_t* idx, int B, float* x_out,
                       int64_t* labels_out, void* stream);
int clhip_slice_argmax_count(const float* logits, int N, int ld, const int* cols, int K, const int64_t* labels_i64,
                             int64_t* correct, int64_t* total, int64_t* out_of_range, void* stream);

int clhip_gather_tasks_crop_flip(const clhip_task_src* tasks_dev, int T, int C, int Hs, int Ws, int th, int tw, const int64_t* idx,
                                 const int* params, int B, float* x_out, int64_t* labels_out, void* stream);

#define CLHIP_ICARL_MAX_CLASSES 128
#define CLHIP_ICARL_MAX_FEATS 4096
#define CLHIP_ICARL_MAX_CLASS_ROWS 65536
typedef struct clhip_icarl_class { int row_begin; int row_end; int k; int out_off; } clhip_icarl_class;
int clhip_icarl_herd(const float* feats, long n_rows, int F, const float* w, const clhip_icarl_class* classes_host,
                     int n_classes, int* ranking, long ranking_len, void* stream);
int clhip_icarl_nme(const float* feats, const float* means, int N, int F, int C, int offset1, int n_outputs, float* out,
                    void* stream);

#ifdef CLHIP_VISIBILITY_PUSHED
#pragma GCC visibility pop
#undef CLHIP_VISIBILITY_PUSHED
#endif

#ifdef __cplusplus
}
#endif
#endif
```

Measured before the change: 284,700 images/s.

## Fuse weight-image preparation into first conv+ReLU+pool kernel launch

The Winograd and BS weight-image transforms, which used to run as a separate kernel before the forward pass, are now appended as extra blocks to the first-layer C=3 conv+ReLU+pool grid. This removes one kernel launch and lets the weight transforms run alongside the first conv. Shared weight-image code moves into a header so both kernels can use it, and new debug accessors expose the prepared weights and a count of fused launches. The trade-off is a heterogeneous grid: 512-thread blocks do 256-thread weight work, so half their threads idle, and the bigger kernel may change occupancy.

```diff
diff --git a/clsurvey_amd/_lib.py b/clsurvey_amd/_lib.py
--- a/clsurvey_amd/_lib.py
+++ b/clsurvey_amd/_lib.py
@@ -133,6 +133,8 @@
     "clhip_net_probe_read": (_i, [_p, C.POINTER(_f), C.POINTER(_i)]),
     "clhip_net_layer_input": (_i, [_p, _i, _p, _p]),
     "clhip_net_layer_pool_idx": (_i, [_p, _i, _p, _p]),
+    "clhip_net_prepared_weights": (_i, [_p, _p, _p]),
+    "clhip_net_edge_grid_count": (_i, [_p]),
     "clhip_net_layer_paths": (_i, [_p, _i]),
     "clhip_net_probe_kind": (_i, [_p, _i, _i]),
     "clhip_net_set_input_grad": (_i, [_p, _i, _p]),
diff --git a/clsurvey_amd/csrc/common.hpp b/clsurvey_amd/csrc/common.hpp
--- a/clsurvey_amd/csrc/common.hpp
+++ b/clsurvey_amd/csrc/common.hpp
@@ -139,6 +139,9 @@
 struct clhip_wino_wt { const float* w; float* U; int Ko, Ci, mode, pad; };
 int clhip_internal_wino_weights(const clhip_wino_wt* jobs, int n, hipStream_t s);
 int clhip_internal_weight_images(const clhip_wino_wt* wino_jobs, int n_wino, const clhip_wino_wt* bs_jobs, int n_bs, hipStream_t s);
+int clhip_internal_c3w64_pool_weight_images(const float* x, const float* w, const float* b, float* y_pool, uint8_t* idx_u8, int N, int C,
+                                            int K, int H, int W, const clhip_wino_wt* wino_jobs, int n_wino, const clhip_wino_wt* bs_jobs,
+                                            int n_bs, int wt_first, hipStream_t s);
 int clhip_internal_wino_conv_u(int mode, const float* in, const float* U, const float* bias, const float* mask_src, float* out,
                                uint8_t* pool_idx, int unpool, int N, int Cin, int Cout, int H, int W, int relu, hipStream_t s);
 bool clhip_internal_wino_ok(int Cin, int Cout, int H, int W);
diff --git a/clsurvey_amd/csrc/conv3x3.hip b/clsurvey_amd/csrc/conv3x3.hip
--- a/clsurvey_amd/csrc/conv3x3.hip
+++ b/clsurvey_amd/csrc/conv3x3.hip
@@ -1,4 +1,5 @@
 #include "common.hpp"
+#include "weight_images.hpp"
 
 namespace {
 
@@ -815,19 +816,20 @@
 #else
 #define C3W64_MFMA(a, b, c, x, y, z) __builtin_amdgcn_mfma_f32_32x32x2f32(a, b, c, x, y, z)
 #endif
+constexpr int W6_AUX = CLHIP_C3W64_BIAS_IN_K ? W6_TWP + 5 : KT;
 template <bool FULL>
-__global__ __launch_bounds__(512) void conv3x3_c3w64_relu_pool_kernel(
+__device__ __forceinline__ void c3w64_relu_pool_body(
+    float* __restrict__ halo_s, float* __restrict__ aux_s, const int bx, const int by, const int gx,
     const float* __restrict__ x, const float* __restrict__ wt, const float* __restrict__ bias,
     float* __restrict__ out, uint8_t* __restrict__ pool_idx, int N, int Cout, int H, int W,
     int tiles_w, int row_pairs, int ntiles) {
-    __shared__ __attribute__((aligned(16))) float halo_s[8 * 2 * W6_HALO];
 #if CLHIP_C3W64_BIAS_IN_K
-    __shared__ float ones_s[W6_TWP + 5];
+    float* const ones_s = aux_s;
 #else
-    __shared__ float bias_s[KT];
+    float* const bias_s = aux_s;
 #endif
     const int tid = threadIdx.x, lane = tid & 63, wave = tid >> 6, li = lane & 31, kk = lane >> 5;
-    const int ko0 = blockIdx.y * KT;
+    const int ko0 = by * KT;
 #if CLHIP_C3W64_BIAS_IN_K
     if (tid < W6_TWP + 5) ones_s[tid] = 1.f;
 #else
@@ -862,7 +864,7 @@
         return 2 * li + 2 * W6_PLANE + 2 * W6_TWP + 2;
     };
 
-    const int simd = blockIdx.x * 4 + (wave & 3), nsimd = gridDim.x * 4;
+    const int simd = bx * 4 + (wave & 3), nsimd = gx * 4;
     const int units = 2 * ntiles;
     const int per = units / nsimd, rem = units - per * nsimd;
     const int s_start = simd * per + min(simd, rem), s_cnt = per + (simd < rem ? 1 : 0);
@@ -1001,13 +1003,63 @@
     }
 }
 
+template <bool FULL>
+__global__ __launch_bounds__(512) void conv3x3_c3w64_relu_pool_kernel(
+    const float* __restrict__ x, const float* __restrict__ wt, const float* __restrict__ bias,
+    float* __restrict__ out, uint8_t* __restrict__ pool_idx, int N, int Cout, int H, int W,
+    int tiles_w, int row_pairs, int ntiles) {
+    __shared__ __attribute__((aligned(16))) float halo_s[8 * 2 * W6_HALO];
+    __shared__ float aux_s[W6_AUX];
+    c3w64_relu_pool_body<FULL>(halo_s, aux_s, (int)blockIdx.x, (int)blockIdx.y, (int)gridDim.x, x, wt, bias, out, pool_idx, N, Cout, H, W,
+                               tiles_w, row_pairs, ntiles);
+}
+
+template <bool FULL>
+__global__ __launch_bounds__(512) void c3w64_relu_pool_wt_kernel(
+    const float* __restrict__ x, const float* __restrict__ wt, const float* __restrict__ bias,
+    float* __restrict__ out, uint8_t* __restrict__ pool_idx, int N, int Cout, int H, int W,
+    int tiles_w, int row_pairs, int ntiles, int gx, int nfl, int nwb, int wt_first, WtJobs J) {
+    __shared__ __attribute__((aligned(16))) float halo_s[8 * 2 * W6_HALO];
+    __shared__ float aux_s[W6_AUX];
+    const int b = (int)blockIdx.x;
+    const int fb = wt_first ? b - nwb : b;
+    if ((unsigned)fb >= (unsigned)nfl) {
+        const int vb = 2 * (wt_first ? b : b - nfl) + ((int)threadIdx.x >> 8);
+        if (vb < J.first[J.n]) weight_image_block(J, vb, (int)threadIdx.x & 255);
+        return;
+    }
+    c3w64_relu_pool_body<FULL>(halo_s, aux_s, fb % gx, fb / gx, gx, x, wt, bias, out, pool_idx, N, Cout, H, W, tiles_w, row_pairs, ntiles);
+}
+
+static inline long long c3w64_gx(long long ntiles) {
+    long long gx = 256;
+    if (gx * 8 > 2 * ntiles) gx = (2 * ntiles + 7) / 8;
+    return gx;
+}
+
+int launch_c3w64_pool_wt(const float* x, const float* wt, const float* bias, float* out, uint8_t* idx, int N, int Cout, int H, int W,
+                         const WtJobs& J, int wt_first, hipStream_t s) {
+    const int tiles_w = W / 64, row_pairs = H / 2;
+    const long long ntiles = (long long)tiles_w * row_pairs * N;
+    const int kts = (Cout + KT - 1) / KT;
+    const long long gx = c3w64_gx(ntiles);
+    const int nfl = (int)(gx * kts), nwb = (J.first[J.n] + 1) / 2;
+    if (Cout % KT == 0)
+        hipLaunchKernelGGL(c3w64_relu_pool_wt_kernel<true>, dim3((unsigned)(nfl + nwb)), dim3(512), 0, s,
+                           x, wt, bias, out, idx, N, Cout, H, W, tiles_w, row_pairs, (int)ntiles, (int)gx, nfl, nwb, wt_first, J);
+    else
+        hipLaunchKernelGGL(c3w64_relu_pool_wt_kernel<false>, dim3((unsigned)(nfl + nwb)), dim3(512), 0, s,
+                           x, wt, bias, out, idx, N, Cout, H, W, tiles_w, row_pairs, (int)ntiles, (int)gx, nfl, nwb, wt_first, J);
+    CLHIP_LAUNCH_CHECK();
+    return 0;
+}
+
 int launch_c3w64_pool(const float* x, const float* wt, const float* bias, float* out, uint8_t* idx,
                       int N, int Cout, int H, int W, hipStream_t s) {
     const int tiles_w = W / 64, row_pairs = H / 2;
     const long long ntiles = (long long)tiles_w * row_pairs * N;
     const int kts = (Cout + KT - 1) / KT;
-    long long gx = 256;
-    if (gx * 8 > 2 * ntiles) gx = (2 * ntiles + 7) / 8;
+    const long long gx = c3w64_gx(ntiles);
     if (Cout % KT == 0)
         hipLaunchKernelGGL(conv3x3_c3w64_relu_pool_kernel<true>, dim3((unsigned)gx, (unsigned)kts), dim3(512), 0, s,
                            x, wt, bias, out, idx, N, Cout, H, W, tiles_w, row_pairs, (int)ntiles);
@@ -1033,6 +1085,11 @@
     return 0;
 }
 
+bool c3w64_shape(int N, int C, int K, int H, int W) {
+    return CLHIP_C3W64 && C == 3 && W % 64 == 0 && H % 2 == 0 && (size_t)N * 3 * H * W < ((size_t)1 << 29) &&
+           (size_t)N * K * (H / 2) * (W / 2) < ((size_t)1 << 29);
+}
+
 bool vec_ok(const float* in, const float* wt, int Cin, int H, int W, int Cw) {
     const int TW = W > 16 ? 32 : (W > 8 ? 16 : 8);
     return (Cin % 8 == 0) && (Cw % 4 == 0) && (W % 4 == 0) && (W % TW == 0) && aligned16(in) && aligned16(wt);
@@ -1063,15 +1120,28 @@
     if (!x || !w || !y_pool || !idx_u8 || N <= 0 || C <= 0 || K <= 0 || H <= 0 || W <= 0 || (H & 1) || (W & 1))
         return CLHIP_EINVAL;
     hipStream_t s = as_stream(stream);
-    if (CLHIP_C3W64 && C == 3 && W % 64 == 0 && H % 2 == 0 && (size_t)N * 3 * H * W < ((size_t)1 << 29) &&
-        (size_t)N * K * (H / 2) * (W / 2) < ((size_t)1 << 29))
-        return launch_c3w64_pool(x, w, b, y_pool, idx_u8, N, K, H, W, s);
+    if (c3w64_shape(N, C, K, H, W)) return launch_c3w64_pool(x, w, b, y_pool, idx_u8, N, K, H, W, s);
     if (C == 3 && W % C3_TW == 0) return launch_c3_pool(x, w, b, y_pool, idx_u8, N, K, H, W, s);
 
     if (C <= 4) return launch_conv<4, 0, false>(x, w, b, nullptr, y_pool, N, C, K, H, W, K, C, 1, s, idx_u8);
     if (vec_ok(x, w, C, H, W, C)) return launch_conv<8, 0, true>(x, w, b, nullptr, y_pool, N, C, K, H, W, K, C, 1, s, idx_u8);
     return launch_conv<8, 0, false>(x, w, b, nullptr, y_pool, N, C, K, H, W, K, C, 1, s, idx_u8);
 }
+
+}
+
+int clhip_internal_c3w64_pool_weight_images(const float* x, const float* w, const float* b, float* y_pool, uint8_t* idx_u8, int N, int C,
+                                            int K, int H, int W, const clhip_wino_wt* wj, int nw, const clhip_wino_wt* bj, int nb,
+                                            int wt_first, hipStream_t s) {
+    if (!x || !w || !y_pool || !idx_u8 || N <= 0 || C <= 0 || K <= 0 || H <= 0 || W <= 0) return CLHIP_EINVAL;
+    if (!c3w64_shape(N, C, K, H, W) || nw < 0 || nb < 0 || nw + nb <= 0 || nw + nb > WT_JOBS) return CLHIP_ENOTSUP;
+    WtJobs J;
+    const int blocks = weight_jobs_table(wj, nw, bj, nb, J);
+    if (blocks < 0) return blocks;
+    return launch_c3w64_pool_wt(x, w, b, y_pool, idx_u8, N, K, H, W, J, wt_first, s);
+}
+
+extern "C" {
 
 int clhip_conv3x3_bwd_data(const float* dy, const float* w, const float* relu_src, float* dx,
                            int N, int C, int K, int H, int W, void* stream) {
diff --git a/clsurvey_amd/csrc/engine.hip b/clsurvey_amd/csrc/engine.hip
--- a/clsurvey_amd/csrc/engine.hip
+++ b/clsurvey_amd/csrc/engine.hip
@@ -50,6 +50,9 @@
 }
 
 constexpr unsigned PROBE_RING = 64;
+#ifndef CLHIP_EDGE_GRIDS_DEFAULT
+#define CLHIP_EDGE_GRIDS_DEFAULT 1
+#endif
 #ifndef CLHIP_OVERLAP_DEFAULT
 #define CLHIP_OVERLAP_DEFAULT 0
 #endif
@@ -80,6 +83,8 @@
     bool fc_tail, no_combo;
     unsigned* tail_counter;
     size_t off_rows;
+    int edge_grids;
+    unsigned edge_count;
     bool overlap;
     int overlap_mode;
     hipStream_t side;
@@ -332,6 +337,9 @@
             p->side = nullptr;
         }
     }
+    p->edge_count = 0;
+    const char* eg = getenv("CLHIP_EDGE_GRIDS");
+    p->edge_grids = (eg && eg[0] >= '0' && eg[0] <= '2' && !eg[1]) ? eg[0] - '0' : CLHIP_EDGE_GRIDS_DEFAULT;
     p->probe_layer = -1;
     p->probe_kind = 0;
     p->probe_count = 0;
@@ -389,6 +397,19 @@
     return 0;
 }
 
+int clhip_net_edge_grid_count(void* handle) {
+    NetPlan* p = static_cast<NetPlan*>(handle);
+    return p ? (int)(p->edge_count & 0x7fffffffu) : CLHIP_EINVAL;
+}
+
+int clhip_net_prepared_weights(void* handle, size_t* ws_byte_off, size_t* bytes) {
+    NetPlan* p = static_cast<NetPlan*>(handle);
+    if (!p || !ws_byte_off || !bytes) return CLHIP_EINVAL;
+    *ws_byte_off = p->off_wino;
+    *bytes = p->wino_bytes;
+    return 0;
+}
+
 int clhip_net_layer_paths(void* handle, int layer) {
     NetPlan* p = static_cast<NetPlan*>(handle);
     if (!p || layer < 0 || layer >= (int)p->layers.size()) return CLHIP_EINVAL;
@@ -481,8 +502,8 @@
               : clhip_internal_wino_conv_u(mode, in, U, bias, mask_src, out, pool_idx, unpool, N, Cin, Cout, H, W, relu, s);
 }
 
-static int wino_prepare(NetPlan* p, const float* params, char* base, bool fwd, bool bwd, hipStream_t s) {
-    std::vector<clhip_wino_wt> jobs, bsjobs;
+static void wino_collect(const NetPlan* p, const float* params, char* base, bool fwd, bool bwd, std::vector<clhip_wino_wt>& jobs,
+                         std::vector<clhip_wino_wt>& bsjobs) {
     jobs.reserve(2 * p->layers.size());
     bsjobs.reserve(2 * p->layers.size());
     for (const LayerPlan& L : p->layers) {
@@ -496,6 +517,11 @@
         if (bwd && L.bs5_d)
             bsjobs.push_back(clhip_wino_wt{params + L.w_off, reinterpret_cast<float*>(base + p->off_wino + L.wino_ud), L.cin, L.cout, 1, 5});
     }
+}
+
+static int wino_prepare(NetPlan* p, const float* params, char* base, bool fwd, bool bwd, hipStream_t s) {
+    std::vector<clhip_wino_wt> jobs, bsjobs;
+    wino_collect(p, params, base, fwd, bwd, jobs, bsjobs);
     return clhip_internal_weight_images(jobs.data(), (int)jobs.size(), bsjobs.data(), (int)bsjobs.size(), s);
 }
 
@@ -507,9 +533,18 @@
     float* acts = reinterpret_cast<float*>(base + p->off_acts);
     uint8_t* idx = reinterpret_cast<uint8_t*>(base + p->off_idx);
     void* scratch = base + p->off_scratch;
+    std::vector<clhip_wino_wt> edge_jobs, edge_bsjobs;
+    bool edge = false;
     if (p->wino_bytes) {
-        int rcw = wino_prepare(p, params, base, true, prep_bwd, as_stream(stream));
-        if (rcw) return rcw;
+        const LayerPlan& L0 = p->layers[0];
+        edge = p->edge_grids && L0.type == 0 && L0.ks == 3 && L0.st == 1 && L0.pd == 1 && !L0.bn && L0.pool && L0.pk == 2 && L0.ps == 2 &&
+               L0.relu && !L0.wino_f && !L0.drop && L0.cin == 3;
+        if (edge) {
+            wino_collect(p, params, base, true, prep_bwd, edge_jobs, edge_bsjobs);
+        } else {
+            int rcw = wino_prepare(p, params, base, true, prep_bwd, as_stream(stream));
+            if (rcw) return rcw;
+        }
     }
     const float* cur = x;
     int rc;
@@ -567,6 +602,16 @@
         } else if (L.type == 0) {
             if (L.pool && L.relu) {
                 float* pl = acts + L.pool_off;
+                if (li == 0 && edge) {
+                    rc = clhip_internal_c3w64_pool_weight_images(cur, params + L.w_off, params + L.b_off, pl, idx + L.idx_off, N, L.cin, L.cout,
+                                                                 L.h, L.w, edge_jobs.data(), (int)edge_jobs.size(), edge_bsjobs.data(),
+                                                                 (int)edge_bsjobs.size(), p->edge_grids == 2, as_stream(stream));
+                    if (rc == 0) { ++p->edge_count; cur = pl; continue; }
+                    if (rc != CLHIP_ENOTSUP) return rc;
+                    rc = clhip_internal_weight_images(edge_jobs.data(), (int)edge_jobs.size(), edge_bsjobs.data(), (int)edge_bsjobs.size(),
+                                                      as_stream(stream));
+                    if (rc) return rc;
+                }
                 rc = L.wino_f ? plan_conv_u(L.bs_f, 0, cur, reinterpret_cast<const float*>(base + p->off_wino + L.wino_uf),
                                                            params + L.b_off, nullptr, pl, idx + L.idx_off, 0, N, L.cin, L.cout, L.h, L.w, 1,
                                                            as_stream(stream))
diff --git a/clsurvey_amd/csrc/weight_images.hpp b/clsurvey_amd/csrc/weight_images.hpp
--- /dev/null
+++ b/clsurvey_amd/csrc/weight_images.hpp
@@ -0,0 +1,108 @@
+#pragma once
+#include "common.hpp"
+#include "bs_weight.hpp"
+
+namespace {
+
+#ifndef CLHIP_W16G_ADIRECT
+#define CLHIP_W16G_ADIRECT 1
+#endif
+
+constexpr int WKT = 64;
+constexpr int WCK = 8;
+constexpr int WFP = 20;
+constexpr int W_FLOATS = WCK * WKT * WFP;
+constexpr int WD_FLOATS = 4 * WKT * 16;
+#if CLHIP_W16G_ADIRECT
+constexpr int WU_FLOATS = W_FLOATS + 2 * WD_FLOATS;
+#else
+constexpr int WU_FLOATS = W_FLOATS;
+#endif
+
+__device__ __forceinline__ void wino_u_store(float* __restrict__ U, int kts, int n_chunks, int kt, int chunk, int c_l, int k_l,
+                                             const float4 (&u)[4]) {
+    float4* dst = reinterpret_cast<float4*>(U + (((size_t)(kt * n_chunks + chunk) * WCK + c_l) * WKT + k_l) * WFP);
+#pragma unroll
+    for (int a = 0; a < 4; ++a) dst[a] = u[a];
+    dst[4] = make_float4(0.f, 0.f, 0.f, 0.f);
+#if CLHIP_W16G_ADIRECT
+    float* Ud = U + (size_t)kts * n_chunks * W_FLOATS;
+    const int chunk4 = 2 * chunk + (c_l >> 2), q = c_l & 3, wk = k_l >> 5, r = (k_l >> 4) & 1, ti = k_l & 15;
+    float4* dd = reinterpret_cast<float4*>(Ud + ((((size_t)(kt * 2 * n_chunks + chunk4) * 2 + wk) * 2 + r) * 4) * 256 + (q * 16 + ti) * 4);
+#pragma unroll
+    for (int a = 0; a < 4; ++a) dd[a * 64] = u[a];
+#else
+    (void)kts;
+#endif
+}
+
+constexpr int WT_JOBS = 24;
+struct WtJobs { int n; int pad; clhip_wino_wt j[WT_JOBS]; int first[WT_JOBS + 1]; };
+
+__device__ __forceinline__ void wino_weight_one(const float* __restrict__ w, float* __restrict__ U, int Ko, int Ci, int mode,
+                                                int n_chunks, int i) {
+    const int k_l = i % WKT, c_l = (i / WKT) % WCK, chunk = (i / (WKT * WCK)) % n_chunks, kt = i / (WKT * WCK * n_chunks);
+    const int k = kt * WKT + k_l, c = chunk * WCK + c_l;
+    float g[3][3];
+#pragma unroll
+    for (int r = 0; r < 3; ++r)
+#pragma unroll
+        for (int s = 0; s < 3; ++s) {
+            float v = 0.f;
+            if (k < Ko && c < Ci)
+                v = mode == 0 ? w[((size_t)k * Ci + c) * 9 + r * 3 + s] : w[((size_t)c * Ko + k) * 9 + (2 - r) * 3 + (2 - s)];
+            g[r][s] = v;
+        }
+    float t[4][3];
+#pragma unroll
+    for (int s = 0; s < 3; ++s) {
+        t[0][s] = g[0][s];
+        t[1][s] = 0.5f * (g[0][s] + g[1][s] + g[2][s]);
+        t[2][s] = 0.5f * (g[0][s] - g[1][s] + g[2][s]);
+        t[3][s] = g[2][s];
+    }
+    float4 u[4];
+#pragma unroll
+    for (int a = 0; a < 4; ++a)
+        u[a] = make_float4(t[a][0], 0.5f * (t[a][0] + t[a][1] + t[a][2]), 0.5f * (t[a][0] - t[a][1] + t[a][2]), t[a][2]);
+    wino_u_store(U, (Ko + WKT - 1) / WKT, n_chunks, kt, chunk, c_l, k_l, u);
+}
+
+__device__ __forceinline__ void weight_image_block(const WtJobs& J, int vb, int tid) {
+    int jb = 0;
+    for (int i = 1; i < J.n; ++i) jb = (vb >= J.first[i]) ? i : jb;
+    const clhip_wino_wt& q = J.j[jb];
+    if ((J.pad >> jb) & 1) {
+        bs_weight_block(q, vb - J.first[jb], tid);
+        return;
+    }
+    const int n_chunks = (q.Ci + WCK - 1) / WCK;
+    const int total = ((q.Ko + WKT - 1) / WKT) * n_chunks * WCK * WKT;
+    const int i = (vb - J.first[jb]) * 256 + tid;
+    if (i < total) wino_weight_one(q.w, q.U, q.Ko, q.Ci, q.mode, n_chunks, i);
+}
+
+static inline int weight_jobs_table(const clhip_wino_wt* wj, int nw, const clhip_wino_wt* bj, int nb, WtJobs& J) {
+    if (nw < 0 || nb < 0 || nw + nb <= 0 || nw + nb > WT_JOBS || (nw && !wj) || (nb && !bj)) return CLHIP_EINVAL;
+    J.n = nw + nb;
+    J.pad = 0;
+    int blocks = 0;
+    for (int i = 0; i < J.n; ++i) {
+        const bool is_bs = i >= nw;
+        const clhip_wino_wt& q = is_bs ? bj[i - nw] : wj[i];
+        if (!q.w || !q.U || q.Ko <= 0 || q.Ci <= 0) return CLHIP_EINVAL;
+        J.j[i] = q;
+        J.first[i] = blocks;
+        if (is_bs) {
+            J.pad |= 1 << i;
+            blocks += bs_weight_blocks(q);
+        } else {
+            const int total = ((q.Ko + WKT - 1) / WKT) * ((q.Ci + WCK - 1) / WCK) * WCK * WKT;
+            blocks += (total + 255) / 256;
+        }
+    }
+    J.first[J.n] = blocks;
+    return blocks;
+}
+
+}
diff --git a/clsurvey_amd/csrc/wino.hip b/clsurvey_amd/csrc/wino.hip
--- a/clsurvey_amd/csrc/wino.hip
+++ b/clsurvey_amd/csrc/wino.hip
@@ -1,5 +1,5 @@
 #include "common.hpp"
-#include "bs_weight.hpp"
+#include "weight_images.hpp"
 #include <cstdlib>
 
 namespace {
@@ -28,37 +28,7 @@
 #ifndef CLHIP_W16G_PF
 #define CLHIP_W16G_PF 2
 #endif
-#ifndef CLHIP_W16G_ADIRECT
-#define CLHIP_W16G_ADIRECT 1
-#endif
-
-constexpr int WKT = 64;
-constexpr int WCK = 8;
-constexpr int WFP = 20;
-constexpr int W_FLOATS = WCK * WKT * WFP;
-constexpr int WD_FLOATS = 4 * WKT * 16;
-#if CLHIP_W16G_ADIRECT
-constexpr int WU_FLOATS = W_FLOATS + 2 * WD_FLOATS;
-#else
-constexpr int WU_FLOATS = W_FLOATS;
-#endif
-
-__device__ __forceinline__ void wino_u_store(float* __restrict__ U, int kts, int n_chunks, int kt, int chunk, int c_l, int k_l,
-                                             const float4 (&u)[4]) {
-    float4* dst = reinterpret_cast<float4*>(U + (((size_t)(kt * n_chunks + chunk) * WCK + c_l) * WKT + k_l) * WFP);
-#pragma unroll
-    for (int a = 0; a < 4; ++a) dst[a] = u[a];
-    dst[4] = make_float4(0.f, 0.f, 0.f, 0.f);
-#if CLHIP_W16G_ADIRECT
-    float* Ud = U + (size_t)kts * n_chunks * W_FLOATS;
-    const int chunk4 = 2 * chunk + (c_l >> 2), q = c_l & 3, wk = k_l >> 5, r = (k_l >> 4) & 1, ti = k_l & 15;
-    float4* dd = reinterpret_cast<float4*>(Ud + ((((size_t)(kt * 2 * n_chunks + chunk4) * 2 + wk) * 2 + r) * 4) * 256 + (q * 16 + ti) * 4);
-#pragma unroll
-    for (int a = 0; a < 4; ++a) dd[a * 64] = u[a];
-#else
-    (void)kts;
-#endif
-}
+
 
 template <int TCB, int TRB, int NIMG>
 struct WGeoW {
@@ -103,50 +73,8 @@
     }
 }
 
-constexpr int WT_JOBS = 24;
-struct WtJobs { int n; int pad; clhip_wino_wt j[WT_JOBS]; int first[WT_JOBS + 1]; };
-
-__device__ __forceinline__ void wino_weight_one(const float* __restrict__ w, float* __restrict__ U, int Ko, int Ci, int mode,
-                                                int n_chunks, int i) {
-    const int k_l = i % WKT, c_l = (i / WKT) % WCK, chunk = (i / (WKT * WCK)) % n_chunks, kt = i / (WKT * WCK * n_chunks);
-    const int k = kt * WKT + k_l, c = chunk * WCK + c_l;
-    float g[3][3];
-#pragma unroll
-    for (int r = 0; r < 3; ++r)
-#pragma unroll
-        for (int s = 0; s < 3; ++s) {
-            float v = 0.f;
-            if (k < Ko && c < Ci)
-                v = mode == 0 ? w[((size_t)k * Ci + c) * 9 + r * 3 + s] : w[((size_t)c * Ko + k) * 9 + (2 - r) * 3 + (2 - s)];
-            g[r][s] = v;
-        }
-    float t[4][3];
-#pragma unroll
-    for (int s = 0; s < 3; ++s) {
-        t[0][s] = g[0][s];
-        t[1][s] = 0.5f * (g[0][s] + g[1][s] + g[2][s]);
-        t[2][s] = 0.5f * (g[0][s] - g[1][s] + g[2][s]);
-        t[3][s] = g[2][s];
-    }
-    float4 u[4];
-#pragma unroll
-    for (int a = 0; a < 4; ++a)
-        u[a] = make_float4(t[a][0], 0.5f * (t[a][0] + t[a][1] + t[a][2]), 0.5f * (t[a][0] - t[a][1] + t[a][2]), t[a][2]);
-    wino_u_store(U, (Ko + WKT - 1) / WKT, n_chunks, kt, chunk, c_l, k_l, u);
-}
-
 __global__ __launch_bounds__(256) void wino_weight_multi_kernel(WtJobs J) {
-    int jb = 0;
-    for (int i = 1; i < J.n; ++i) jb = ((int)blockIdx.x >= J.first[i]) ? i : jb;
-    const clhip_wino_wt& q = J.j[jb];
-    if ((J.pad >> jb) & 1) {
-        bs_weight_block(q, (int)blockIdx.x - J.first[jb], (int)threadIdx.x);
-        return;
-    }
-    const int n_chunks = (q.Ci + WCK - 1) / WCK;
-    const int total = ((q.Ko + WKT - 1) / WKT) * n_chunks * WCK * WKT;
-    const int i = ((int)blockIdx.x - J.first[jb]) * 256 + threadIdx.x;
-    if (i < total) wino_weight_one(q.w, q.U, q.Ko, q.Ci, q.mode, n_chunks, i);
+    weight_image_block(J, (int)blockIdx.x, (int)threadIdx.x);
 }
 
 template <int TCB, int TRB, int NIMG, int MODE, bool UNPOOL, bool ROWPACK = false>
@@ -1763,26 +1691,9 @@
         if (rc) return rc;
         return clhip_internal_bs_weights(bj, nb, s);
     }
-    if (!wj || !bj) return CLHIP_EINVAL;
     WtJobs J;
-    J.n = nw + nb;
-    J.pad = 0;
-    int blocks = 0;
-    for (int i = 0; i < J.n; ++i) {
-        const bool is_bs = i >= nw;
-        const clhip_wino_wt& q = is_bs ? bj[i - nw] : wj[i];
-        if (!q.w || !q.U || q.Ko <= 0 || q.Ci <= 0) return CLHIP_EINVAL;
-        J.j[i] = q;
-        J.first[i] = blocks;
-        if (is_bs) {
-            J.pad |= 1 << i;
-            blocks += bs_weight_blocks(q);
-        } else {
-            const int total = ((q.Ko + WKT - 1) / WKT) * ((q.Ci + WCK - 1) / WCK) * WCK * WKT;
-            blocks += (total + 255) / 256;
-        }
-    }
-    J.first[J.n] = blocks;
+    const int blocks = weight_jobs_table(wj, nw, bj, nb, J);
+    if (blocks < 0) return blocks;
     hipLaunchKernelGGL(wino_weight_multi_kernel, dim3(blocks), dim3(256), 0, s, J);
     CLHIP_LAUNCH_CHECK();
     return 0;
diff --git a/clsurvey_amd/net.py b/clsurvey_amd/net.py
--- a/clsurvey_amd/net.py
+++ b/clsurvey_amd/net.py
@@ -246,6 +246,17 @@
         check(_lib.lib().clhip_net_layer_pool_idx(self._h, int(layer), C.byref(off), C.byref(elems)), "clhip_net_layer_pool_idx")
         return self.ws[off.value:off.value + n * elems.value].view(n, elems.value)
 
+    def prepared_weights(self):
+        off, nbytes = C.c_size_t(), C.c_size_t()
+        check(_lib.lib().clhip_net_prepared_weights(self._h, C.byref(off), C.byref(nbytes)), "clhip_net_prepared_weights")
+        return self.ws[off.value:off.value + nbytes.value]
+
+    def edge_grid_count(self):
+        n = _lib.lib().clhip_net_edge_grid_count(self._h)
+        if n < 0:
+            raise RuntimeError("clhip_net_edge_grid_count")
+        return n
+
     def layer_paths(self, layer):
         bits = _lib.lib().clhip_net_layer_paths(self._h, int(layer))
         if bits < 0:
diff --git a/include/clhip.h b/include/clhip.h
--- a/include/clhip.h
+++ b/include/clhip.h
@@ -204,6 +204,8 @@
 int clhip_net_probe_kind(void* handle, int layer, int kind);
 int clhip_net_probe_read(void* handle, float* avg_us, int* count);
 int clhip_net_layer_pool_idx(void* handle, int layer, size_t* ws_byte_off, size_t* elems_per_sample);
+int clhip_net_prepared_weights(void* handle, size_t* ws_byte_off, size_t* bytes);
+int clhip_net_edge_grid_count(void* handle);
 int clhip_net_layer_paths(void* handle, int layer);
 
 int clhip_net_layer_input(void* handle, int layer, size_t* ws_float_off, size_t* in_elems);
```

New measurement: 288,700 images/s (median of 6 runs). 1.4% higher.
